# weilonghu/KGC-GCN

Hardware: AMD Instinct MI355X
Metric: aggregated_edges_per_sec (higher is better)
Workload: dtype f32 (dense step as six bf16-split MFMA products, f32 accumulation: f32-faithful); 1 GPU; wn18rr-shape synthetic graph (N=40943, R=11, E=86835), 2-layer M-GCN encoder 100->200->200, full-graph forward, eval mode; n_ranks_seen=1

## Files before the change

include/mgcn_hip.h:

```cpp
#ifndef MGCN_HIP_H
#define MGCN_HIP_H

#include <stddef.h>
#include <stdint.h>

#ifdef __cplusplus
extern "C" {
#endif

#define MGCN_ABI_VERSION 4

enum {
  MGCN_OK = 0,
  MGCN_EINVAL = 1,
  MGCN_ELAUNCH = 2,
  MGCN_EUNSUPPORTED = 3
};

typedef struct mgcn_edge_rec {
  int32_t src;
  int32_t type;
  float norm;
  int32_t eid;
} mgcn_edge_rec;

int mgcn_abi_version(void);
const char *mgcn_last_error(void);

typedef struct mgcn_ingest mgcn_ingest;
int mgcn_ingest_open(const char *train_path, const char *valid_path, const char *test_path, mgcn_ingest **out);
void mgcn_ingest_close(mgcn_ingest *h);
int64_t mgcn_ingest_count(const mgcn_ingest *h, int32_t what);
int mgcn_ingest_triples(const mgcn_ingest *h, int32_t split, int64_t *triples_host);
int64_t mgcn_ingest_names_bytes(const mgcn_ingest *h, int32_t kind);
int mgcn_ingest_names(const mgcn_ingest *h, int32_t kind, char *bytes_host, int64_t *offsets_host);

int mgcn_filter_index_build(int64_t num_triples, const int64_t *triples_host, int64_t num_relations, int64_t *keys_host,
                            int64_t *ptr_host, int32_t *tails_host, int64_t *num_keys, int64_t *num_tails);

int mgcn_csr_build_host(int64_t num_nodes, int64_t num_edges_half, int64_t num_rel_rows,
                        const int64_t *edge_index_host, const int64_t *edge_type_host,
                        int64_t hub_threshold, int64_t hub_chunk, int32_t *rowptr_host,
                        mgcn_edge_rec *rec_host, int64_t *perm_host, int32_t *hubinfo_host,
                        int32_t *chunks_host, int64_t max_chunks, int64_t *num_chunks_host,
                        int32_t *slot_dst_host, int32_t *mirror_host, int32_t *typeptr_host,
                        int32_t *typeslots_host);

int64_t mgcn_hub_partial_floats(int64_t num_chunks, int32_t dim);
int mgcn_aggregate_fwd(int64_t num_nodes, int64_t num_edges_half, int32_t dim, int32_t num_rel_rows,
                       const int32_t *rowptr_dev, const mgcn_edge_rec *rec_dev, const float *x_dev,
                       int64_t ldx, const float *rel_dev, const float *loop_rel_dev, const float *ee_dev,
                       int32_t ee_in_slot_order, const float *loop_edge_dev, float *a_dev, int64_t lda,
                       int64_t node_begin, int64_t node_end, const int32_t *hubinfo_dev, const int32_t *chunks_dev,
                       int64_t chunk_begin, int64_t chunk_end, float *partial_dev, int64_t ee_sub_in, int64_t ee_sub_out,
                       int64_t ee_sub_hub, void *stream);

int mgcn_aggregate_bwd(int64_t num_nodes, int64_t num_edges_half, int32_t dim, int32_t num_rel_rows,
                       const int32_t *rowptr_dev, const mgcn_edge_rec *rec_dev,
                       const int32_t *slot_dst_dev , const int32_t *mirror_dev,
                       const int32_t *hubinfo_dev, const int32_t *chunks_dev, int64_t num_hub_chunks,
                       const int32_t *typeptr_dev, const int32_t *typeslots_dev, const float *x_dev, int64_t ldx, const float *rel_dev, const float *ee_dev,
                       const float *g_dev, int64_t ldg, float *gx_dev, float *gee_dev, float *grel_dev,
                       float *workspace_dev, size_t workspace_bytes, void *stream);
size_t mgcn_aggregate_bwd_workspace(int64_t num_edges_half, int32_t dim, int32_t num_rel_rows, int64_t num_hub_chunks);

size_t mgcn_aggregate_bwd_shard_workspace(int64_t shard_rows, int32_t dim, int32_t num_rel_rows, int64_t num_hub_chunks);
int mgcn_aggregate_bwd_shard(int64_t num_nodes, int64_t num_edges_half, int32_t dim, int32_t num_rel_rows,
                             const mgcn_edge_rec *rec_dev, const int32_t *slot_dst_dev, int64_t node_begin, int64_t node_end,
                             int64_t rows_in, int64_t rows_out, int64_t rows_hub, int64_t ee_sub_in, int64_t ee_sub_out,
                             int64_t ee_sub_hub, const int32_t *src_ptr_dev, const int32_t *src_rows_dev,
                             const int32_t *hubinfo_dev, const int32_t *src_chunks_dev, int64_t num_hub_chunks,
                             const int32_t *type_ptr_dev, const int32_t *type_rows_dev, const float *x_dev, int64_t ldx,
                             const float *rel_dev, const float *ee_dev, const float *g_dev, int64_t ldg, float *gx_dev,
                             float *gee_dev, float *grel_dev, float *workspace_dev, size_t workspace_bytes, void *stream);

int mgcn_dense_bn_tanh_fwd(int64_t num_nodes, int32_t dim_in, int32_t dim_out, const float *a_dev, int64_t lda,
                           const float *w_dev, const float *bias_dev, const float *bn_mean_dev, const float *bn_var_dev,
                           const float *bn_gamma_dev, const float *bn_beta_dev, float bn_eps,
                           float *out_dev, int64_t ldo, void *stream);

int mgcn_fused_kernel_generation(int32_t dim_in, int32_t dim_out, int64_t num_rows, int32_t with_row_bounds);
int mgcn_layer_fwd_fused(int64_t num_nodes, int64_t num_edges_half, int32_t dim_in, int32_t dim_out,
                         int32_t num_rel_rows, const int32_t *rowptr_dev, const mgcn_edge_rec *rec_dev,
                         const float *x_dev, int64_t ldx, const float *rel_dev, const float *loop_rel_dev,
                         const float *ee_dev, int32_t ee_in_slot_order, const float *loop_edge_dev,
                         const float *wp_dev, const float *bias_dev, const float *bn_mean_dev,
                         const float *bn_var_dev, const float *bn_gamma_dev, const float *bn_beta_dev,
                         float bn_eps, float *out_dev, int64_t ldo, int64_t node_begin, int64_t node_end,
                         int64_t ee_sub_in, int64_t ee_sub_out, int64_t ee_sub_hub, const int32_t *hubinfo_dev,
                         const int32_t *chunks_dev, int64_t chunk_begin, int64_t chunk_end, float *partial_dev,
                         const float *rels_weight_dev, float *rel_out_dev, const int32_t *row_bounds_dev,
                         int32_t num_row_bounds, int32_t tune, uint32_t *status_dev, void *stream);
int mgcn_pack_weights(int32_t dim_in, int32_t dim_out, const float *w_dev, float *wp_dev, size_t wp_bytes, void *stream);
size_t mgcn_packed_weights_bytes(int32_t dim_in, int32_t dim_out);
int mgcn_pack_weights_gen(int32_t generation, int32_t dim_in, int32_t dim_out, const float *w_dev, float *wp_dev,
                          size_t wp_bytes, void *stream);
size_t mgcn_packed_weights_bytes_gen(int32_t generation, int32_t dim_in, int32_t dim_out);

size_t mgcn_bn_tanh_train_workspace(int64_t num_rows, int32_t dim_out);
int mgcn_bn_tanh_train_fwd(int64_t num_rows, int32_t dim_out, const float *u_in_dev, const float *u_out_dev,
                           const float *u_loop_dev, int64_t ldu, const float *bias_dev, const float *gamma_dev,
                           const float *beta_dev, float *running_mean_dev, float *running_var_dev, float momentum, float eps,
                           float *z_dev, float *y_dev, float *save_mean_dev, float *save_rstd_dev, float *workspace_dev,
                           size_t workspace_bytes, void *stream);
int mgcn_bn_tanh_train_bwd(int64_t num_rows, int32_t dim_out, const float *z_dev, const float *y_dev, const float *gy_dev,
                           const float *save_mean_dev, const float *save_rstd_dev, const float *gamma_dev, float *gz_dev,
                           float *gu_dev, float *ggamma_dev, float *gbeta_dev, float *workspace_dev, size_t workspace_bytes,
                           void *stream);

int mgcn_bn_train_stage_sum(int64_t num_rows, int32_t dim_out, const float *u_in_dev, const float *u_out_dev,
                            const float *u_loop_dev, int64_t ldu, const float *bias_dev, float *z_dev, float *part_dev, void *stream);
int mgcn_bn_train_stage_center(int64_t num_rows, int32_t dim_out, const float *z_dev, const float *sum_parts_dev, int64_t num_blocks,
                               int64_t total_rows, float *mean_dev, float *part_dev, void *stream);
int mgcn_bn_train_stage_finish(int64_t num_rows, int32_t dim_out, const float *z_dev, const float *sq_parts_dev, int64_t num_blocks,
                               int64_t total_rows, const float *mean_dev, const float *gamma_dev, const float *beta_dev,
                               float *running_mean_dev, float *running_var_dev, float momentum, float eps, float *rstd_dev,
                               float *y_dev, void *stream);
int mgcn_bn_train_bwd_stage_sums(int64_t num_rows, int32_t dim_out, const float *z_dev, const float *y_dev, const float *gy_dev,
                                 const float *save_mean_dev, const float *save_rstd_dev, float *g_part_dev, float *gx_part_dev,
                                 void *stream);
int mgcn_bn_train_bwd_stage_apply(int64_t num_rows, int32_t dim_out, const float *z_dev, const float *y_dev, const float *gy_dev,
                                  const float *save_mean_dev, const float *save_rstd_dev, const float *gamma_dev,
                                  const float *g_parts_dev, const float *gx_parts_dev, int64_t num_blocks, int64_t total_rows,
                                  float *gz_dev, float *gu_dev, float *ggamma_dev, float *gbeta_dev, void *stream);

size_t mgcn_matmul_tn_workspace(int64_t k, int32_t m, int32_t n);
int mgcn_matmul_tn_f32(int64_t k, int32_t m, int32_t n, const float *a_dev, int64_t lda, const float *b_dev, int64_t ldb,
                       float *c_dev, int64_t ldc, float *workspace_dev, size_t workspace_bytes, void *stream);

int mgcn_matmul_f32(int64_t m, int32_t k, int32_t n, const float *a_dev, int64_t lda, const float *b_dev,
                    int64_t ldb, float *c_dev, int64_t ldc, void *stream);

int mgcn_score_fwd(int32_t batch, int64_t n_local, int32_t dim, const float *x_dev, int64_t ldx,
                   const float *ent_dev, int64_t lde, const float *bias_dev, float *score_dev, int64_t lds,
                   void *stream);
int mgcn_score_target(int32_t batch, int64_t n_local, int64_t ent_row0, int32_t dim, const float *x_dev,
                      int64_t ldx, const float *ent_dev, int64_t lde, const float *bias_dev,
                      const int64_t *obj_dev, float *target_dev, void *stream);
int mgcn_score_rank(int32_t batch, int64_t n_local, int64_t ent_row0, int32_t dim, const float *x_dev,
                    int64_t ldx, const float *ent_dev, int64_t lde, const float *bias_dev,
                    const int64_t *obj_dev, const float *target_dev, const float *label_dev, int64_t ldl,
                    const uint32_t *mask_dev, int64_t ldm, int64_t *counts_dev, void *stream);
int64_t mgcn_score_bce_partials(int32_t batch, int64_t n_local);
int mgcn_score_bce_fwd(int32_t batch, int64_t n_local, int32_t dim, const float *x_dev, int64_t ldx, const float *ent_dev,
                       int64_t lde, const float *bias_dev, const uint32_t *mask_dev, int64_t ldm, float hot, float cold,
                       float inv_count, float *grad_logit_dev, int64_t ldg, float *loss_partial_dev, void *stream);

int mgcn_filter_mask(int32_t batch, const int64_t *qkey_dev, int64_t num_keys, const int64_t *keys_dev,
                     const int64_t *ptr_dev, const int32_t *tails_dev, int64_t ent_row0, int64_t n_local,
                     uint32_t *mask_dev, int64_t ldm, void *stream);

int mgcn_label_rows(int32_t batch, const int64_t *qkey_dev, int64_t num_keys, const int64_t *keys_dev,
                    const int64_t *ptr_dev, const int32_t *tails_dev, int64_t ent_row0, int64_t n_local, float hot,
                    float cold, float *out_dev, int64_t ldo, void *stream);

size_t mgcn_score_topk_workspace(int32_t batch, int64_t n_local, int32_t k);
int mgcn_score_topk(int32_t batch, int64_t n_local, int64_t ent_row0, int32_t dim, const float *x_dev, int64_t ldx,
                    const float *ent_dev, int64_t lde, const float *bias_dev, const uint32_t *mask_dev, int64_t ldm,
                    int32_t k, float *out_score_dev, int64_t ldo, int64_t *out_id_dev, int64_t ldi, void *workspace_dev,
                    size_t workspace_bytes, void *stream);
int mgcn_topk_merge(int32_t batch, int32_t lists, const float *in_score_dev, const int64_t *in_id_dev, int64_t ld_in,
                    int32_t k, float *out_score_dev, int64_t *out_id_dev, void *stream);

size_t mgcn_conve_packed_bytes(int32_t k_w, int32_t k_h, int32_t kernel_size, int32_t num_filter, int32_t dim_out);
int mgcn_conve_pack(int32_t k_w, int32_t k_h, int32_t kernel_size, int32_t num_filter, int32_t dim_out,
                    const float *conv_w_dev, const float *conv_b_dev, const float *fc_w_dev, int64_t ldw,
                    const float *fc_b_dev, const float *bn0_mean_dev, const float *bn0_var_dev,
                    const float *bn0_gamma_dev, const float *bn0_beta_dev, float bn0_eps, const float *bn1_mean_dev,
                    const float *bn1_var_dev, const float *bn1_gamma_dev, const float *bn1_beta_dev, float bn1_eps,
                    const float *bn2_mean_dev, const float *bn2_var_dev, const float *bn2_gamma_dev,
                    const float *bn2_beta_dev, float bn2_eps, void *packed_dev, size_t packed_bytes, void *stream);
size_t mgcn_conve_trunk_workspace(int32_t batch, int32_t k_w, int32_t k_h, int32_t kernel_size, int32_t num_filter,
                                  int32_t dim_out);
int mgcn_conve_trunk_fwd(int32_t batch, int32_t k_w, int32_t k_h, int32_t kernel_size, int32_t num_filter,
                         int32_t dim_out, const float *ent_dev, int64_t lde, int64_t ent_rows,
                         const int64_t *src_index_dev, const float *rel_dev, int64_t ldr, int64_t rel_rows,
                         const int64_t *rel_index_dev, const void *packed_dev, float *out_dev, int64_t ldo,
                         void *workspace_dev, size_t workspace_bytes, void *stream);

size_t mgcn_conve_train_workspace(int32_t batch, int32_t k_w, int32_t k_h, int32_t kernel_size, int32_t num_filter,
                                  int32_t dim_out);
int mgcn_conve_train_fwd(int32_t batch, int32_t k_w, int32_t k_h, int32_t kernel_size, int32_t num_filter, int32_t dim_out,
                         const float *s_dev, int64_t lds, const float *r_dev, int64_t ldr, const float *conv_w_dev,
                         const float *conv_b_dev, const float *fc_w_dev, int64_t ldw, const float *fc_b_dev,
                         const float *bn0_gamma_dev, const float *bn0_beta_dev, float *bn0_running_mean_dev,
                         float *bn0_running_var_dev, float bn0_momentum, float bn0_eps, const float *bn1_gamma_dev,
                         const float *bn1_beta_dev, float *bn1_running_mean_dev, float *bn1_running_var_dev, float bn1_momentum,
                         float bn1_eps, const uint8_t *keep_dev, float inv_keep, float *z_dev, int64_t ldz, float *saved_dev,
                         void *workspace_dev, size_t workspace_bytes, void *stream);
int mgcn_conve_train_bwd(int32_t batch, int32_t k_w, int32_t k_h, int32_t kernel_size, int32_t num_filter, int32_t dim_out,
                         const float *s_dev, int64_t lds, const float *r_dev, int64_t ldr, const float *conv_w_dev,
                         const float *fc_w_dev, int64_t ldw, const float *bn0_gamma_dev, const float *bn0_beta_dev,
                         const float *bn1_gamma_dev, const float *bn1_beta_dev, const uint8_t *keep_dev, float inv_keep,
                         const float *saved_dev, const float *gz_dev, int64_t ldg, float *ds_dev, int64_t ldds, float *dr_dev,
                         int64_t lddr, float *d_conv_w_dev, float *d_conv_b_dev, float *d_bn0_gamma_dev, float *d_bn0_beta_dev,
                         float *d_bn1_gamma_dev, float *d_bn1_beta_dev, float *d_fc_w_dev, int64_t lddw, float *d_fc_b_dev,
                         void *workspace_dev, size_t workspace_bytes, void *stream);

#define MGCN_ADAM_CHUNK 8192
#define MGCN_ADAM_BATCH 64
size_t mgcn_adam_sq_norms_workspace(int64_t n, const int64_t *numel_host);
int mgcn_adam_sq_norms(int64_t n, const float *const *grad_host, const int64_t *numel_host, float *sq_dev,
                       void *workspace_dev, size_t workspace_bytes, void *stream);
int mgcn_adam_clip_coef(int64_t n, const float *sq_dev, float max_norm, float *out_dev, void *stream);
int mgcn_adam_step(int64_t n, const float *const *grad_host, float *const *param_host, float *const *exp_avg_host,
                   float *const *exp_avg_sq_host, const int64_t *numel_host, const float *coef_dev, float step_size,
                   float bc2_sqrt, double beta1, double beta2, double eps, double weight_decay, void *stream);

#define MGCN_QUERY_MAX_BATCH 4096
size_t mgcn_query_rows_bwd_workspace(int32_t batch);
int mgcn_query_rows_bwd(int32_t batch, int64_t num_rows, int32_t dim, const int64_t *idx_dev, const float *d_dev, int64_t ldd,
                        float *out_dev, int64_t ldo, void *workspace_dev, size_t workspace_bytes, void *stream);
int mgcn_conve_tail_fwd(int32_t batch, int32_t dim, const float *z_dev, int64_t ldz, const uint8_t *keep_dev, int64_t ldk,
                        float inv_keep, const float *gamma_dev, const float *beta_dev, float *running_mean_dev,
                        float *running_var_dev, float momentum, float eps, float *x_dev, int64_t ldx, float *saved_dev,
                        int64_t ldsv, void *stream);
int mgcn_conve_tail_bwd(int32_t batch, int32_t dim, const float *z_dev, int64_t ldz, const uint8_t *keep_dev, int64_t ldk,
                        float inv_keep, const float *x_dev, int64_t ldx, const float *saved_dev, int64_t ldsv,
                        const float *gamma_dev, const float *gx_dev, int64_t ldg, float *gz_dev, int64_t ldgz,
                        float *d_gamma_dev, float *d_beta_dev, void *stream);

#ifdef __cplusplus
}
#endif
#endif
```

kgc-gcn_amd/_native.py:

```python
import ctypes
import os

import torch

_HERE = os.path.dirname(os.path.abspath(__file__))
LIB_PATH = os.environ.get('MGCN_LIB') or os.path.join(_HERE, 'csrc', 'libmgcn_hip.so')
ABI_VERSION = 4

_lib = None

_i32, _i64, _f32 = ctypes.c_int32, ctypes.c_int64, ctypes.c_float
_ptr = ctypes.c_void_p

_SIGNATURES = {
    'mgcn_abi_version': (ctypes.c_int, []),
    'mgcn_last_error': (ctypes.c_char_p, []),
    'mgcn_csr_build_host': (ctypes.c_int, [_i64, _i64, _i64, _ptr, _ptr, _i64, _i64, _ptr, _ptr, _ptr, _ptr, _ptr, _i64,
                                           _ptr] + [_ptr] * 4),
    'mgcn_aggregate_fwd': (ctypes.c_int, [_i64, _i64, _i32, _i32, _ptr, _ptr, _ptr, _i64, _ptr, _ptr, _ptr, _i32,
                                          _ptr, _ptr, _i64, _i64, _i64, _ptr, _ptr, _i64, _i64, _ptr, _i64, _i64, _i64, _ptr]),
    'mgcn_aggregate_bwd': (ctypes.c_int, [_i64, _i64, _i32, _i32] + [_ptr] * 6 + [_i64, _ptr, _ptr] +
                           [_ptr, _i64, _ptr, _ptr, _ptr, _i64, _ptr, _ptr, _ptr, _ptr, ctypes.c_size_t, _ptr]),
    'mgcn_aggregate_bwd_workspace': (ctypes.c_size_t, [_i64, _i32, _i32, _i64]),
    'mgcn_aggregate_bwd_shard': (ctypes.c_int, [_i64, _i64, _i32, _i32, _ptr, _ptr] + [_i64] * 8 + [_ptr] * 4 + [_i64, _ptr, _ptr,
                                                _ptr, _i64, _ptr, _ptr, _ptr, _i64, _ptr, _ptr, _ptr, _ptr, ctypes.c_size_t, _ptr]),
    'mgcn_aggregate_bwd_shard_workspace': (ctypes.c_size_t, [_i64, _i32, _i32, _i64]),
    'mgcn_bn_train_stage_sum': (ctypes.c_int, [_i64, _i32, _ptr, _ptr, _ptr, _i64, _ptr, _ptr, _ptr, _ptr]),
    'mgcn_bn_train_stage_center': (ctypes.c_int, [_i64, _i32, _ptr, _ptr, _i64, _i64, _ptr, _ptr, _ptr]),
    'mgcn_bn_train_stage_finish': (ctypes.c_int, [_i64, _i32, _ptr, _ptr, _i64, _i64] + [_ptr] * 5 + [_f32, _f32, _ptr, _ptr, _ptr]),
    'mgcn_bn_train_bwd_stage_sums': (ctypes.c_int, [_i64, _i32] + [_ptr] * 8),
    'mgcn_bn_train_bwd_stage_apply': (ctypes.c_int, [_i64, _i32] + [_ptr] * 8 + [_i64, _i64] + [_ptr] * 5),
    'mgcn_dense_bn_tanh_fwd': (ctypes.c_int, [_i64, _i32, _i32, _ptr, _i64] + [_ptr] * 6 + [_f32, _ptr, _i64, _ptr]),
    'mgcn_layer_fwd_fused': (ctypes.c_int, [_i64, _i64, _i32, _i32, _i32, _ptr, _ptr, _ptr, _i64, _ptr, _ptr, _ptr, _i32,
                                            _ptr, _ptr, _ptr, _ptr, _ptr, _ptr, _ptr, _f32, _ptr, _i64, _i64, _i64,
                                            _i64, _i64, _i64, _ptr, _ptr, _i64, _i64, _ptr, _ptr, _ptr, _ptr, _i32, _i32, _ptr,
                                            _ptr]),
    'mgcn_pack_weights': (ctypes.c_int, [_i32, _i32, _ptr, _ptr, ctypes.c_size_t, _ptr]),
    'mgcn_packed_weights_bytes': (ctypes.c_size_t, [_i32, _i32]),
    'mgcn_pack_weights_gen': (ctypes.c_int, [_i32, _i32, _i32, _ptr, _ptr, ctypes.c_size_t, _ptr]),
    'mgcn_packed_weights_bytes_gen': (ctypes.c_size_t, [_i32, _i32, _i32]),
    'mgcn_matmul_f32': (ctypes.c_int, [_i64, _i32, _i32, _ptr, _i64, _ptr, _i64, _ptr, _i64, _ptr]),
    'mgcn_bn_tanh_train_workspace': (ctypes.c_size_t, [_i64, _i32]),
    'mgcn_bn_tanh_train_fwd': (ctypes.c_int, [_i64, _i32, _ptr, _ptr, _ptr, _i64, _ptr, _ptr, _ptr, _ptr, _ptr, _f32, _f32, _ptr,
                                              _ptr, _ptr, _ptr, _ptr, ctypes.c_size_t, _ptr]),
    'mgcn_bn_tanh_train_bwd': (ctypes.c_int, [_i64, _i32] + [_ptr] * 11 + [ctypes.c_size_t, _ptr]),
    'mgcn_matmul_tn_workspace': (ctypes.c_size_t, [_i64, _i32, _i32]),
    'mgcn_matmul_tn_f32': (ctypes.c_int, [_i64, _i32, _i32, _ptr, _i64, _ptr, _i64, _ptr, _i64, _ptr, ctypes.c_size_t, _ptr]),
    'mgcn_score_fwd': (ctypes.c_int, [_i32, _i64, _i32, _ptr, _i64, _ptr, _i64, _ptr, _ptr, _i64, _ptr]),
    'mgcn_score_target': (ctypes.c_int, [_i32, _i64, _i64, _i32, _ptr, _i64, _ptr, _i64, _ptr, _ptr, _ptr, _ptr]),
    'mgcn_score_rank': (ctypes.c_int, [_i32, _i64, _i64, _i32, _ptr, _i64, _ptr, _i64, _ptr, _ptr, _ptr, _ptr, _i64,
                                       _ptr, _i64, _ptr, _ptr]),
    'mgcn_filter_mask': (ctypes.c_int, [_i32, _ptr, _i64, _ptr, _ptr, _ptr, _i64, _i64, _ptr, _i64, _ptr]),
    'mgcn_score_bce_partials': (_i64, [_i32, _i64]),
    'mgcn_hub_partial_floats': (_i64, [_i64, _i32]),
    'mgcn_fused_kernel_generation': (ctypes.c_int, [_i32, _i32, _i64, _i32]),
    'mgcn_score_bce_fwd': (ctypes.c_int, [_i32, _i64, _i32, _ptr, _i64, _ptr, _i64, _ptr, _ptr, _i64, _f32, _f32, _f32, _ptr,
                                          _i64, _ptr, _ptr]),
    'mgcn_label_rows': (ctypes.c_int, [_i32, _ptr, _i64, _ptr, _ptr, _ptr, _i64, _i64, _f32, _f32, _ptr, _i64, _ptr]),
    'mgcn_score_topk_workspace': (ctypes.c_size_t, [_i32, _i64, _i32]),
    'mgcn_score_topk': (ctypes.c_int, [_i32, _i64, _i64, _i32, _ptr, _i64, _ptr, _i64, _ptr, _ptr, _i64, _i32, _ptr, _i64,
                                       _ptr, _i64, _ptr, ctypes.c_size_t, _ptr]),
    'mgcn_topk_merge': (ctypes.c_int, [_i32, _i32, _ptr, _ptr, _i64, _i32, _ptr, _ptr, _ptr]),
    'mgcn_conve_packed_bytes': (ctypes.c_size_t, [_i32] * 5),
    'mgcn_conve_pack': (ctypes.c_int, [_i32] * 5 + [_ptr, _ptr, _ptr, _i64, _ptr] + ([_ptr] * 4 + [_f32]) * 3 +
                        [_ptr, ctypes.c_size_t, _ptr]),
    'mgcn_conve_trunk_workspace': (ctypes.c_size_t, [_i32] * 6),
    'mgcn_conve_trunk_fwd': (ctypes.c_int, [_i32] * 6 + [_ptr, _i64, _i64, _ptr, _ptr, _i64, _i64, _ptr, _ptr, _ptr, _i64, _ptr,
                                            ctypes.c_size_t, _ptr]),
    'mgcn_conve_train_workspace': (ctypes.c_size_t, [_i32] * 6),
    'mgcn_conve_train_fwd': (ctypes.c_int, [_i32] * 6 + [_ptr, _i64, _ptr, _i64, _ptr, _ptr, _ptr, _i64, _ptr] +
                             [_ptr, _ptr, _ptr, _ptr, _f32, _f32] * 2 + [_ptr, _f32, _ptr, _i64, _ptr, _ptr, ctypes.c_size_t, _ptr]),
    'mgcn_conve_train_bwd': (ctypes.c_int, [_i32] * 6 + [_ptr, _i64, _ptr, _i64, _ptr, _ptr, _i64] + [_ptr] * 5 + [_f32, _ptr, _ptr, _i64,
                                                         _ptr, _i64, _ptr, _i64] + [_ptr] * 7 + [_i64, _ptr, _ptr, ctypes.c_size_t, _ptr]),
    'mgcn_adam_sq_norms_workspace': (ctypes.c_size_t, [_i64, _ptr]),
    'mgcn_adam_sq_norms': (ctypes.c_int, [_i64, _ptr, _ptr, _ptr, _ptr, ctypes.c_size_t, _ptr]),
    'mgcn_adam_clip_coef': (ctypes.c_int, [_i64, _ptr, _f32, _ptr, _ptr]),
    'mgcn_adam_step': (ctypes.c_int, [_i64] + [_ptr] * 6 + [_f32, _f32] + [ctypes.c_double] * 4 + [_ptr]),
    'mgcn_query_rows_bwd_workspace': (ctypes.c_size_t, [_i32]),
    'mgcn_query_rows_bwd': (ctypes.c_int, [_i32, _i64, _i32, _ptr, _ptr, _i64, _ptr, _i64, _ptr, ctypes.c_size_t, _ptr]),
    'mgcn_conve_tail_fwd': (ctypes.c_int, [_i32, _i32, _ptr, _i64, _ptr, _i64, _f32, _ptr, _ptr, _ptr, _ptr, _f32, _f32, _ptr, _i64, _ptr,
                                           _i64, _ptr]),
    'mgcn_conve_tail_bwd': (ctypes.c_int, [_i32, _i32, _ptr, _i64, _ptr, _i64, _f32, _ptr, _i64, _ptr, _i64, _ptr, _ptr, _i64, _ptr, _i64,
                                           _ptr, _ptr, _ptr]),
    'mgcn_ingest_open': (ctypes.c_int, [ctypes.c_char_p, ctypes.c_char_p, ctypes.c_char_p, ctypes.POINTER(_ptr)]),
    'mgcn_ingest_close': (None, [_ptr]),
    'mgcn_ingest_count': (_i64, [_ptr, _i32]),
    'mgcn_ingest_triples': (ctypes.c_int, [_ptr, _i32, _ptr]),
    'mgcn_ingest_names_bytes': (_i64, [_ptr, _i32]),
    'mgcn_ingest_names': (ctypes.c_int, [_ptr, _i32, _ptr, _ptr]),
    'mgcn_filter_index_build': (ctypes.c_int, [_i64, _ptr, _i64, _ptr, _ptr, _ptr, ctypes.POINTER(_i64), ctypes.POINTER(_i64)]),
}

EXPORTS = tuple(sorted(_SIGNATURES))


class NativeError(RuntimeError):
    pass


class FusedUnsupported(NativeError):
    """mgcn_layer_fwd_fused returned MGCN_EUNSUPPORTED (misaligned operand, shape outside the kernel): callers take the
    aggregation + dense launches instead."""


def lib():
    global _lib
    if _lib is None:
        if not os.path.exists(LIB_PATH):
            raise NativeError('%s not found: build it with `python -c "import __graft_entry__ as g; g.build()"` '
                              '(hipcc --offload-arch=gfx950). There is no CPU fallback.' % LIB_PATH)
        handle = ctypes.CDLL(LIB_PATH)
        for name, (res, args) in _SIGNATURES.items():
            fn = getattr(handle, name)
            fn.restype, fn.argtypes = res, args
        if handle.mgcn_abi_version() != ABI_VERSION:
            raise NativeError('libmgcn_hip.so ABI %d, binding expects %d' % (handle.mgcn_abi_version(), ABI_VERSION))
        _lib = handle
    return _lib


def _check(rc, what):
    if rc != 0:
        raise NativeError('%s failed (%d): %s' % (what, rc, lib().mgcn_last_error().decode()))


def _dev(t, dtype, what, allow_none=False):
    if t is None:
        if allow_none:
            return None
        raise NativeError('%s: tensor required' % what)
    if not t.is_cuda:
        raise NativeError('%s must live on a GPU (got %s): the M-GCN hot path has no CPU fallback' % (what, t.device))
    if t.dtype != dtype:
        raise NativeError('%s: dtype %s, expected %s' % (what, t.dtype, dtype))
    if t.dim() > 0 and t.numel() > 0 and t.size(-1) > 1 and t.stride(-1) != 1:
        raise NativeError('%s: last dimension must be contiguous' % what)
    return t.data_ptr()


def _ld(t):
    return t.stride(0) if t.dim() == 2 and t.size(0) > 1 else t.size(-1)


def _stream(t):
    return torch.cuda.current_stream(t.device).cuda_stream


def _same_device(*ts):
    devs = {t.device for t in ts if t is not None}
    if len(devs) > 1:
        raise NativeError('tensors on different devices: %s' % sorted(map(str, devs)))


HUB_THRESHOLD = int(os.environ.get('MGCN_HUB_THRESHOLD', '32'))
HUB_CHUNK = int(os.environ.get('MGCN_HUB_CHUNK', '64'))


def csr_build_host(num_nodes, num_rel_rows, edge_index, edge_type, with_backward=True, hub_threshold=None,
                   hub_chunk=None):
    ei = edge_index.detach().to('cpu', torch.int64).contiguous()
    et = edge_type.detach().to('cpu', torch.int64).contiguous()
    if ei.dim() != 2 or ei.size(0) != 2 or ei.size(1) % 2 or et.numel() != ei.size(1):
        raise NativeError('csr_build: edge_index must be [2, 2E] and edge_type [2E]')
    E2, E, N = ei.size(1), ei.size(1) // 2, int(num_nodes)
    thr = HUB_THRESHOLD if hub_threshold is None else int(hub_threshold)
    chk = HUB_CHUNK if hub_chunk is None else int(hub_chunk)
    max_chunks = (E2 // max(chk, 1) + E2 // max(thr, 1) + 2) if thr > 0 else 0
    out = dict(rowptr=torch.empty((2, N + 1), dtype=torch.int32), rec=torch.empty((E2, 4), dtype=torch.int32),
               perm=torch.empty(E2, dtype=torch.int64), hubinfo=torch.empty((2, N, 2), dtype=torch.int32),
               chunks=torch.empty((max(max_chunks, 1), 4), dtype=torch.int32))
    nch = ctypes.c_int64(0)
    if with_backward:
        out.update(slot_dst=torch.empty(E2, dtype=torch.int32), mirror=torch.empty(E2, dtype=torch.int32),
                   typeptr=torch.empty(num_rel_rows + 1, dtype=torch.int32),
                   typeslots=torch.empty(E2, dtype=torch.int32))
    p = lambda k: out[k].data_ptr() if k in out else None
    _check(lib().mgcn_csr_build_host(N, E, int(num_rel_rows), ei.data_ptr(), et.data_ptr(), thr, chk, p('rowptr'),
                                     p('rec'), p('perm'), p('hubinfo'), p('chunks'), max_chunks, ctypes.byref(nch),
                                     p('slot_dst'), p('mirror'), p('typeptr'), p('typeslots')),
           'mgcn_csr_build_host')
    out['num_chunks'] = int(nch.value)
    out['chunks'] = out['chunks'][:max(int(nch.value), 1)].contiguous()
    return out


def _hub_args(csr, d, device, n0, n1):
    c0, c1 = csr.chunk_range(n0, n1)
    if c1 == c0:
        return None, None, 0, 0, None
    cache = csr.__dict__.setdefault('_hub_partials', {})
    key = (int(d), c0, c1, str(device))
    hit = cache.get(key)
    stream = torch.cuda.current_stream(device)
    if hit is None:
        hit = cache[key] = [torch.zeros(int(lib().mgcn_hub_partial_floats(c1 - c0, int(d))), dtype=torch.float32, device=device),
                            stream]
    elif hit[1] != stream and not torch.cuda.is_current_stream_capturing():
        stream.wait_stream(hit[1])
        hit[1] = stream
    return _dev(csr.hubinfo, torch.int32, 'hubinfo'), _dev(csr.chunks, torch.int32, 'chunks'), c0, c1, hit[0]


def _hub_failed(csr, d, device, n0, n1):
    c0, c1 = csr.chunk_range(n0, n1)
    csr.__dict__.get('_hub_partials', {}).pop((int(d), c0, c1, str(device)), None)


def aggregate_fwd(csr, x, rel, ee, ee_in_slot_order, loop_edge, out, loop_rel=None, node_range=None, ee_sub=(0, 0, 0),
                  out_row0=0):
    N, E, D = csr.num_nodes, csr.num_edges_half, x.size(1)
    _same_device(csr.rowptr, x, rel, ee, loop_edge, out, loop_rel)
    if loop_rel is None:
        if rel.size(0) != csr.num_rel_rows:
            raise NativeError('aggregate_fwd: rel has %d rows, graph expects %d' % (rel.size(0), csr.num_rel_rows))
        loop_rel, rel = rel[-1], rel[:-1]
    if x.size(0) != N or rel.size(0) != csr.num_rel_rows - 1 or rel.size(1) != D or loop_rel.numel() != D:
        raise NativeError('aggregate_fwd: x %s / rel %s do not match graph (N=%d, rel rows=%d)'
                          % (tuple(x.shape), tuple(rel.shape), N, csr.num_rel_rows))
    ee_sub = tuple(int(v) for v in ee_sub)
    sharded = ee_sub != (0, 0, 0) or (ee is not None and ee.size(0) != 2 * E)
    if ee is not None and not sharded and tuple(ee.shape) != (2 * E, D):
        raise NativeError('aggregate_fwd: per-edge table %s, expected (%d, %d)' % (tuple(ee.shape), 2 * E, D))
    if not rel.is_contiguous() or (ee is not None and not ee.is_contiguous()):
        raise NativeError('aggregate_fwd: relation and per-edge tables must be contiguous')
    modes = 3 if loop_edge is not None else 2
    if loop_edge is not None and loop_edge.numel() != D:
        raise NativeError('aggregate_fwd: loop_edge must have %d elements' % D)
    n0, n1 = (0, N) if node_range is None else (int(node_range[0]), int(node_range[1]))
    if not 0 <= n0 <= n1 <= N:
        raise NativeError('aggregate_fwd: node range (%d, %d) outside [0, %d]' % (n0, n1, N))
    out_row0 = int(out_row0)
    if out.size(1) < modes * D or out_row0 > n0 or out_row0 + out.size(0) < n1 or (out_row0 == 0 and node_range is None and out.size(0) != N):
        raise NativeError('aggregate_fwd: out %s (rows from %d) does not cover destinations [%d, %d) x %d columns'
                          % (tuple(out.shape), out_row0, n0, n1, modes * D))
    if sharded:
        rows = csr.shard_slot_counts(n0, n1)
        if ee is None or not ee_in_slot_order or tuple(ee.shape) != (sum(rows), D) or not ee.is_contiguous() or \
                ee_sub != csr.shard_ee_sub(n0, n1):
            raise NativeError('aggregate_fwd: per-edge shard does not match destinations [%d, %d)' % (n0, n1))
        if ee.numel() == 0:
            ee = x.new_zeros((1, D))
    hub_info, hub_chunks, hub_c0, hub_c1, hub_partial = _hub_args(csr, D, x.device, n0, n1)
    rc = lib().mgcn_aggregate_fwd(
        N, E, D, csr.num_rel_rows, _dev(csr.rowptr, torch.int32, 'rowptr'), _dev(csr.rec, torch.int32, 'rec'),
        _dev(x, torch.float32, 'x'), _ld(x), _dev(rel, torch.float32, 'rel'), _dev(loop_rel, torch.float32, 'loop_rel'),
        _dev(ee, torch.float32, 'ee', True), int(bool(ee_in_slot_order)), _dev(loop_edge, torch.float32, 'loop_edge', True),
        _dev(out, torch.float32, 'out') - out_row0 * _ld(out) * 4, _ld(out), n0, n1, hub_info, hub_chunks, hub_c0, hub_c1,
        _dev(hub_partial, torch.float32, 'partial', True), ee_sub[0], ee_sub[1], ee_sub[2], _stream(x))
    if rc != 0 and hub_partial is not None:
        _hub_failed(csr, D, x.device, n0, n1)
    _check(rc, 'mgcn_aggregate_fwd')
    return out


def _bwd_out(out, i, want, shape, device, what):
    given = None if out is None else out[i]
    if not want:
        if given is not None:
            raise NativeError('%s: out[%d] given for a gradient that is not computed' % (what, i))
        return None
    if given is None:
        return torch.empty(shape, dtype=torch.float32, device=device)
    if tuple(given.shape) != tuple(shape) or given.dtype != torch.float32 or given.device != device or not given.is_contiguous():
        raise NativeError('%s: out[%d] must be a contiguous float32 %s on %s' % (what, i, tuple(shape), device))
    return given


def aggregate_bwd(csr, x, rel, ee, g, want_gx=True, want_gee=True, want_grel=True, out=None):
    N, E, D = csr.num_nodes, csr.num_edges_half, x.size(1)
    _same_device(csr.rowptr, x, rel, ee, g)
    if not csr.has_backward:
        raise NativeError('aggregate_bwd: graph was prepared without the backward indices')
    if want_gx and not csr.mirrored:
        raise NativeError('aggregate_bwd: the edge list is not mirror-symmetric (edge e + E is not the reverse of edge e, '
                          'data_loader.py:143-149), so the gradient w.r.t. the layer input cannot be formed from the '
                          'destination runs; forward, per-edge and relation gradients are unaffected')
    if g.size(0) != N or g.size(1) < 2 * D:
        raise NativeError('aggregate_bwd: g %s too small' % (tuple(g.shape),))
    if x.size(0) != N or tuple(rel.shape) != (csr.num_rel_rows, D) or not rel.is_contiguous():
        raise NativeError('aggregate_bwd: x / rel do not match the graph')
    if ee is not None and (tuple(ee.shape) != (2 * E, D) or not ee.is_contiguous()):
        raise NativeError('aggregate_bwd: per-edge table must be contiguous (%d, %d) in slot order' % (2 * E, D))
    if out is not None and len(out) != 3:
        raise NativeError('aggregate_bwd: out must be (gx, gee, grel)')
    gx = _bwd_out(out, 0, want_gx, (N, D), x.device, 'aggregate_bwd')
    gee = _bwd_out(out, 1, want_gee and ee is not None, (2 * E, D), x.device, 'aggregate_bwd')
    grel = _bwd_out(out, 2, want_grel, (csr.num_rel_rows, D), x.device, 'aggregate_bwd')
    need_ws = want_grel or (want_gx and csr.num_chunks > 0)
    ws_bytes = lib().mgcn_aggregate_bwd_workspace(E, D, csr.num_rel_rows, csr.num_chunks) if need_ws else 0
    ws = torch.empty(max(ws_bytes // 4, 1), dtype=torch.float32, device=x.device) if need_ws else None
    hubs = csr.num_chunks > 0
    _check(lib().mgcn_aggregate_bwd(
        N, E, D, csr.num_rel_rows, _dev(csr.rowptr, torch.int32, 'rowptr'), _dev(csr.rec, torch.int32, 'rec'),
        _dev(csr.slot_dst, torch.int32, 'slot_dst'), _dev(csr.mirror, torch.int32, 'mirror'),
        _dev(csr.hubinfo, torch.int32, 'hubinfo') if hubs else None,
        _dev(csr.chunks, torch.int32, 'chunks') if hubs else None, csr.num_chunks,
        _dev(csr.typeptr, torch.int32, 'typeptr'), _dev(csr.typeslots, torch.int32, 'typeslots'),
        _dev(x, torch.float32, 'x'), _ld(x), _dev(rel, torch.float32, 'rel'), _dev(ee, torch.float32, 'ee', True),
        _dev(g, torch.float32, 'g'), _ld(g), _dev(gx, torch.float32, 'gx', True), _dev(gee, torch.float32, 'gee', True),
        _dev(grel, torch.float32, 'grel', True), _dev(ws, torch.float32, 'ws', True), ws_bytes, _stream(x)),
        'mgcn_aggregate_bwd')
    return gx, gee, grel


def aggregate_bwd_shard(csr, x, rel, ee, g, node_range, want_gx=True, out=None):
    N, E, D = csr.num_nodes, csr.num_edges_half, x.size(1)
    n0, n1 = int(node_range[0]), int(node_range[1])
    _same_device(csr.rowptr, x, rel, ee, g)
    if not csr.has_backward:
        raise NativeError('aggregate_bwd_shard: graph was prepared without the backward indices')
    if want_gx and not csr.mirrored:
        raise NativeError('aggregate_bwd_shard: the edge list is not mirror-symmetric: no gradient w.r.t. the layer input')
    if not 0 <= n0 <= n1 <= N:
        raise NativeError('aggregate_bwd_shard: node range (%d, %d) outside [0, %d]' % (n0, n1, N))
    if x.size(0) != N or tuple(rel.shape) != (csr.num_rel_rows, D) or not rel.is_contiguous():
        raise NativeError('aggregate_bwd_shard: x / rel do not match the graph')
    rows = csr.shard_slot_counts(n0, n1)
    if ee is None or tuple(ee.shape) != (sum(rows), D) or not ee.is_contiguous():
        raise NativeError('aggregate_bwd_shard: per-edge shard %s does not match destinations [%d, %d) (%d rows)'
                          % (None if ee is None else tuple(ee.shape), n0, n1, sum(rows)))
    if g.dim() != 2 or g.size(0) != n1 - n0 or g.size(1) < 2 * D:
        raise NativeError('aggregate_bwd_shard: g %s must be [%d, >= %d]' % (tuple(g.shape), n1 - n0, 2 * D))
    idx = csr.shard_backward_index(n0, n1)
    sub = csr.shard_ee_sub(n0, n1)
    if out is not None and len(out) != 3:
        raise NativeError('aggregate_bwd_shard: out must be (gx, gee, grel)')
    gx = _bwd_out(out, 0, want_gx, (N, D), x.device, 'aggregate_bwd_shard')
    gee = _bwd_out(out, 1, True, (sum(rows), D), x.device, 'aggregate_bwd_shard')
    grel = _bwd_out(out, 2, True, (csr.num_rel_rows, D), x.device, 'aggregate_bwd_shard')
    hubs = csr.num_chunks > 0
    ws_bytes = lib().mgcn_aggregate_bwd_shard_workspace(sum(rows), D, csr.num_rel_rows, csr.num_chunks)
    ws = torch.empty(max(ws_bytes // 4, 4), dtype=torch.float32, device=x.device)
    nz = lambda t, dtype, what: _dev(t, dtype, what) if t.numel() > 0 else None
    _check(lib().mgcn_aggregate_bwd_shard(
        N, E, D, csr.num_rel_rows, _dev(csr.rec, torch.int32, 'rec'), _dev(csr.slot_dst, torch.int32, 'slot_dst'), n0, n1,
        rows[0], rows[1], rows[2], sub[0], sub[1], sub[2], _dev(idx['src_ptr'], torch.int32, 'src_ptr'),
        nz(idx['src_rows'], torch.int32, 'src_rows'), _dev(csr.hubinfo, torch.int32, 'hubinfo') if hubs else None,
        _dev(idx['src_chunks'], torch.int32, 'src_chunks') if hubs else None, csr.num_chunks,
        _dev(idx['type_ptr'], torch.int32, 'type_ptr'), nz(idx['type_rows'], torch.int32, 'type_rows'), _dev(x, torch.float32, 'x'), _ld(x),
        _dev(rel, torch.float32, 'rel'), nz(ee, torch.float32, 'ee'), nz(g, torch.float32, 'g'), _ld(g) if g.numel() > 0 else 2 * D,
        _dev(gx, torch.float32, 'gx', True), nz(gee, torch.float32, 'gee'), _dev(grel, torch.float32, 'grel'), _dev(ws, torch.float32, 'ws'),
        ws_bytes, _stream(x)), 'mgcn_aggregate_bwd_shard')
    return gx, gee, grel


def dense_bn_tanh_fwd(a, w_cat, bias, bn_mean, bn_var, bn_gamma, bn_beta, eps, out):
    N, O = a.size(0), w_cat.size(1)
    D = w_cat.size(0) // 3
    _same_device(a, w_cat, bias, bn_mean, bn_var, bn_gamma, bn_beta, out)
    if w_cat.dim() != 2 or w_cat.size(0) != 3 * D or not w_cat.is_contiguous():
        raise NativeError('dense_bn_tanh_fwd: w_cat must be contiguous (3D, O)')
    for v in (bn_mean, bn_var, bn_gamma, bn_beta) + ((bias,) if bias is not None else ()):
        if v.numel() != O:
            raise NativeError('dense_bn_tanh_fwd: per-column vectors must have %d elements' % O)
    if a.size(1) < 3 * D or tuple(out.shape) != (N, O):
        raise NativeError('dense_bn_tanh_fwd: a %s / out %s do not match' % (tuple(a.shape), tuple(out.shape)))
    _check(lib().mgcn_dense_bn_tanh_fwd(
        N, D, O, _dev(a, torch.float32, 'a'), _ld(a), _dev(w_cat, torch.float32, 'w_cat'),
        _dev(bias, torch.float32, 'bias', True), _dev(bn_mean, torch.float32, 'bn_mean'),
        _dev(bn_var, torch.float32, 'bn_var'), _dev(bn_gamma, torch.float32, 'bn_gamma'),
        _dev(bn_beta, torch.float32, 'bn_beta'), float(eps), _dev(out, torch.float32, 'out'), _ld(out), _stream(a)),
        'mgcn_dense_bn_tanh_fwd')
    return out


FUSED_TUNE = int(os.environ.get('MGCN_FUSED_TUNE', '0'), 0)


def tune_generation(tune=None):
    f = ((FUSED_TUNE if tune is None else int(tune)) >> 10) & 3
    return 0 if f == 0 else (4 if f == 1 else f)


_FUSED_STATUS = {}


def fused_status(device):
    key = str(torch.device(device))
    if key not in _FUSED_STATUS:
        _FUSED_STATUS[key] = torch.zeros(1, dtype=torch.int32, device=device)
    return _FUSED_STATUS[key]


def check_fused_status(device):
    key = str(torch.device(device))
    if key in _FUSED_STATUS:
        v = int(_FUSED_STATUS[key].item())
        if v:
            _FUSED_STATUS[key].zero_()
            raise NativeError('a fused layer launch on %s reported status %d: a bounded LDS-counter spin ran out '
                              '(layer_fused3.hip), rows of that launch are invalid' % (key, v))
FUSED_ENABLED = os.environ.get('MGCN_FUSED', '1') != '0'


_CU_COUNT = {}


def _cu_count(device):
    key = str(device)
    if key not in _CU_COUNT:
        _CU_COUNT[key] = int(torch.cuda.get_device_properties(device).multi_processor_count)
    return _CU_COUNT[key]


def fused_supported(d_in, d_out):
    return FUSED_ENABLED and d_in % 4 == 0 and d_in <= 1024 and d_out % 4 == 0 and d_out <= 512


def pack_weights(w_cat, out=None, generation=None):
    D, O = w_cat.size(0) // 3, w_cat.size(1)
    if w_cat.dim() != 2 or w_cat.size(0) != 3 * D or not w_cat.is_contiguous():
        raise NativeError('pack_weights: w_cat must be contiguous (3D, O)')
    gen = tune_generation() if generation is None else int(generation)
    nbytes = lib().mgcn_packed_weights_bytes_gen(gen, D, O)
    if out is None:
        out = torch.empty(nbytes // 4, dtype=torch.float32, device=w_cat.device)
    if out.numel() * 4 < nbytes:
        raise NativeError('pack_weights: out too small')
    _same_device(w_cat, out)
    _check(lib().mgcn_pack_weights_gen(gen, D, O, _dev(w_cat, torch.float32, 'w_cat'), _dev(out, torch.float32, 'wp'),
                                       out.numel() * 4, _stream(w_cat)), 'mgcn_pack_weights')
    return out


def layer_fwd_fused(csr, x, rel, loop_rel, ee, ee_in_slot_order, loop_edge, w_packed, d_out, bias, bn_mean, bn_var,
                    bn_gamma, bn_beta, eps, out, node_range=None, ee_sub=(0, 0, 0), rels_weight=None, rel_out=None,
                    tune=None, balance=True):
    N, E, D, O = csr.num_nodes, csr.num_edges_half, x.size(1), int(d_out)
    n0, n1 = (0, N) if node_range is None else (int(node_range[0]), int(node_range[1]))
    if not 0 <= n0 <= n1 <= N:
        raise NativeError('layer_fwd_fused: node range (%d, %d) outside [0, %d]' % (n0, n1, N))
    ee_sub = tuple(int(v) for v in ee_sub) + (0,) * (3 - len(ee_sub))
    sharded = ee_sub != (0, 0, 0) or (ee is not None and ee.size(0) != 2 * E)
    _same_device(csr.rowptr, x, rel, loop_rel, ee, loop_edge, w_packed, bias, bn_mean, bn_var, bn_gamma, bn_beta, out)
    if x.size(0) != N or tuple(rel.shape) != (csr.num_rel_rows - 1, D) or loop_rel.numel() != D or loop_edge.numel() != D:
        raise NativeError('layer_fwd_fused: x / rel / loop rows do not match the graph')
    if ee is not None and not sharded and (tuple(ee.shape) != (2 * E, D) or not ee.is_contiguous()):
        raise NativeError('layer_fwd_fused: per-edge table must be contiguous (%d, %d)' % (2 * E, D))
    if ee is not None and sharded:
        rows = csr.shard_slot_counts(n0, n1)
        if not ee_in_slot_order or tuple(ee.shape) != (sum(rows), D) or not ee.is_contiguous() or \
                ee_sub != csr.shard_ee_sub(n0, n1):
            raise NativeError('layer_fwd_fused: per-edge shard does not match destinations [%d, %d)' % (n0, n1))
    tune = FUSED_TUNE if tune is None else int(tune)
    if not rel.is_contiguous() or w_packed.numel() * 4 < lib().mgcn_packed_weights_bytes_gen(tune_generation(tune), D, O):
        raise NativeError('layer_fwd_fused: rel must be contiguous and w_packed sized by mgcn_packed_weights_bytes')
    for v in (bn_mean, bn_var, bn_gamma, bn_beta) + ((bias,) if bias is not None else ()):
        if v.numel() != O:
            raise NativeError('layer_fwd_fused: per-column vectors must have %d elements' % O)
    if tuple(out.shape) != (n1 - n0, O):
        raise NativeError('layer_fwd_fused: out must be (%d, %d)' % (n1 - n0, O))
    if (rels_weight is None) != (rel_out is None):
        raise NativeError('layer_fwd_fused: give rels_weight and rel_out together')
    if rel_out is not None:
        _same_device(x, rels_weight, rel_out)
        if tuple(rels_weight.shape) != (D, O) or not rels_weight.is_contiguous() or \
                tuple(rel_out.shape) != (csr.num_rel_rows - 1, O) or not rel_out.is_contiguous():
            raise NativeError('layer_fwd_fused: rels_weight must be contiguous (%d, %d) and rel_out (%d, %d)'
                              % (D, O, csr.num_rel_rows - 1, O))
    if n1 == n0 and rel_out is None:
        return out
    if ee is not None and ee.numel() == 0:
        ee = x.new_zeros((1, D))
    hub_info, hub_chunks, hub_c0, hub_c1, hub_partial = _hub_args(csr, D, x.device, n0, n1)
    bounds = csr.workgroup_bounds(n0, n1, _cu_count(x.device)) if balance and n1 > n0 else None
    rc = lib().mgcn_layer_fwd_fused(
        N, E, D, O, csr.num_rel_rows, _dev(csr.rowptr, torch.int32, 'rowptr'), _dev(csr.rec, torch.int32, 'rec'),
        _dev(x, torch.float32, 'x'), _ld(x), _dev(rel, torch.float32, 'rel'), _dev(loop_rel, torch.float32, 'loop_rel'),
        _dev(ee, torch.float32, 'ee', True), int(bool(ee_in_slot_order)), _dev(loop_edge, torch.float32, 'loop_edge'),
        _dev(w_packed, torch.float32, 'w_packed'), _dev(bias, torch.float32, 'bias', True),
        _dev(bn_mean, torch.float32, 'bn_mean'), _dev(bn_var, torch.float32, 'bn_var'),
        _dev(bn_gamma, torch.float32, 'bn_gamma'), _dev(bn_beta, torch.float32, 'bn_beta'), float(eps),
        _dev(out, torch.float32, 'out'), _ld(out), n0, n1, int(ee_sub[0]), int(ee_sub[1]), int(ee_sub[2]),
        hub_info, hub_chunks, hub_c0, hub_c1,
        _dev(hub_partial, torch.float32, 'partial', True), _dev(rels_weight, torch.float32, 'rels_weight', True),
        _dev(rel_out, torch.float32, 'rel_out', True), _dev(bounds, torch.int32, 'row_bounds', True),
        bounds.numel() - 1 if bounds is not None else 0, tune, _dev(fused_status(x.device), torch.int32, 'status'),
        _stream(x))
    if rc != 0 and hub_partial is not None:
        _hub_failed(csr, D, x.device, n0, n1)
    if rc == 3:
        raise FusedUnsupported('mgcn_layer_fwd_fused: %s' % lib().mgcn_last_error().decode())
    _check(rc, 'mgcn_layer_fwd_fused')
    return out


def matmul(a, b):
    _same_device(a, b)
    if a.dim() != 2 or b.dim() != 2 or a.size(1) != b.size(0):
        raise NativeError('matmul: shapes %s @ %s' % (tuple(a.shape), tuple(b.shape)))
    c = torch.empty((a.size(0), b.size(1)), dtype=torch.float32, device=a.device)
    _check(lib().mgcn_matmul_f32(a.size(0), a.size(1), b.size(1), _dev(a, torch.float32, 'a'), _ld(a),
                                 _dev(b, torch.float32, 'b'), _ld(b), _dev(c, torch.float32, 'c'), _ld(c), _stream(a)),
           'mgcn_matmul_f32')
    return c


def matmul_tn(a, b):
    _same_device(a, b)
    if a.dim() != 2 or b.dim() != 2 or a.size(0) != b.size(0):
        raise NativeError('matmul_tn: shapes %s^T @ %s' % (tuple(a.shape), tuple(b.shape)))
    K, M, N = a.size(0), a.size(1), b.size(1)
    c = torch.empty((M, N), dtype=torch.float32, device=a.device)
    nbytes = lib().mgcn_matmul_tn_workspace(K, M, N)
    ws = torch.empty(max(nbytes // 4, 1), dtype=torch.float32, device=a.device)
    _check(lib().mgcn_matmul_tn_f32(K, M, N, _dev(a, torch.float32, 'a'), _ld(a), _dev(b, torch.float32, 'b'), _ld(b),
                                    _dev(c, torch.float32, 'c'), _ld(c), _dev(ws, torch.float32, 'ws'), nbytes, _stream(a)),
           'mgcn_matmul_tn_f32')
    return c


def matmul_tn_supported(m, n):
    return m <= 208 and n <= 256


def bn_tanh_train_fwd(u_in, u_out, u_loop, bias, gamma, beta, running_mean, running_var, momentum, eps):
    N, O = u_in.shape
    _same_device(u_in, u_out, u_loop, bias, gamma, beta, running_mean, running_var)
    for t in (u_in, u_out, u_loop):
        if tuple(t.shape) != (N, O) or t.stride(1) != 1 or t.stride(0) != u_in.stride(0):
            raise NativeError('bn_tanh_train_fwd: the three products must be [N, O] with the same row stride')
    z = torch.empty((N, O), dtype=torch.float32, device=u_in.device)
    y = torch.empty_like(z)
    mean = torch.empty(O, dtype=torch.float32, device=u_in.device)
    rstd = torch.empty_like(mean)
    nbytes = lib().mgcn_bn_tanh_train_workspace(N, O)
    ws = torch.empty(nbytes // 4, dtype=torch.float32, device=u_in.device)
    _check(lib().mgcn_bn_tanh_train_fwd(
        N, O, _dev(u_in, torch.float32, 'u_in'), _dev(u_out, torch.float32, 'u_out'), _dev(u_loop, torch.float32, 'u_loop'),
        u_in.stride(0), _dev(bias, torch.float32, 'bias', True), _dev(gamma, torch.float32, 'gamma'), _dev(beta, torch.float32, 'beta'),
        _dev(running_mean, torch.float32, 'running_mean', True), _dev(running_var, torch.float32, 'running_var', True),
        float(momentum), float(eps), _dev(z, torch.float32, 'z'), _dev(y, torch.float32, 'y'), _dev(mean, torch.float32, 'mean'),
        _dev(rstd, torch.float32, 'rstd'), _dev(ws, torch.float32, 'ws'), nbytes, _stream(u_in)), 'mgcn_bn_tanh_train_fwd')
    return y, z, mean, rstd


def bn_tanh_train_bwd(z, y, gy, mean, rstd, gamma):
    N, O = z.shape
    _same_device(z, y, gy, mean, rstd, gamma)
    gy = gy.contiguous()
    gz, gu = torch.empty_like(z), torch.empty_like(z)
    gg, gb = torch.empty_like(mean), torch.empty_like(mean)
    nbytes = lib().mgcn_bn_tanh_train_workspace(N, O)
    ws = torch.empty(nbytes // 4, dtype=torch.float32, device=z.device)
    _check(lib().mgcn_bn_tanh_train_bwd(
        N, O, _dev(z, torch.float32, 'z'), _dev(y, torch.float32, 'y'), _dev(gy, torch.float32, 'gy'), _dev(mean, torch.float32, 'mean'),
        _dev(rstd, torch.float32, 'rstd'), _dev(gamma, torch.float32, 'gamma'), _dev(gz, torch.float32, 'gz'), _dev(gu, torch.float32, 'gu'),
        _dev(gg, torch.float32, 'ggamma'), _dev(gb, torch.float32, 'gbeta'), _dev(ws, torch.float32, 'ws'), nbytes, _stream(z)),
        'mgcn_bn_tanh_train_bwd')
    return gz, gu, gg, gb


BN_BLOCK = 128


def bn_blocks(rows):
    return (int(rows) + BN_BLOCK - 1) // BN_BLOCK


def _bn_parts(parts, O, what):
    if parts.dim() != 2 or parts.size(0) < 1 or parts.size(1) != O or not parts.is_contiguous():
        raise NativeError('%s: block partials must be contiguous [blocks >= 1, %d]' % (what, O))
    return parts.size(0)


def bn_train_stage_sum(u_in, u_out, u_loop, bias):
    n, O = u_in.shape
    _same_device(u_in, u_out, u_loop, bias)
    for t in (u_in, u_out, u_loop):
        if tuple(t.shape) != (n, O) or (n > 0 and (t.stride(1) != 1 or t.stride(0) != u_in.stride(0))):
            raise NativeError('bn_train_stage_sum: the three products must be [N, O] with the same row stride')
    if bias is not None and bias.numel() != O:
        raise NativeError('bn_train_stage_sum: bias must have %d elements' % O)
    z = torch.empty((n, O), dtype=torch.float32, device=u_in.device)
    part = torch.empty((bn_blocks(n), O), dtype=torch.float32, device=u_in.device)
    if n > 0:
        _check(lib().mgcn_bn_train_stage_sum(n, O, _dev(u_in, torch.float32, 'u_in'), _dev(u_out, torch.float32, 'u_out'),
                                             _dev(u_loop, torch.float32, 'u_loop'), u_in.stride(0), _dev(bias, torch.float32, 'bias', True),
                                             _dev(z, torch.float32, 'z'), _dev(part, torch.float32, 'part'), _stream(u_in)),
               'mgcn_bn_train_stage_sum')
    return z, part


def bn_train_stage_center(z, sum_parts, total_rows):
    n, O = z.shape
    _same_device(z, sum_parts)
    nb = _bn_parts(sum_parts, O, 'bn_train_stage_center')
    mean = torch.empty(O, dtype=torch.float32, device=z.device)
    part = torch.empty((bn_blocks(n), O), dtype=torch.float32, device=z.device)
    _check(lib().mgcn_bn_train_stage_center(n, O, _dev(z, torch.float32, 'z', n == 0), _dev(sum_parts, torch.float32, 'sum_parts'), nb,
                                            int(total_rows), _dev(mean, torch.float32, 'mean'),
                                            _dev(part, torch.float32, 'part') if n > 0 else None, _stream(sum_parts)),
           'mgcn_bn_train_stage_center')
    return mean, part


def bn_train_stage_finish(z, sq_parts, total_rows, mean, gamma, beta, running_mean, running_var, momentum, eps):
    n, O = z.shape
    _same_device(z, sq_parts, mean, gamma, beta, running_mean, running_var)
    nb = _bn_parts(sq_parts, O, 'bn_train_stage_finish')
    for v in (mean, gamma, beta) + tuple(t for t in (running_mean, running_var) if t is not None):
        if v.numel() != O or not v.is_contiguous():
            raise NativeError('bn_train_stage_finish: per-column vectors must be contiguous with %d elements' % O)
    y = torch.empty_like(z)
    rstd = torch.empty(O, dtype=torch.float32, device=z.device)
    _check(lib().mgcn_bn_train_stage_finish(
        n, O, _dev(z, torch.float32, 'z', n == 0), _dev(sq_parts, torch.float32, 'sq_parts'), nb, int(total_rows),
        _dev(mean, torch.float32, 'mean'), _dev(gamma, torch.float32, 'gamma'), _dev(beta, torch.float32, 'beta'),
        _dev(running_mean, torch.float32, 'running_mean', True), _dev(running_var, torch.float32, 'running_var', True),
        float(momentum), float(eps), _dev(rstd, torch.float32, 'rstd'), _dev(y, torch.float32, 'y') if n > 0 else None,
        _stream(sq_parts)), 'mgcn_bn_train_stage_finish')
    return y, rstd


def bn_train_bwd_stage_sums(z, y, gy, mean, rstd):
    n, O = z.shape
    _same_device(z, y, gy, mean, rstd)
    gy = gy.contiguous()
    part = torch.empty((2, bn_blocks(n), O), dtype=torch.float32, device=z.device)
    if n > 0:
        _check(lib().mgcn_bn_train_bwd_stage_sums(n, O, _dev(z, torch.float32, 'z'), _dev(y, torch.float32, 'y'),
                                                  _dev(gy, torch.float32, 'gy'), _dev(mean, torch.float32, 'mean'),
                                                  _dev(rstd, torch.float32, 'rstd'), _dev(part[0], torch.float32, 'g_part'),
                                                  _dev(part[1], torch.float32, 'gx_part'), _stream(z)), 'mgcn_bn_train_bwd_stage_sums')
    return part


def bn_train_bwd_stage_apply(z, y, gy, mean, rstd, gamma, g_parts, gx_parts, total_rows):
    n, O = z.shape
    _same_device(z, y, gy, mean, rstd, gamma, g_parts, gx_parts)
    nb = _bn_parts(g_parts, O, 'bn_train_bwd_stage_apply')
    if _bn_parts(gx_parts, O, 'bn_train_bwd_stage_apply') != nb:
        raise NativeError('bn_train_bwd_stage_apply: g / gx partials differ in blocks')
    gy = gy.contiguous()
    gz, gu = torch.empty_like(z), torch.empty_like(z)
    gg, gb = torch.empty_like(mean), torch.empty_like(mean)
    live = n > 0
    _check(lib().mgcn_bn_train_bwd_stage_apply(
        n, O, _dev(z, torch.float32, 'z', not live), _dev(y, torch.float32, 'y', not live), _dev(gy, torch.float32, 'gy', not live),
        _dev(mean, torch.float32, 'mean'), _dev(rstd, torch.float32, 'rstd'), _dev(gamma, torch.float32, 'gamma'),
        _dev(g_parts, torch.float32, 'g_parts'), _dev(gx_parts, torch.float32, 'gx_parts'), nb, int(total_rows),
        _dev(gz, torch.float32, 'gz') if live else None, _dev(gu, torch.float32, 'gu') if live else None,
        _dev(gg, torch.float32, 'ggamma'), _dev(gb, torch.float32, 'gbeta'), _stream(mean)), 'mgcn_bn_train_bwd_stage_apply')
    return gz, gu, gg, gb


def _score_args(x, ent, bias):
    _same_device(x, ent, bias)
    if x.dim() != 2 or ent.dim() != 2 or x.size(1) != ent.size(1) or bias.numel() != ent.size(0):
        raise NativeError('score: x %s, ent %s, bias %s do not match' % (tuple(x.shape), tuple(ent.shape), tuple(bias.shape)))
    return x.size(0), ent.size(0), x.size(1)


def score_fwd(x, ent, bias):
    B, n, O = _score_args(x, ent, bias)
    out = torch.empty((B, n), dtype=torch.float32, device=x.device)
    _check(lib().mgcn_score_fwd(B, n, O, _dev(x, torch.float32, 'x'), _ld(x), _dev(ent, torch.float32, 'ent'), _ld(ent),
                                _dev(bias, torch.float32, 'bias'), _dev(out, torch.float32, 'score'), _ld(out),
                                _stream(x)), 'mgcn_score_fwd')
    return out


def score_target(x, ent, bias, obj, ent_row0=0, out=None):
    B, n, O = _score_args(x, ent, bias)
    if obj.numel() != B:
        raise NativeError('score_target: obj must have %d elements' % B)
    if out is None:
        out = torch.zeros(B, dtype=torch.float32, device=x.device)
    _check(lib().mgcn_score_target(B, n, int(ent_row0), O, _dev(x, torch.float32, 'x'), _ld(x),
                                   _dev(ent, torch.float32, 'ent'), _ld(ent), _dev(bias, torch.float32, 'bias'),
                                   _dev(obj, torch.int64, 'obj'), _dev(out, torch.float32, 'target'), _stream(x)),
           'mgcn_score_target')
    return out


def score_rank(x, ent, bias, obj, target, label=None, ent_row0=0, counts=None, mask=None):
    B, n, O = _score_args(x, ent, bias)
    if (label is None) == (mask is None):
        raise NativeError('score_rank: give exactly one of label / mask')
    if obj.numel() != B or target.numel() != B:
        raise NativeError('score_rank: obj/target do not match batch %d' % B)
    if label is not None and (label.dim() != 2 or label.size(0) != B or label.size(1) != n):
        raise NativeError('score_rank: label must be (%d, %d)' % (B, n))
    if mask is not None and (mask.dim() != 2 or mask.size(0) != B or mask.size(1) < (n + 31) // 32 or not mask.is_contiguous()):
        raise NativeError('score_rank: mask must be contiguous (%d, >= %d)' % (B, (n + 31) // 32))
    if counts is None:
        counts = torch.zeros((B, 3), dtype=torch.int64, device=x.device)
    _same_device(x, ent, bias, obj, target, label, mask, counts)
    _check(lib().mgcn_score_rank(B, n, int(ent_row0), O, _dev(x, torch.float32, 'x'), _ld(x),
                                 _dev(ent, torch.float32, 'ent'), _ld(ent), _dev(bias, torch.float32, 'bias'),
                                 _dev(obj, torch.int64, 'obj'), _dev(target, torch.float32, 'target'),
                                 _dev(label, torch.float32, 'label', True), _ld(label) if label is not None else 0,
                                 _dev(mask, torch.int32, 'mask', True), mask.size(1) if mask is not None else 0,
                                 _dev(counts, torch.int64, 'counts'), _stream(x)), 'mgcn_score_rank')
    return counts


TOPK_MAX = 1024


def _check_k(k, what):
    if not 1 <= int(k) <= TOPK_MAX:
        raise NativeError('%s: k = %d outside [1, %d]' % (what, int(k), TOPK_MAX))
    return int(k)


def _topk_out(out, B, k, device, what, contiguous):
    if out is None:
        return (torch.empty((B, k), dtype=torch.float32, device=device),
                torch.empty((B, k), dtype=torch.int64, device=device))
    scores, ids = out
    for t, name in ((scores, 'scores'), (ids, 'ids')):
        if t.dim() != 2 or tuple(t.shape) != (B, k):
            raise NativeError('%s: out %s %s must be (%d, %d)' % (what, name, tuple(t.shape), B, k))
        if contiguous and not t.is_contiguous():
            raise NativeError('%s: out %s must be contiguous' % (what, name))
        if B > 1 and t.stride(0) < k:
            raise NativeError('%s: out %s rows overlap (stride %d < %d)' % (what, name, t.stride(0), k))
    return scores, ids


def score_topk(x, ent, bias, k, mask=None, ent_row0=0, out=None):
    B, n, O = _score_args(x, ent, bias)
    k = _check_k(k, 'score_topk')
    if mask is not None and (mask.dim() != 2 or mask.size(0) != B or mask.size(1) < (n + 31) // 32 or not mask.is_contiguous()):
        raise NativeError('score_topk: mask must be contiguous (%d, >= %d)' % (B, (n + 31) // 32))
    scores, ids = _topk_out(out, B, k, x.device, 'score_topk', False)
    _same_device(x, ent, bias, mask, scores, ids)
    nbytes = lib().mgcn_score_topk_workspace(B, n, k)
    ws = torch.empty(max(nbytes, 16), dtype=torch.uint8, device=x.device)
    _check(lib().mgcn_score_topk(B, n, int(ent_row0), O, _dev(x, torch.float32, 'x'), _ld(x),
                                 _dev(ent, torch.float32, 'ent'), _ld(ent), _dev(bias, torch.float32, 'bias'),
                                 _dev(mask, torch.int32, 'mask', True), mask.size(1) if mask is not None else 0, k,
                                 _dev(scores, torch.float32, 'scores'), _ld(scores),
                                 _dev(ids, torch.int64, 'ids'), _ld(ids),
                                 _dev(ws, torch.uint8, 'workspace'), nbytes, _stream(x)), 'mgcn_score_topk')
    return scores, ids


def topk_merge(scores, ids, k, out=None):
    k = _check_k(k, 'topk_merge')
    _same_device(scores, ids)
    if scores.dim() != 2 or ids.shape != scores.shape or scores.size(1) % k != 0:
        raise NativeError('topk_merge: scores %s / ids %s must be equal [B, lists * %d]' % (tuple(scores.shape), tuple(ids.shape), k))
    B, lists = scores.size(0), scores.size(1) // k
    scores, ids = scores.contiguous(), ids.contiguous()
    out_s, out_i = _topk_out(out, B, k, scores.device, 'topk_merge', True)
    _same_device(scores, out_s, out_i)
    _check(lib().mgcn_topk_merge(B, lists, _dev(scores, torch.float32, 'scores'), _dev(ids, torch.int64, 'ids'),
                                 scores.size(1), k, _dev(out_s, torch.float32, 'out scores'),
                                 _dev(out_i, torch.int64, 'out ids'), _stream(scores)), 'mgcn_topk_merge')
    return out_s, out_i


def conve_supported(k_w, k_h, kernel_size, num_filter, dim_out):
    geom = tuple(int(v) for v in (k_w, k_h, kernel_size, num_filter, dim_out))
    return min(geom) >= 1 and lib().mgcn_conve_packed_bytes(*geom) > 0


def conve_pack(geom, conv_w, conv_b, fc_w, fc_b, bn0, bn1, bn2, out=None):
    geom = tuple(int(v) for v in geom)
    nbytes = lib().mgcn_conve_packed_bytes(*geom)
    if nbytes == 0:
        raise NativeError('conve_pack: geometry %s is not supported' % (geom,))
    if not conv_w.is_contiguous() or fc_w.dim() != 2:
        raise NativeError('conve_pack: conv weight must be contiguous, fc weight 2-d')
    if out is None or out.numel() * 4 < nbytes or out.device != fc_w.device:
        out = torch.empty(nbytes // 4, dtype=torch.float32, device=fc_w.device)
    args = []
    for mean, var, gamma, beta, eps in (bn0, bn1, bn2):
        _same_device(fc_w, mean, var, gamma, beta)
        args += [_dev(mean, torch.float32, 'bn mean'), _dev(var, torch.float32, 'bn var'), _dev(gamma, torch.float32, 'bn weight', True),
                 _dev(beta, torch.float32, 'bn bias', True), float(eps)]
    _same_device(fc_w, conv_w, conv_b, fc_b, out)
    _check(lib().mgcn_conve_pack(*geom, _dev(conv_w, torch.float32, 'conv weight'), _dev(conv_b, torch.float32, 'conv bias', True),
                                 _dev(fc_w, torch.float32, 'fc weight'), _ld(fc_w), _dev(fc_b, torch.float32, 'fc bias', True),
                                 *args, _dev(out, torch.float32, 'pack'), out.numel() * 4, _stream(fc_w)), 'mgcn_conve_pack')
    return out


def conve_trunk(geom, packed, ent, src, rel, rel_idx, out=None):
    geom = tuple(int(v) for v in geom)
    O = geom[4]
    if ent.dim() != 2 or rel.dim() != 2 or ent.size(1) != O or rel.size(1) != O:
        raise NativeError('conve_trunk: tables must be [rows, %d], got %s and %s' % (O, tuple(ent.shape), tuple(rel.shape)))
    if (src is None) != (rel_idx is None):
        raise NativeError('conve_trunk: give both index vectors or neither')
    B = int(src.numel()) if src is not None else int(ent.size(0))
    if src is not None and (rel_idx.numel() != B or not src.is_contiguous() or not rel_idx.is_contiguous()):
        raise NativeError('conve_trunk: index vectors must be contiguous and of equal length')
    if src is None and rel.size(0) != B:
        raise NativeError('conve_trunk: without index vectors both tables need the same number of rows')
    _same_device(ent, rel, src, rel_idx, packed, out)
    if out is None:
        out = torch.empty((B, O), dtype=torch.float32, device=ent.device)
    elif out.dim() != 2 or out.size(0) != B or out.size(1) != O:
        raise NativeError('conve_trunk: out must be [%d, %d]' % (B, O))
    if B == 0:
        return out
    nbytes = lib().mgcn_conve_trunk_workspace(B, *geom)
    ws = torch.empty(nbytes, dtype=torch.uint8, device=ent.device) if nbytes else None
    _check(lib().mgcn_conve_trunk_fwd(B, *geom, _dev(ent, torch.float32, 'ent'), _ld(ent), ent.size(0),
                                      _dev(src, torch.int64, 'src', True), _dev(rel, torch.float32, 'rel'), _ld(rel), rel.size(0),
                                      _dev(rel_idx, torch.int64, 'rel index', True), _dev(packed, torch.float32, 'pack'),
                                      _dev(out, torch.float32, 'out'), _ld(out) if B > 1 else max(out.stride(0), O),
                                      _dev(ws, torch.uint8, 'workspace', True), nbytes, _stream(ent)), 'mgcn_conve_trunk_fwd')
    return out


def conve_train_supported(batch, geom):
    geom = tuple(int(v) for v in geom)
    return min(geom) >= 1 and int(batch) >= 1 and lib().mgcn_conve_train_workspace(int(batch), *geom) > 0


def _rows(t, O, what):
    if t.dim() != 2 or t.size(1) != O:
        raise NativeError('%s must be [B, %d], got %s' % (what, O, tuple(t.shape)))
    return _dev(t, torch.float32, what), (_ld(t) if t.size(0) > 1 else max(t.stride(0), O))


def conve_train_fwd(geom, s, r, conv_w, conv_b, fc_w, fc_b, bn0, bn1, keep, inv_keep):
    geom = tuple(int(v) for v in geom)
    O, B = geom[4], int(s.size(0))
    nbytes = lib().mgcn_conve_train_workspace(B, *geom)
    if nbytes == 0:
        raise NativeError('conve_train_fwd: batch %d of geometry %s is not supported' % (B, geom))
    if not conv_w.is_contiguous() or fc_w.dim() != 2 or (keep is not None and not keep.is_contiguous()):
        raise NativeError('conve_train_fwd: conv weight and mask must be contiguous, fc weight 2-d')
    _same_device(s, r, conv_w, conv_b, fc_w, fc_b, keep, *bn0[:4], *bn1[:4])
    sp, lds = _rows(s, O, 's')
    rp, ldr = _rows(r, O, 'r')
    z = torch.empty((B, O), dtype=torch.float32, device=s.device)
    saved = torch.empty(2 + 2 * geom[3], dtype=torch.float32, device=s.device)
    ws = torch.empty(nbytes, dtype=torch.uint8, device=s.device)
    bn_args = []
    for gamma, beta, rm, rv, mom, eps in (bn0, bn1):
        bn_args += [_dev(gamma, torch.float32, 'bn weight'), _dev(beta, torch.float32, 'bn bias'), _dev(rm, torch.float32, 'running mean'),
                    _dev(rv, torch.float32, 'running var'), float(mom), float(eps)]
    _check(lib().mgcn_conve_train_fwd(B, *geom, sp, lds, rp, ldr, _dev(conv_w, torch.float32, 'conv weight'),
                                      _dev(conv_b, torch.float32, 'conv bias', True), _dev(fc_w, torch.float32, 'fc weight'), _ld(fc_w),
                                      _dev(fc_b, torch.float32, 'fc bias', True), *bn_args,
                                      None if keep is None else keep.data_ptr(), float(inv_keep), _dev(z, torch.float32, 'z'), O,
                                      _dev(saved, torch.float32, 'saved'), ws.data_ptr(), nbytes, _stream(s)), 'mgcn_conve_train_fwd')
    return z, saved, ws


def conve_train_bwd(geom, s, r, conv_w, fc_w, bn0_weight, bn0_bias, bn1_weight, bn1_bias, keep, inv_keep, saved, ws, gz, want):
    geom = tuple(int(v) for v in geom)
    k_w, k_h, ks, F, O = geom
    B = int(s.size(0))
    sp, lds = _rows(s, O, 's')
    rp, ldr = _rows(r, O, 'r')
    gp, ldg = _rows(gz, O, 'gz')
    _same_device(s, r, conv_w, fc_w, keep, saved, ws, gz)
    shapes = {'s': (B, O), 'r': (B, O), 'conv_w': tuple(conv_w.shape), 'conv_b': (F,), 'g0': (1,), 'b0': (1,), 'g1': (F,), 'b1': (F,),
              'fc_w': (O, fc_w.size(1)), 'fc_b': (O,)}
    out = {k: torch.empty(shapes[k], dtype=torch.float32, device=s.device) for k in shapes if k in want}
    ptr = lambda k: out[k].data_ptr() if k in out else None
    _check(lib().mgcn_conve_train_bwd(B, *geom, sp, lds, rp, ldr, _dev(conv_w, torch.float32, 'conv weight'),
                                      _dev(fc_w, torch.float32, 'fc weight'), _ld(fc_w), _dev(bn0_weight, torch.float32, 'bn0 weight'),
                                      _dev(bn0_bias, torch.float32, 'bn0 bias'), _dev(bn1_weight, torch.float32, 'bn1 weight'),
                                      _dev(bn1_bias, torch.float32, 'bn1 bias'), None if keep is None else keep.data_ptr(),
                                      float(inv_keep), _dev(saved, torch.float32, 'saved'), gp, ldg, ptr('s'), O, ptr('r'), O,
                                      ptr('conv_w'), ptr('conv_b'), ptr('g0'), ptr('b0'), ptr('g1'), ptr('b1'), ptr('fc_w'),
                                      fc_w.size(1), ptr('fc_b'), ws.data_ptr(), ws.numel(), _stream(s)), 'mgcn_conve_train_bwd')
    return out


QUERY_MAX_BATCH = 4096


def query_rows_supported(batch):
    return 1 <= int(batch) <= QUERY_MAX_BATCH


def query_rows_bwd(idx, d, num_rows, out=None):
    if idx.dim() != 1 or d.dim() != 2 or d.size(0) != idx.numel():
        raise NativeError('query_rows_bwd: idx must be [B] and d [B, dim], got %s and %s' % (tuple(idx.shape), tuple(d.shape)))
    B, dim = int(d.size(0)), int(d.size(1))
    if out is None:
        out = torch.empty((int(num_rows), dim), dtype=torch.float32, device=d.device)
    elif out.dim() != 2 or tuple(out.shape) != (int(num_rows), dim):
        raise NativeError('query_rows_bwd: out must be [%d, %d]' % (num_rows, dim))
    _same_device(idx, d, out)
    dp, ldd = _rows(d, dim, 'd')
    op, ldo = _rows(out, dim, 'out')
    nbytes = lib().mgcn_query_rows_bwd_workspace(B)
    if nbytes == 0:
        raise NativeError('query_rows_bwd: a batch of %d is not supported' % B)
    ws = torch.empty(nbytes, dtype=torch.uint8, device=d.device)
    _check(lib().mgcn_query_rows_bwd(B, int(num_rows), dim, _dev(idx.contiguous(), torch.int64, 'idx'), dp, ldd, op, ldo, ws.data_ptr(),
                                     nbytes, _stream(d)), 'mgcn_query_rows_bwd')
    return out


def conve_tail_supported(batch, dim):
    return 2 <= int(batch) <= QUERY_MAX_BATCH and int(dim) >= 1


def _keep_rows(keep, B, O):
    if keep is None:
        return None, O
    if keep.dtype not in (torch.bool, torch.uint8) or tuple(keep.shape) != (B, O) or (O > 1 and keep.stride(1) != 1):
        raise NativeError('conve tail: keep must be bool / uint8 [%d, %d] with a contiguous last dimension' % (B, O))
    return keep.data_ptr(), max(keep.stride(0), O)


def conve_tail_fwd(z, keep, inv_keep, gamma, beta, running_mean, running_var, momentum, eps):
    B, O = int(z.size(0)), int(z.size(1))
    _same_device(z, keep, gamma, beta, running_mean, running_var)
    zp, ldz = _rows(z, O, 'z')
    kp, ldk = _keep_rows(keep, B, O)
    x = torch.empty((B, O), dtype=torch.float32, device=z.device)
    saved = torch.empty((2, O), dtype=torch.float32, device=z.device)
    _check(lib().mgcn_conve_tail_fwd(B, O, zp, ldz, kp, ldk, float(inv_keep), _dev(gamma, torch.float32, 'bn weight'),
                                     _dev(beta, torch.float32, 'bn bias'), _dev(running_mean, torch.float32, 'running mean'),
                                     _dev(running_var, torch.float32, 'running var'), float(momentum), float(eps), x.data_ptr(), O,
                                     saved.data_ptr(), O, _stream(z)), 'mgcn_conve_tail_fwd')
    return x, saved


def conve_tail_bwd(z, keep, inv_keep, x, saved, gamma, gx, want=('z', 'gamma', 'beta')):
    B, O = int(z.size(0)), int(z.size(1))
    _same_device(z, keep, x, saved, gamma, gx)
    zp, ldz = _rows(z, O, 'z')
    kp, ldk = _keep_rows(keep, B, O)
    xp, ldx = _rows(x, O, 'x')
    gp, ldg = _rows(gx, O, 'gx')
    if tuple(saved.shape) != (2, O) or not saved.is_contiguous():
        raise NativeError('conve_tail_bwd: saved must be contiguous [2, %d]' % O)
    new = lambda name, shape: torch.empty(shape, dtype=torch.float32, device=z.device) if name in want else None
    gz, dg, db = new('z', (B, O)), new('gamma', (O,)), new('beta', (O,))
    ptr = lambda t: None if t is None else t.data_ptr()
    _check(lib().mgcn_conve_tail_bwd(B, O, zp, ldz, kp, ldk, float(inv_keep), xp, ldx, _dev(saved, torch.float32, 'saved'), O,
                                     _dev(gamma, torch.float32, 'bn weight'), gp, ldg, ptr(gz), O, ptr(dg), ptr(db), _stream(z)),
           'mgcn_conve_tail_bwd')
    return gz, dg, db


def filter_mask(qkey, keys, ptr, tails, n_local, ent_row0=0, out=None):
    B, words = qkey.numel(), (int(n_local) + 31) // 32
    if out is None:
        out = torch.empty((B, words), dtype=torch.int32, device=qkey.device)
    if out.size(0) != B or out.size(1) < words or not out.is_contiguous():
        raise NativeError('filter_mask: out must be contiguous (%d, >= %d)' % (B, words))
    if ptr.numel() != keys.numel() + 1:
        raise NativeError('filter_mask: ptr must have len(keys) + 1 entries')
    _same_device(qkey, keys, ptr, tails, out)
    _check(lib().mgcn_filter_mask(B, _dev(qkey, torch.int64, 'qkey'), keys.numel(), _dev(keys, torch.int64, 'keys'),
                                  _dev(ptr, torch.int64, 'ptr'), _dev(tails, torch.int32, 'tails'), int(ent_row0),
                                  int(n_local), _dev(out, torch.int32, 'mask'), out.size(1), _stream(qkey)),
           'mgcn_filter_mask')
    return out


def smoothed_targets(lbl_smooth, num_entities):
    import numpy as np
    y = np.array([1.0, 0.0], dtype=np.float32)
    if lbl_smooth != 0.0:
        y = (1.0 - lbl_smooth) * y + (1.0 / int(num_entities))
    return float(y[0]), float(y[1])


def score_bce_supported(x, ent):
    return (x.size(0) % 4 == 0 and x.size(1) % 4 == 0 and x.is_contiguous() and ent.is_contiguous()
            and x.data_ptr() % 16 == 0 and ent.data_ptr() % 16 == 0)


def score_bce_fwd(x, ent, bias, mask, hot, cold, num_entities=None):
    B, n, O = _score_args(x, ent, bias)
    if mask.dim() != 2 or mask.size(0) != B or mask.size(1) < (n + 31) // 32 or not mask.is_contiguous():
        raise NativeError('score_bce_fwd: mask must be contiguous (%d, >= %d)' % (B, (n + 31) // 32))
    _same_device(x, ent, bias, mask)
    g = torch.empty((n, B), dtype=torch.float32, device=x.device)
    parts = torch.empty(int(lib().mgcn_score_bce_partials(B, n)), dtype=torch.float32, device=x.device)
    inv = 1.0 / (float(B) * float(n if num_entities is None else int(num_entities)))
    _check(lib().mgcn_score_bce_fwd(B, n, O, _dev(x, torch.float32, 'x'), _ld(x), _dev(ent, torch.float32, 'ent'), _ld(ent),
                                    _dev(bias, torch.float32, 'bias'), _dev(mask, torch.int32, 'mask'), mask.size(1),
                                    float(hot), float(cold), inv, _dev(g, torch.float32, 'grad_logit'), g.stride(0),
                                    _dev(parts, torch.float32, 'loss_partial'), _stream(x)), 'mgcn_score_bce_fwd')
    return parts.sum() * inv, g


def label_rows(qkey, keys, ptr, tails, n_local, lbl_smooth=0.0, num_entities=None, ent_row0=0, out=None):
    B = qkey.numel()
    y = smoothed_targets(lbl_smooth, int(n_local if num_entities is None else num_entities))
    if out is None:
        out = torch.empty((B, int(n_local)), dtype=torch.float32, device=qkey.device)
    if out.size(0) != B or out.size(1) < n_local or out.stride(1) != 1:
        raise NativeError('label_rows: out must be (%d, >= %d) with unit column stride' % (B, n_local))
    if ptr.numel() != keys.numel() + 1:
        raise NativeError('label_rows: ptr must have len(keys) + 1 entries')
    _same_device(qkey, keys, ptr, tails, out)
    _check(lib().mgcn_label_rows(B, _dev(qkey, torch.int64, 'qkey'), keys.numel(), _dev(keys, torch.int64, 'keys'),
                                 _dev(ptr, torch.int64, 'ptr'), _dev(tails, torch.int32, 'tails'), int(ent_row0),
                                 int(n_local), float(y[0]), float(y[1]), _dev(out, torch.float32, 'labels'),
                                 out.stride(0), _stream(qkey)), 'mgcn_label_rows')
    return out


ADAM_CHUNK = 8192
ADAM_BATCH = 64


def _ptr_array(tensors):
    return (_ptr * max(len(tensors), 1))(*[None if t is None else t.data_ptr() for t in tensors])


def _adam_list(what, lists):
    first = lists[0]
    for ts in lists:
        if len(ts) != len(first):
            raise NativeError('%s: the tensor lists differ in length' % what)
        for t, ref in zip(ts, first):
            if t is None:
                continue
            _dev(t, torch.float32, what)
            if not t.is_contiguous() or (ref is not None and t.numel() != ref.numel()):
                raise NativeError('%s: tensors must be contiguous with matching element counts' % what)
    _same_device(*[t for ts in lists for t in ts])


def adam_sq_norms(grads, out=None):
    _adam_list('adam_sq_norms', [grads])
    live = [g for g in grads if g is not None]
    if not live:
        raise NativeError('adam_sq_norms: no gradient to take the device from')
    dev, n = live[0].device, len(grads)
    numel = (_i64 * max(n, 1))(*[0 if g is None else g.numel() for g in grads])
    sq = torch.empty(n, dtype=torch.float32, device=dev) if out is None else out
    if sq.numel() != n or not sq.is_contiguous():
        raise NativeError('adam_sq_norms: out must be contiguous [%d]' % n)
    nbytes = lib().mgcn_adam_sq_norms_workspace(n, numel)
    ws = torch.empty(max(nbytes // 4, 1), dtype=torch.float32, device=dev)
    _check(lib().mgcn_adam_sq_norms(n, _ptr_array(grads), numel, _dev(sq, torch.float32, 'sq'), _dev(ws, torch.float32, 'ws'),
                                    nbytes, _stream(sq)), 'mgcn_adam_sq_norms')
    return sq


def adam_clip_coef(sq, max_norm, out=None):
    if out is None:
        out = torch.empty(2, dtype=torch.float32, device=sq.device)
    _same_device(sq, out)
    if not sq.is_contiguous() or out.numel() != 2 or not out.is_contiguous():
        raise NativeError('adam_clip_coef: sq must be contiguous and out [2]')
    _check(lib().mgcn_adam_clip_coef(sq.numel(), _dev(sq, torch.float32, 'sq'), float(max_norm), _dev(out, torch.float32, 'out'),
                                     _stream(sq)), 'mgcn_adam_clip_coef')
    return out


def adam_step(grads, params, exp_avgs, exp_avg_sqs, coef, step_size, bc2_sqrt, beta1, beta2, eps, weight_decay):
    _adam_list('adam_step', [params, grads, exp_avgs, exp_avg_sqs])
    _same_device(coef, *params)
    n = len(params)
    if n == 0:
        return
    numel = (_i64 * n)(*[p.numel() for p in params])
    _check(lib().mgcn_adam_step(n, _ptr_array(grads), _ptr_array(params), _ptr_array(exp_avgs), _ptr_array(exp_avg_sqs), numel,
                                _dev(coef, torch.float32, 'coef', True), float(step_size), float(bc2_sqrt), float(beta1),
                                float(beta2), float(eps), float(weight_decay), _stream(params[0])), 'mgcn_adam_step')


class IngestUnsupported(NativeError):
    """The native reader declined the files (non-ASCII names): use the Python reader."""


def ingest(train_path, valid_path, test_path):
    handle = _ptr()
    rc = lib().mgcn_ingest_open(os.fsencode(train_path), os.fsencode(valid_path), os.fsencode(test_path),
                                ctypes.byref(handle))
    if rc != 0:
        msg = (lib().mgcn_last_error() or b'').decode('utf-8', 'replace')
        if rc == 3:
            raise IngestUnsupported(msg)
        if 'KeyError' in msg:
            raise KeyError(msg.split("'")[1] if "'" in msg else msg)
        if 'ValueError' in msg:
            raise ValueError(msg)
        if 'cannot open' in msg:
            raise FileNotFoundError(msg)
        raise NativeError('mgcn_ingest_open failed (%d): %s' % (rc, msg))
    try:
        names = []
        for kind in (0, 1):
            n, nbytes = lib().mgcn_ingest_count(handle, kind), lib().mgcn_ingest_names_bytes(handle, kind)
            buf = ctypes.create_string_buffer(max(int(nbytes), 1))
            offs = torch.empty(n + 1, dtype=torch.int64)
            _check(lib().mgcn_ingest_names(handle, kind, ctypes.cast(buf, _ptr), offs.data_ptr()), 'mgcn_ingest_names')
            raw, o = buf.raw, offs.tolist()
            names.append([raw[o[i]:o[i + 1]].decode('ascii') for i in range(n)])
        ids = {}
        for k, split in enumerate(('train', 'valid', 'test')):
            t = torch.empty((int(lib().mgcn_ingest_count(handle, 2 + k)), 3), dtype=torch.int64)
            _check(lib().mgcn_ingest_triples(handle, k, t.data_ptr() if t.numel() else None), 'mgcn_ingest_triples')
            ids[split] = t
        return names[0], names[1], ids
    finally:
        lib().mgcn_ingest_close(handle)


def filter_index_build(triples, num_relations):
    t = triples.detach().to('cpu', torch.int64).contiguous().reshape(-1, 3)
    nk, nt = _i64(0), _i64(0)
    tp = t.data_ptr() if t.numel() else None
    _check(lib().mgcn_filter_index_build(t.size(0), tp, int(num_relations), None, None, None, ctypes.byref(nk),
                                         ctypes.byref(nt)), 'mgcn_filter_index_build')
    keys = torch.empty(nk.value, dtype=torch.int64)
    ptr = torch.empty(nk.value + 1, dtype=torch.int64)
    tails = torch.empty(nt.value, dtype=torch.int32)
    _check(lib().mgcn_filter_index_build(t.size(0), tp, int(num_relations), keys.data_ptr(), ptr.data_ptr(),
                                         tails.data_ptr() if nt.value else None, ctypes.byref(nk), ctypes.byref(nt)),
           'mgcn_filter_index_build')
    return keys, ptr, tails
```

kgc-gcn_amd/csrc/csr_build.cpp:

```cpp
#include <cmath>
#include <cstring>
#include <vector>

#include "mgcn_common.h"

namespace mgcn {
char *error_buffer() {
  static thread_local char buf[512] = {0};
  return buf;
}
}

extern "C" int mgcn_abi_version(void) { return MGCN_ABI_VERSION; }
extern "C" const char *mgcn_last_error(void) { return mgcn::error_buffer(); }

extern "C" int mgcn_csr_build_host(int64_t num_nodes, int64_t num_edges_half, int64_t num_rel_rows,
                                   const int64_t *edge_index_host, const int64_t *edge_type_host,
                                   int64_t hub_threshold, int64_t hub_chunk, int32_t *rowptr_host,
                                   mgcn_edge_rec *rec_host, int64_t *perm_host, int32_t *hubinfo_host,
                                   int32_t *chunks_host, int64_t max_chunks, int64_t *num_chunks_host,
                                   int32_t *slot_dst_host, int32_t *mirror_host, int32_t *typeptr_host,
                                   int32_t *typeslots_host) {
  const int64_t N = num_nodes, E = num_edges_half, E2 = 2 * num_edges_half;
  MGCN_REQUIRE(N >= 0 && E >= 0 && num_rel_rows >= 0, "csr_build: negative size");
  MGCN_REQUIRE(N < (int64_t(1) << 31) - 1 && E2 < (int64_t(1) << 31) - 1, "csr_build: sizes exceed int32 slots");
  MGCN_REQUIRE(rowptr_host && (E == 0 || (rec_host && perm_host)), "csr_build: null output");
  MGCN_REQUIRE(E == 0 || (edge_index_host && edge_type_host), "csr_build: null input");
  const bool hubs = hub_threshold > 0;
  MGCN_REQUIRE(!hubs || (hub_chunk > 0 && hubinfo_host && chunks_host && num_chunks_host),
               "csr_build: hub splitting needs hub_chunk > 0 and the hubinfo / chunks / num_chunks outputs");
  const bool bwd = typeptr_host != nullptr;
  MGCN_REQUIRE(E == 0 || (bwd == (slot_dst_host != nullptr) && bwd == (mirror_host != nullptr) &&
                          bwd == (typeslots_host != nullptr)),
               "csr_build: backward index outputs must be given all together or not at all");
  const int64_t *src = edge_index_host, *dst = edge_index_host + E2;
  for (int64_t e = 0; e < E2; ++e) {
    MGCN_REQUIRE(src[e] >= 0 && src[e] < N && dst[e] >= 0 && dst[e] < N,
                 "csr_build: edge %lld endpoint (%lld -> %lld) outside [0, %lld)", (long long)e,
                 (long long)src[e], (long long)dst[e], (long long)N);
    MGCN_REQUIRE(edge_type_host[e] >= 0 && edge_type_host[e] < num_rel_rows - 1,
                 "csr_build: edge %lld type %lld outside [0, %lld) (row %lld is the self-loop row)", (long long)e,
                 (long long)edge_type_host[e], (long long)(num_rel_rows - 1), (long long)(num_rel_rows - 1));
  }
  std::vector<int32_t> cnt(2 * N, 0);
  for (int h = 0; h < 2; ++h)
    for (int64_t e = h * E; e < (h + 1) * E; ++e) cnt[h * N + dst[e]]++;
  auto is_hub = [&](int h, int64_t n) { return hubs && cnt[h * N + n] > hub_threshold; };
  int64_t pos = 0;
  for (int h = 0; h < 2; ++h) {
    int32_t *rowptr = rowptr_host + h * (N + 1);
    for (int64_t n = 0; n < N; ++n) {
      rowptr[n] = int32_t(pos);
      if (!is_hub(h, n)) pos += cnt[h * N + n];
    }
    rowptr[N] = int32_t(pos);
  }
  std::vector<int32_t> cursor(2 * N);
  for (int h = 0; h < 2; ++h)
    for (int64_t n = 0; n < N; ++n) cursor[h * N + n] = rowptr_host[h * (N + 1) + n];
  int64_t nchunks = 0;
  if (hubinfo_host)
    for (int64_t i = 0; i < 4 * N; ++i) hubinfo_host[i] = (i & 1) ? 0 : -1;
  if (hubs) {
    for (int64_t n = 0; n < N; ++n)
      for (int h = 0; h < 2; ++h) {
        if (!is_hub(h, n)) continue;
        const int64_t len = cnt[h * N + n], nch = (len + hub_chunk - 1) / hub_chunk;
        MGCN_REQUIRE(nchunks + nch <= max_chunks, "csr_build: chunk table too small (%lld)", (long long)max_chunks);
        hubinfo_host[(h * N + n) * 2 + 0] = int32_t(nchunks);
        hubinfo_host[(h * N + n) * 2 + 1] = int32_t(nch);
        for (int64_t k = 0; k < nch; ++k) {
          int32_t *c = chunks_host + (nchunks + k) * 4;
          c[0] = int32_t(pos + k * hub_chunk);
          c[1] = int32_t(pos + (k + 1 < nch ? (k + 1) * hub_chunk : len));
          c[2] = int32_t(nchunks);
          c[3] = int32_t(nch);
        }
        nchunks += nch;
        cursor[h * N + n] = int32_t(pos);
        pos += len;
      }
  }
  if (num_chunks_host) *num_chunks_host = nchunks;
  std::vector<float> cinv(N);
  for (int h = 0; h < 2; ++h) {
    const int64_t lo = h * E;
    std::vector<int32_t> deg(N, 0);
    for (int64_t e = lo; e < lo + E; ++e) deg[src[e]]++;
    for (int64_t n = 0; n < N; ++n) cinv[n] = deg[n] ? 1.0f / std::sqrt(static_cast<float>(deg[n])) : 0.0f;
    for (int64_t e = lo; e < lo + E; ++e) {
      const int64_t slot = cursor[h * N + dst[e]]++;
      mgcn_edge_rec r;
      r.src = static_cast<int32_t>(src[e]);
      r.type = static_cast<int32_t>(edge_type_host[e]);
      r.norm = cinv[src[e]] * cinv[dst[e]];
      r.eid = static_cast<int32_t>(e);
      rec_host[slot] = r;
      perm_host[slot] = e;
      if (bwd) slot_dst_host[slot] = static_cast<int32_t>(dst[e]) | (h ? int32_t(0x80000000u) : 0);
    }
  }
  if (bwd) {
    bool mirrored = true;
    for (int64_t e = 0; e < E && mirrored; ++e) mirrored = src[e + E] == dst[e] && dst[e + E] == src[e];
    if (mirrored) {
      std::vector<int32_t> slot_of(E2);
      for (int64_t s = 0; s < E2; ++s) slot_of[perm_host[s]] = int32_t(s);
      for (int64_t s = 0; s < E2; ++s) mirror_host[s] = slot_of[(perm_host[s] + E) % E2];
    } else {
      for (int64_t s = 0; s < E2; ++s) mirror_host[s] = -1;
    }
    std::vector<int32_t> tcur(num_rel_rows + 1, 0);
    std::memset(typeptr_host, 0, sizeof(int32_t) * (num_rel_rows + 1));
    for (int64_t s = 0; s < E2; ++s) typeptr_host[rec_host[s].type + 1]++;
    for (int64_t t = 0; t < num_rel_rows; ++t) typeptr_host[t + 1] += typeptr_host[t];
    std::memcpy(tcur.data(), typeptr_host, sizeof(int32_t) * (num_rel_rows + 1));
    for (int64_t s = 0; s < E2; ++s) typeslots_host[tcur[rec_host[s].type]++] = static_cast<int32_t>(s);
  }
  return MGCN_OK;
}
```

kgc-gcn_amd/csrc/layer_fused.hip:

```cpp
#include <hip/hip_runtime.h>

#include <cstdlib>

#include "fused_common.h"


namespace {
bool lockstep_shape(int32_t dim_in, int32_t dim_out) { return dim_in <= 256 && mgcn::fused2_takes(dim_in, dim_out); }
int pack_generation(int32_t dim_in, int32_t dim_out) { return lockstep_shape(dim_in, dim_out) ? 2 : 3; }
bool generation_takes(int gen, int32_t dim_in, int32_t dim_out) {
  if (gen == 4) return mgcn::fused4_takes(dim_in, dim_out);
  if (gen == 2) return lockstep_shape(dim_in, dim_out);
  return gen == 3 && mgcn::fused3_takes(dim_in, dim_out);
}
}

extern "C" size_t mgcn_packed_weights_bytes_gen(int32_t generation, int32_t dim_in, int32_t dim_out) {
  const int gen = generation ? generation : pack_generation(dim_in, dim_out);
  if (gen == 4) return mgcn::fused4_packed_bytes(dim_in, dim_out);
  if (gen == 2) return mgcn::fused2_packed_bytes(dim_in, dim_out);
  return mgcn::fused3_packed_bytes(dim_in, dim_out);
}

extern "C" size_t mgcn_packed_weights_bytes(int32_t dim_in, int32_t dim_out) {
  return mgcn_packed_weights_bytes_gen(0, dim_in, dim_out);
}

extern "C" int mgcn_pack_weights_gen(int32_t generation, int32_t dim_in, int32_t dim_out, const float *w_dev, float *wp_dev,
                                     size_t wp_bytes, void *stream) {
  MGCN_REQUIRE(dim_in > 0 && dim_out > 0 && w_dev && wp_dev, "pack_weights: bad arguments");
  const int gen = generation ? generation : pack_generation(dim_in, dim_out);
  MGCN_REQUIRE(gen >= 2 && gen <= 4 && generation_takes(gen, dim_in, dim_out),
               "pack_weights: generation %d does not take D=%d O=%d", gen, dim_in, dim_out);
  MGCN_REQUIRE(wp_bytes >= mgcn_packed_weights_bytes_gen(gen, dim_in, dim_out) && mgcn::aligned16(wp_dev),
               "pack_weights: packed buffer too small or misaligned");
  if (gen == 4) return mgcn::fused4_pack(dim_in, dim_out, w_dev, wp_dev, stream);
  if (gen == 2) return mgcn::fused2_pack(dim_in, dim_out, w_dev, wp_dev, stream);
  return mgcn::fused3_pack(dim_in, dim_out, w_dev, wp_dev, stream);
}

extern "C" int mgcn_pack_weights(int32_t dim_in, int32_t dim_out, const float *w_dev, float *wp_dev, size_t wp_bytes,
                                 void *stream) {
  return mgcn_pack_weights_gen(0, dim_in, dim_out, w_dev, wp_dev, wp_bytes, stream);
}

extern "C" int mgcn_fused_kernel_generation(int32_t dim_in, int32_t dim_out, int64_t num_rows, int32_t with_row_bounds) {
  if (!lockstep_shape(dim_in, dim_out)) return 3;
  const bool few_tiles = (num_rows + 79) / 80 < 2 * int64_t(mgcn::cu_count());
  return (with_row_bounds && few_tiles && dim_out > 128) ? 3 : 2;
}

extern "C" int mgcn_layer_fwd_fused(int64_t num_nodes, int64_t num_edges_half, int32_t dim_in, int32_t dim_out,
                                    int32_t num_rel_rows, const int32_t *rowptr_dev, const mgcn_edge_rec *rec_dev,
                                    const float *x_dev, int64_t ldx, const float *rel_dev, const float *loop_rel_dev,
                                    const float *ee_dev, int32_t ee_in_slot_order, const float *loop_edge_dev,
                                    const float *wp_dev, const float *bias_dev, const float *bn_mean_dev,
                                    const float *bn_var_dev, const float *bn_gamma_dev, const float *bn_beta_dev,
                                    float bn_eps, float *out_dev, int64_t ldo, int64_t node_begin, int64_t node_end,
                                    int64_t ee_sub_in, int64_t ee_sub_out, int64_t ee_sub_hub,
                                    const int32_t *hubinfo_dev, const int32_t *chunks_dev, int64_t chunk_begin,
                                    int64_t chunk_end, float *partial_dev, const float *rels_weight_dev,
                                    float *rel_out_dev, const int32_t *row_bounds_dev, int32_t num_row_bounds,
                                    int32_t tune, uint32_t *status_dev, void *stream) {
  MGCN_REQUIRE(num_nodes >= 0 && num_edges_half >= 0 && dim_in > 0 && dim_out > 0 && num_rel_rows > 0,
               "layer_fwd_fused: bad sizes");
  MGCN_REQUIRE(node_begin >= 0 && node_begin <= node_end && node_end <= num_nodes, "layer_fwd_fused: bad node range");
  MGCN_REQUIRE(num_nodes < (int64_t(1) << 31) - 256 && 2 * num_edges_half < (int64_t(1) << 31) - 1,
               "layer_fwd_fused: sizes exceed int32");
  MGCN_REQUIRE(rowptr_dev && x_dev && loop_rel_dev && loop_edge_dev && wp_dev && bn_mean_dev && bn_var_dev &&
                   bn_gamma_dev && bn_beta_dev && (out_dev || node_end == node_begin) && (rel_dev || num_rel_rows == 1) &&
                   (num_edges_half == 0 || rec_dev), "layer_fwd_fused: null pointer");
  MGCN_REQUIRE(ldx >= dim_in && ldo >= dim_out, "layer_fwd_fused: ldx/ldo too small");
  const bool aligned = mgcn::aligned16(x_dev) && mgcn::aligned16(rel_dev) && mgcn::aligned16(loop_rel_dev) &&
                       mgcn::aligned16(loop_edge_dev) && (!ee_dev || mgcn::aligned16(ee_dev)) &&
                       mgcn::aligned16(out_dev) && mgcn::aligned16(wp_dev) && ldx % 4 == 0 && ldo % 4 == 0;
  if (!aligned || !mgcn::fused3_takes(dim_in, dim_out) || !ee_dev || !ee_in_slot_order || ldx >= (int64_t(1) << 31))
    return mgcn::fail(MGCN_EUNSUPPORTED, "layer_fwd_fused: needs 16-byte aligned operands, a per-edge table in slot order, "
                      "D %% 4 == 0, D <= 1024, O %% 4 == 0, O <= 512 (got D=%d O=%d)", dim_in, dim_out);
  const int64_t num_chunks = chunk_end - chunk_begin;
  MGCN_REQUIRE(chunk_begin >= 0 && num_chunks >= 0 && chunk_end < (int64_t(1) << 31) &&
                   (num_chunks == 0 || (hubinfo_dev && chunks_dev && partial_dev && mgcn::aligned16(partial_dev))),
               "layer_fwd_fused: hub chunks need hubinfo / chunks / a 16-byte aligned partial buffer");
  const bool want_rel = rel_out_dev != nullptr && num_rel_rows > 1;
  MGCN_REQUIRE(!want_rel || (rels_weight_dev && rel_dev), "layer_fwd_fused: the relation projection needs rels_weight and rel");
  if (node_end == node_begin && !want_rel) return MGCN_OK;
  if (num_chunks > 0 && node_end > node_begin) {
    if (int rc = mgcn::launch_hub_partials(num_nodes, dim_in, num_rel_rows, rec_dev, x_dev, ldx, rel_dev, loop_rel_dev,
                                           ee_dev, ee_in_slot_order, ee_sub_hub, chunks_dev, chunk_begin, chunk_end,
                                           partial_dev, stream))
      return rc;
  }
  const int forced = ((tune >> 10) & 3) == 1 ? 4 : ((tune >> 10) & 3);
  const int gen = forced == 0 ? mgcn_fused_kernel_generation(dim_in, dim_out, node_end - node_begin, num_row_bounds > 0) : forced;
  MGCN_REQUIRE(forced != 3 || !lockstep_shape(dim_in, dim_out) || dim_out > 128,
               "layer_fwd_fused: tune %d: generation 3 reads another packing than generation 2 for O <= 128", tune);
  MGCN_REQUIRE(generation_takes(gen, dim_in, dim_out), "layer_fwd_fused: tune %d: generation %d does not take D=%d O=%d", tune, gen,
               dim_in, dim_out);
  MGCN_REQUIRE(num_row_bounds >= 0 && num_row_bounds <= 4096 && (num_row_bounds == 0 || row_bounds_dev),
               "layer_fwd_fused: bad row bounds");
  const mgcn::FusedLaunch a = {num_nodes, dim_in, dim_out, num_rel_rows, rowptr_dev, rec_dev, x_dev, ldx, rel_dev, loop_rel_dev, ee_dev,
                               loop_edge_dev, wp_dev, bias_dev, bn_mean_dev, bn_var_dev, bn_gamma_dev, bn_beta_dev, bn_eps, out_dev, ldo,
                               node_begin, node_end, ee_sub_in, ee_sub_out, num_chunks > 0 ? hubinfo_dev : nullptr, chunk_begin,
                               partial_dev, want_rel ? rels_weight_dev : nullptr, want_rel ? rel_out_dev : nullptr, row_bounds_dev,
                               num_row_bounds, tune, status_dev, stream};
  if (gen == 4) return mgcn::fused4_launch(a);
  if (gen == 2) return mgcn::fused2_launch(a);
  return mgcn::fused3_launch(a);
}
```

kgc-gcn_amd/csrc/layer_fused2.hip:

```cpp
#include <hip/hip_runtime.h>

#include <cstdlib>
#include <type_traits>

#include "fused_common.h"

namespace {

constexpr int T2 = 1024;

struct Args2 : LayerArgs {
  int32_t nch, nkb_last, kbm, G;
  float bn_eps;
#ifdef MGCN_DIAG
  unsigned long long *stamps;
  int32_t ablate;
#endif
};
#ifdef MGCN_DIAG
#define MGCN_ABLATE(bit) (p.ablate & (bit))
#define MGCN_STAMP(role, idx)                                                                                      \
  do {                                                                                                             \
    if (p.stamps && lane == 0 && (idx) < 128) p.stamps[(int64_t(blockIdx.x) * 2 + (role)) * 128 + (idx)] = __builtin_readcyclecounter(); \
  } while (0)
#else
#define MGCN_ABLATE(bit) 0
#define MGCN_STAMP(role, idx) do {} while (0)
#endif

constexpr int EPI_FLOATS = 2 * 208;
constexpr int REL_LDS_MAX_BYTES = 32 * 1024;

template <int NT, int NRT, bool RELLDS, bool HUBS>
__global__ __launch_bounds__(T2, 4) void layer_fused2_kernel(Args2 p) {
  constexpr int BM = NRT * 16;
  constexpr int PIECE = 16 * BM * 16;
  constexpr int BUF = 3 * PIECE;
  constexpr int RPG = BM / 16;
  constexpr int UB = 4;
  constexpr int CH = 32 / UB * UB;
  extern __shared__ __attribute__((aligned(16))) unsigned char lds2[];
  float *epi = reinterpret_cast<float *>(lds2 + 2 * BUF);
  float *rel_lds = epi + EPI_FLOATS;

  const int bid = int(blockIdx.x), nblk = int(gridDim.x);
  const int tid = threadIdx.x;
  const int wave = __builtin_amdgcn_readfirstlane(tid >> 6), lane = tid & 63;
  const int nrows = p.node1 - p.node0;
  const int ntiles = (nrows + BM - 1) / BM;
  const int my_tiles = (ntiles - bid + nblk - 1) / nblk;
  const int nch = p.nch;

#ifdef MGCN_DIAG
  if (p.stamps && lane == 0 && (wave == 0 || wave == 8)) {
    p.stamps[(int64_t(blockIdx.x) * 2 + (wave ? 1 : 0)) * 128 + 120] = __builtin_readcyclecounter();
    p.stamps[(int64_t(blockIdx.x) * 2 + (wave ? 1 : 0)) * 128 + 121] = __builtin_amdgcn_s_memrealtime();
  }
#endif
  auto stage_barrier = [] () __attribute__((always_inline)) {
    asm volatile("s_waitcnt lgkmcnt(0)\n\ts_barrier" ::: "memory");
  };
  if (wave >= 8) {
    __builtin_amdgcn_s_setprio(3);
    const int gtid = tid - 512;
    const int grp = gtid >> 5, lig = gtid & 31;
    const int glane0 = lane & 32;
    const int g_lo = grp * RPG, g_hi = g_lo + RPG;
    const int qcol = lig >> 1, frot = (qcol >> 1) & 7;
    const int wbase = qcol * BM * 16 + (lig & 1) * 8;
    const uint32_t ldx32 = uint32_t(p.ldx), d32 = uint32_t(p.d);

    auto write_row = [&](unsigned char *img, int row, float4 v, bool ok) __attribute__((always_inline)) {
      uint32_t h[2], m[2], l[2];
      split3p(ok ? v.x : 0.f, ok ? v.y : 0.f, h[0], m[0], l[0]);
      split3p(ok ? v.z : 0.f, ok ? v.w : 0.f, h[1], m[1], l[1]);
      unsigned char *dst = img + wbase + ((row & ~15) + (((row & 15) + frot) & 15)) * 16;
      *reinterpret_cast<uint2 *>(dst) = make_uint2(h[0], h[1]);
      *reinterpret_cast<uint2 *>(dst + PIECE) = make_uint2(m[0], m[1]);
      *reinterpret_cast<uint2 *>(dst + 2 * PIECE) = make_uint2(l[0], l[1]);
    };
    auto rp_of = [&](int it_, int mode_) {
      return rp_load(p.rowptr + int64_t(mode_) * (p.n + 1), p.node0 + (bid + it_ * nblk) * BM, BM, p.node1, lig);
    };
    auto rp_get = [&](const RowPtrs &r, int idx) {
      const int from = glane0 + (idx & 31);
      const int va = __shfl(r.a, from), vb = __shfl(r.b, from), vc = __shfl(r.c, from);
      return idx < 32 ? va : (idx < 64 ? vb : vc);
    };
    struct Part { int lo, hi, rp; };
    auto partition = [&](const RowPtrs &r) {
      const int base = __shfl(r.a, glane0);
      const int tot = rp_get(r, BM) - base;
      const int c = 2 > (tot >> 8) + 1 ? 2 : (tot >> 8) + 1;
      const int ptot = tot + c * BM;
      const int thr_lo = (grp * ptot) >> 4, thr_hi = ((grp + 1) * ptot) >> 4;
      int lo = 0, hi = 0;
      const int vals[3] = {r.a, r.b, r.c};
#pragma unroll
      for (int k = 0; k < 3; ++k) {
        const int i = lig + 32 * k;
        const int pw = (vals[k] - base) + c * i;
        const unsigned long long blo = __ballot(i < BM && pw < thr_lo), bhi = __ballot(i < BM && pw < thr_hi);
        lo += __popc(uint32_t(blo >> glane0));
        hi += __popc(uint32_t(bhi >> glane0));
      }
      Part q;
      q.lo = lo; q.hi = hi;
      const int idx = lo + (lig < hi - lo ? lig : hi - lo);
      const int from = glane0 + (idx & 31);
      const int va = __shfl(r.a, from), vb = __shfl(r.b, from), vc = __shfl(r.c, from);
      q.rp = idx < 32 ? va : (idx < 64 ? vb : vc);
      return q;
    };
    auto rec_chunk = [&](int cbeg, int end) {
      int4 r = make_int4(0, 0, 0, 0);
      if (end > cbeg) r = p.rec[(cbeg + lig < end) ? cbeg + lig : end - 1];
      return r;
    };
    Part cur = partition(rp_of(0, 0));
    int4 currec = rec_chunk(__shfl(cur.rp, glane0), __shfl(cur.rp, glane0 + (cur.hi - cur.lo)));
    int stage = 0;
    for (int it = 0; it < my_tiles; ++it) {
      const int r0 = p.node0 + (bid + it * nblk) * BM;
      for (int mi = 0; mi < 3; ++mi) {
        const int mode = mi == 0 ? 2 : mi - 1;
        if (mode < 2) {
          const int myrp = cur.rp, e_lo = cur.lo, e_hi = cur.hi, e_n = cur.hi - cur.lo;
          const int4 firstrec = currec;
          const int ee_sub_mode = p.ee_sub[mode];
          const bool has_next = mode == 0 || it + 1 < my_tiles;
          RowPtrs nrp = {0, 0, 0};
          if (has_next) nrp = rp_of(mode == 0 ? it : it + 1, mode == 0 ? 1 : 0);
          Part nxt = {0, 0, 0};
          bool next_recs_issued = false;
          int4 nrec = make_int4(0, 0, 0, 0);
          auto prefetch_next = [&]() __attribute__((always_inline)) {
            if (has_next) {
              nxt = partition(nrp);
              nrec = rec_chunk(__shfl(nxt.rp, glane0), __shfl(nxt.rp, glane0 + (nxt.hi - nxt.lo)));
            }
          };
          int2 myhub = make_int2(-1, 0);
          {
            const int node = r0 + e_lo + lig;
            if (HUBS && p.hubinfo && lig < e_n && node < p.node1) myhub = p.hubinfo[int64_t(mode) * p.n + node];
          }
          const int beg = __shfl(myrp, glane0), end = MGCN_ABLATE(1) ? beg : __shfl(myrp, glane0 + e_n);
          for (int chunk = 0; chunk < nch; ++chunk, ++stage) {
            if (wave == 8) MGCN_STAMP(1, 2 * stage);
            unsigned char *img = lds2 + (stage & 1) * BUF;
            const int coff_ = chunk * 128 + lig * 4;
            const bool col_ok = coff_ < p.d;
            const int coff = col_ok ? coff_ : 0;
            const float *xb = p.x + coff, *relb = (RELLDS ? rel_lds : p.rel) + coff, *eeb = p.ee + coff;
            int4 myrec = firstrec;
            int row = e_lo, nb = __shfl(myrp, glane0 + 1);
            float4 sum = make_float4(0.f, 0.f, 0.f, 0.f);
            auto flush = [&]() __attribute__((always_inline)) {
              if (HUBS && p.hubinfo) {
                const int first = __shfl(myhub.x, glane0 + (row - e_lo)), cnt = __shfl(myhub.y, glane0 + (row - e_lo));
                if (cnt > 0) {
                  const float4 ps = *reinterpret_cast<const float4 *>(p.partial + int64_t(first - p.chunk0) * p.d + coff);
                  sum = make_float4(sum.x + ps.x, sum.y + ps.y, sum.z + ps.z, sum.w + ps.w);
                }
              }
              write_row(img, row, sum, col_ok);
              sum = make_float4(0.f, 0.f, 0.f, 0.f);
              ++row;
            };
            int cbase = beg;
#ifdef MGCN_DIAG
            int bstamp = 64;
            if (wave == 8 && stage == 1) { MGCN_STAMP(1, 63); }
#endif
            for (int s = beg; s < end; s += UB) {
              if (s >= cbase + CH) {
                cbase += CH;
                myrec = rec_chunk(cbase, end);
              }
              int rsrc[UB], rtyp[UB], rnrm[UB];
#pragma unroll
              for (int u = 0; u < UB; ++u) {
                const int from = glane0 + (((s + u < end) ? s + u : end - 1) - cbase);
                rsrc[u] = __shfl(myrec.x, from);
                rtyp[u] = __shfl(myrec.y, from);
                rnrm[u] = __shfl(myrec.z, from);
              }
              float4 xv[UB], rv[UB], ev[UB];
#pragma unroll
              for (int u = 0; u < UB; ++u) {
                if (MGCN_ABLATE(16)) rsrc[u] = 0;
                xv[u] = *reinterpret_cast<const float4 *>(xb + uint64_t(uint32_t(rsrc[u])) * ldx32);
                if (!RELLDS) rv[u] = *reinterpret_cast<const float4 *>(relb + uint64_t(uint32_t(rtyp[u])) * d32);
                const uint32_t erow = MGCN_ABLATE(16) ? 0u : uint32_t(((s + u < end) ? s + u : end - 1) - ee_sub_mode);
                ev[u] = *reinterpret_cast<const float4 *>(eeb + uint64_t(erow) * d32);
              }
#ifdef MGCN_DIAG
              if (wave == 8 && stage == 1 && bstamp < 126) { MGCN_STAMP(1, bstamp); ++bstamp; }
#endif
              if (!next_recs_issued) {
                next_recs_issued = true;
                prefetch_next();
              }
#ifdef MGCN_DIAG
              if (wave == 8 && stage == 1 && bstamp < 126) {
                asm volatile("s_waitcnt vmcnt(0)" ::: "memory");
                MGCN_STAMP(1, bstamp); ++bstamp;
              }
#endif
#pragma unroll
              for (int u = 0; u < UB; ++u) {
                if (s + u < end) {
                  while (s + u >= nb) {
                    flush();
                    nb = __shfl(myrp, glane0 + (row - e_lo) + 1);
                  }
                  const float4 rr = RELLDS ? *reinterpret_cast<const float4 *>(relb + uint32_t(rtyp[u]) * d32) : rv[u];
                  const float4 m = f4mul(f4mul(xv[u], rr), ev[u]);
                  const float wgt = __int_as_float(rnrm[u]);
                  sum = make_float4(sum.x + m.x * wgt, sum.y + m.y * wgt, sum.z + m.z * wgt, sum.w + m.w * wgt);
                }
              }
            }
            if (!next_recs_issued) {
              next_recs_issued = true;
              prefetch_next();
            }
#ifdef MGCN_DIAG
            if (wave == 8 && stage == 1 && bstamp < 126) { MGCN_STAMP(1, bstamp); ++bstamp; }
#endif
            while (row < e_hi) flush();
            if (wave == 8) MGCN_STAMP(1, 2 * stage + 1);
            stage_barrier();
          }
          cur = nxt;
          currec = nrec;
        } else {
          for (int chunk = 0; chunk < nch; ++chunk, ++stage) {
            if (wave == 8) MGCN_STAMP(1, 2 * stage);
            unsigned char *img = lds2 + (stage & 1) * BUF;
            const int coff_ = chunk * 128 + lig * 4;
            const bool col_ok = coff_ < p.d;
            const int coff = col_ok ? coff_ : 0;
            const float4 lr = *reinterpret_cast<const float4 *>(p.loop_rel + coff);
            const float4 le = *reinterpret_cast<const float4 *>(p.loop_edge + coff);
            float4 xs[RPG];
#pragma unroll
            for (int i = 0; i < RPG; ++i) {
              const int node = (r0 + g_lo + i < p.node1) ? r0 + g_lo + i : p.node1 - 1;
              xs[i] = *reinterpret_cast<const float4 *>(p.x + int64_t(node) * p.ldx + coff);
            }
#pragma unroll
            for (int i = 0; i < RPG; ++i) write_row(img, g_lo + i, f4mul(f4mul(xs[i], lr), le), col_ok);
            if (wave == 8) MGCN_STAMP(1, 2 * stage + 1);
            stage_barrier();
          }
        }
      }
    }
    if (p.rel_out) rel_projection(p, wave, 8, 8, lane, bid, nblk);
#ifdef MGCN_DIAG
    if (p.stamps && lane == 0 && wave == 8) {
      p.stamps[(int64_t(blockIdx.x) * 2 + 1) * 128 + 122] = __builtin_readcyclecounter();
      p.stamps[(int64_t(blockIdx.x) * 2 + 1) * 128 + 123] = __builtin_amdgcn_s_memrealtime();
    }
#endif
  } else {
    auto multiply = [&](auto Hc) __attribute__((always_inline)) {
    constexpr int H = decltype(Hc)::value;
    constexpr int QALL = NT / 4, R = NT % 4;
    constexpr int QA = (QALL + 1) / 2;
    constexpr int Q = H == 0 ? QA : QALL - QA;
    constexpr int QF = Q > 0 ? Q : 1;
    constexpr int NX = H == 1 ? R * NRT : 0;
    constexpr int XE = (NX + 3) / 4;
    constexpr int XF = XE > 0 ? XE : 1;
    constexpr int XW = (R == 1) ? 1 : XF;
    const int w = wave & 3;
    const int r = lane & 15, gq = lane >> 4;
    const int ct0 = w * QALL + (H == 0 ? 0 : QA);
    int xct[XF], xrt[XF];
    bool xok[XF];
#pragma unroll
    for (int j = 0; j < XF; ++j) {
      const int e = 4 * j + w;
      xok[j] = XE > 0 && e < NX;
      xct[j] = xok[j] ? 4 * QALL + e / NRT : 0;
      xrt[j] = xok[j] ? e % NRT : -1;
    }
    const int G = p.G;
    auto wload = [&](u32x4 (&wq)[QF][3], u32x4 (&wx)[XW][3], int g) {
      if (MGCN_ABLATE(8)) g = 0;
      if (MGCN_ABLATE(64) && g != 0) return;
      const u32x4 *base = p.wp + (int64_t(g) * NT) * 3 * 64 + lane;
#pragma unroll
      for (int t = 0; t < Q; ++t) {
#pragma unroll
        for (int pc = 0; pc < 3; ++pc) wq[t][pc] = base[((ct0 + t) * 3 + pc) * 64];
      }
      if (XE > 0) {
#pragma unroll
        for (int j = 0; j < XW; ++j) {
#pragma unroll
          for (int pc = 0; pc < 3; ++pc) wx[j][pc] = base[(xct[j] * 3 + pc) * 64];
        }
      }
    };
    u32x4 wq0[QF][3], wx0[XW][3], wq1[QF][3], wx1[XW][3], wq2[QF][3], wx2[XW][3];

    f32x4 acc[NRT][QF], accx[XF];
    auto zero_acc = [&]() {
#pragma unroll
      for (int rt = 0; rt < NRT; ++rt) {
#pragma unroll
        for (int t = 0; t < QF; ++t) acc[rt][t] = f32x4{0.f, 0.f, 0.f, 0.f};
      }
#pragma unroll
      for (int j = 0; j < XF; ++j) accx[j] = f32x4{0.f, 0.f, 0.f, 0.f};
    };
    auto store_unit = [&](f32x4 a, int prow, int col, const float4 &sc, const float4 &sh) {
      if (prow < nrows) {
        const float4 v = make_float4(tanh_fast(fmaf(a[0], sc.x, sh.x)), tanh_fast(fmaf(a[1], sc.y, sh.y)),
                                     tanh_fast(fmaf(a[2], sc.z, sh.z)), tanh_fast(fmaf(a[3], sc.w, sh.w)));
        *reinterpret_cast<float4 *>(p.out + int64_t(prow) * p.ldo + col) = v;
      }
    };
    auto epilogue = [&](int tile) {
      const int prow0 = tile * BM + r;
      auto column_tile = [&](int ct, auto &&body) {
        const int col = ct * 16 + 4 * gq;
        if (col < p.o) body(col, *reinterpret_cast<const float4 *>(epi + col), *reinterpret_cast<const float4 *>(epi + 208 + col));
      };
#pragma unroll
      for (int t = 0; t < Q; ++t) {
        column_tile(ct0 + t, [&](int col, const float4 &sc, const float4 &sh) {
#pragma unroll
          for (int rt = 0; rt < NRT; ++rt) store_unit(acc[rt][t], prow0 + rt * 16, col, sc, sh);
        });
      }
      if (XE > 0) {
#pragma unroll
        for (int j = 0; j < XF; ++j) {
          if (xok[j])
            column_tile(xct[j], [&](int col, const float4 &sc, const float4 &sh) { store_unit(accx[j], prow0 + xrt[j] * 16, col, sc, sh); });
        }
      }
    };

    auto rotated = [&](int kb_, int) { return kb_; };
    int kb = 0, chunk = 0, stage = 0;
    bool barrier_done = false;
    int nkb_ = 0, nchunk = 0, nmode = 0;
    auto advance_next = [&]() {
      const int n = (nchunk == nch - 1) ? p.nkb_last : 4;
      if (++nkb_ == n) {
        nkb_ = 0;
        if (++nchunk == nch) {
          nchunk = 0;
          nmode = nmode == 2 ? 0 : nmode + 1;
        }
      }
    };
    auto gindex = [&]() {
      const int mode_ = nmode == 0 ? 2 : nmode - 1;
      return mode_ * p.kbm + 4 * nchunk + rotated(nkb_, nchunk);
    };
    wload(wq0, wx0, gindex());
    advance_next();
    if (H == 0) {
      const int t8 = (wave & 3) * 64 + lane;
      if (t8 < 208) epilogue_table_entry(p, p.bn_eps, epi, 208, t8);
    }
    if (RELLDS) copy_rel_table(p, rel_lds, wave, lane, 8);
    auto kblock = [&](u32x4 (&wq)[QF][3], u32x4 (&wx)[XW][3], u32x4 (&nq)[QF][3], u32x4 (&nx)[XW][3]) {
      wload(nq, nx, gindex());
      advance_next();
      const int nkb_c = (chunk == nch - 1) ? p.nkb_last : 4;
      if (kb == 0) {
        if (!barrier_done) stage_barrier();
        barrier_done = false;
        if (wave == 0) MGCN_STAMP(0, 2 * stage);
      }
      const int qc = 4 * rotated(kb, chunk) + gq;
      const unsigned char *ap = lds2 + (stage & 1) * BUF + (qc * BM + ((r + ((qc >> 1) & 7)) & 15)) * 16;
      constexpr int WP[6] = {0, 2, 1, 0, 1, 0}, AP[6] = {2, 0, 1, 1, 0, 0};
#pragma unroll
      for (int rt = 0; rt < NRT; ++rt) {
        if (Q > 0 && !MGCN_ABLATE(2)) {
          bf16x8 a[3];
#pragma unroll
          for (int pc = 0; pc < 3; ++pc)
            a[pc] = __builtin_bit_cast(bf16x8, MGCN_ABLATE(32) ? wq[0][pc] : *reinterpret_cast<const u32x4 *>(ap + pc * PIECE + rt * 256));
#pragma unroll
          for (int pr = 0; pr < 6; ++pr) {
#pragma unroll
            for (int t = 0; t < Q; ++t)
              acc[rt][t] = __builtin_amdgcn_mfma_f32_16x16x32_bf16(__builtin_bit_cast(bf16x8, wq[t][WP[pr]]), a[AP[pr]],
                                                                   acc[rt][t], 0, 0, 0);
          }
        }
      }
      if (XE > 0) {
#pragma unroll
        for (int j = 0; j < XF; ++j) {
          if (xok[j]) {
            bf16x8 a[3];
#pragma unroll
            for (int pc = 0; pc < 3; ++pc)
              a[pc] = __builtin_bit_cast(bf16x8, MGCN_ABLATE(32) ? wx[0][pc] : *reinterpret_cast<const u32x4 *>(ap + pc * PIECE + xrt[j] * 256));
#pragma unroll
            for (int pr = 0; pr < 6; ++pr)
              accx[j] = __builtin_amdgcn_mfma_f32_16x16x32_bf16(__builtin_bit_cast(bf16x8, wx[XW == 1 ? 0 : j][WP[pr]]),
                                                                a[AP[pr]], accx[j], 0, 0, 0);
          }
        }
      }
      if (++kb == nkb_c) {
        if (wave == 0) MGCN_STAMP(0, 2 * stage + 1);
        if (stage < 8) MGCN_STAMP(0, 32 + 8 * stage + wave);
        kb = 0;
        ++stage;
        if (++chunk == nch) chunk = 0;
      }
    };
    for (int it = 0; it < my_tiles; ++it) {
      zero_acc();
      for (int g0 = 0; g0 < G; g0 += 3) {
        kblock(wq0, wx0, wq1, wx1);
        kblock(wq1, wx1, wq2, wx2);
        kblock(wq2, wx2, wq0, wx0);
      }
      if (it + 1 < my_tiles) {
        stage_barrier();
        barrier_done = true;
      }
      if (wave == 0) MGCN_STAMP(0, 100 + 2 * it);
      if (!MGCN_ABLATE(4)) epilogue(bid + it * nblk);
      if (wave == 0) MGCN_STAMP(0, 101 + 2 * it);
    }
#ifdef MGCN_DIAG
    if (p.stamps && lane == 0 && wave == 0) {
      p.stamps[int64_t(blockIdx.x) * 2 * 128 + 122] = __builtin_readcyclecounter();
      p.stamps[int64_t(blockIdx.x) * 2 * 128 + 123] = __builtin_amdgcn_s_memrealtime();
    }
#endif
    };
    if (wave < 4) multiply(std::integral_constant<int, 0>{});
    else multiply(std::integral_constant<int, 1>{});
  }
}

template <int NT, int NRT, bool RELLDS, bool HUBS>
int launch2(const Args2 &p, int grid, hipStream_t st) {
  constexpr size_t lds_bytes = size_t(2) * 3 * 16 * (NRT * 16) * 16 + EPI_FLOATS * 4 + (RELLDS ? REL_LDS_MAX_BYTES : 0);
  if (hipFuncSetAttribute(reinterpret_cast<const void *>(&layer_fused2_kernel<NT, NRT, RELLDS, HUBS>),
                          hipFuncAttributeMaxDynamicSharedMemorySize, int(lds_bytes)) != hipSuccess)
    return mgcn::fail(MGCN_ELAUNCH, "layer_fused2: cannot reserve %zu bytes of LDS", lds_bytes);
  hipLaunchKernelGGL((layer_fused2_kernel<NT, NRT, RELLDS, HUBS>), dim3(unsigned(grid)), dim3(T2), lds_bytes, st, p);
  MGCN_CHECK_LAUNCH("layer_fused2_kernel");
  return MGCN_OK;
}

int pick_nt2(int o) { return o <= 32 ? 2 : o <= 64 ? 4 : o <= 128 ? 8 : 13; }

struct Shape2 {
  int nch, nkb_last, kbm, G;
};
Shape2 shape2(int d) {
  Shape2 s;
  s.nch = (d + 127) / 128;
  const int wlast = d - 128 * (s.nch - 1);
  s.nkb_last = (wlast + 31) / 32;
  s.kbm = 4 * (s.nch - 1) + s.nkb_last;
  s.G = 3 * s.kbm;
  return s;
}

#ifdef MGCN_DIAG
unsigned long long *diag_stamps() {
  static unsigned long long *buf = nullptr;
  if (!buf && getenv("MGCN_FUSED_STAMPS")) {
    if (hipMalloc(&buf, 1024 * 2 * 128 * 8) != hipSuccess) buf = nullptr;
    else (void)hipMemset(buf, 0, 1024 * 2 * 128 * 8);
  }
  return buf;
}
#endif

}

#ifdef MGCN_DIAG
extern "C" int mgcn_diag_read_stamps(unsigned long long *host_out) {
  unsigned long long *b = diag_stamps();
  if (!b) return 1;
  return hipMemcpy(host_out, b, 1024 * 2 * 128 * 8, hipMemcpyDeviceToHost) == hipSuccess ? 0 : 2;
}
#endif

namespace mgcn {

bool fused2_takes(int32_t dim_in, int32_t dim_out) {
  return dim_in > 0 && dim_in % 4 == 0 && dim_in <= 1024 && dim_out > 0 && dim_out % 4 == 0 && dim_out <= 208;
}

size_t fused2_packed_bytes(int32_t dim_in, int32_t dim_out) { return pack_modes_bytes(dim_in, pick_nt2(dim_out)); }

int fused2_pack(int32_t dim_in, int32_t dim_out, const float *w_dev, void *wp_dev, void *stream) {
  const int kbm = pack_modes_kbm(dim_in);
  return pack_launch(wp_dev, 3 * kbm, pick_nt2(dim_out), ModeWeights{w_dev, dim_in, dim_out, kbm}, stream);
}

int fused2_launch(const FusedLaunch &a) {
  const int32_t dim_in = a.dim_in, dim_out = a.dim_out;
  const Shape2 s = shape2(dim_in);
  Args2 p = {};
  fill_layer_args(p, a);
  p.nch = s.nch; p.nkb_last = s.nkb_last; p.kbm = s.kbm; p.G = s.G;
  p.bn_eps = a.bn_eps;
#ifdef MGCN_DIAG
  if (const char *ab = getenv("MGCN_FUSED_ABLATE")) p.ablate = atoi(ab);
  p.stamps = diag_stamps();
#endif
  const int cus = cu_count();
  const int64_t nrows = a.node_end - a.node_begin;
  auto grid_for = [&](int rt) { const int64_t t = (nrows + rt * 16 - 1) / (rt * 16); return int(t < cus ? (t > 0 ? t : 1) : cus); };
  auto makespan = [&](int bm) { return ((nrows + bm - 1) / bm + cus - 1) / cus * bm; };
  int nrt = makespan(64) < makespan(80) ? 4 : 5;
#ifdef MGCN_DIAG
  if (const char *e = getenv("MGCN_FUSED_NRT")) nrt = atoi(e) == 4 ? 4 : 5;
#endif
  const int grid = grid_for(nrt);
  hipStream_t st = static_cast<hipStream_t>(a.stream);
  const bool rel_lds = a.rel && size_t(a.num_rel_rows - 1) * dim_in * 4 <= size_t(REL_LDS_MAX_BYTES);
  const bool hubs = a.hubinfo != nullptr;
  switch (pick_nt2(dim_out)) {
    case 2: return launch2<2, 5, false, true>(p, grid_for(5), st);
    case 4: return launch2<4, 5, false, true>(p, grid_for(5), st);
    case 8: return launch2<8, 5, false, true>(p, grid_for(5), st);
    default:
      if (nrt == 4) {
        if (rel_lds) return hubs ? launch2<13, 4, true, true>(p, grid, st) : launch2<13, 4, true, false>(p, grid, st);
        return hubs ? launch2<13, 4, false, true>(p, grid, st) : launch2<13, 4, false, false>(p, grid, st);
      }
      if (rel_lds) return hubs ? launch2<13, 5, true, true>(p, grid, st) : launch2<13, 5, true, false>(p, grid, st);
      return hubs ? launch2<13, 5, false, true>(p, grid, st) : launch2<13, 5, false, false>(p, grid, st);
  }
}

}
```

kgc-gcn_amd/csrc/layer_fused3.hip:

```cpp
#include <hip/hip_runtime.h>

#include <type_traits>

#include "fused_common.h"

namespace {

constexpr int T3 = 1024;
constexpr int SPIN_LIMIT = 1 << 22;

struct Args3 : LayerArgs {
  int32_t npass, nkb_last, kbp, kbm, G;
  int32_t ncc;
  int32_t rows_per_wg, nimg;
  uint32_t *status;
  const int32_t *bounds;
  float bn_eps;
#ifdef MGCN_DIAG
  unsigned long long *diag;
#endif
};
#ifdef MGCN_DIAG
#define DIAG_NOW() __builtin_readcyclecounter()
#define DIAG_LAP(acc) do { const unsigned long long t_ = DIAG_NOW(); acc += t_ - t_last; t_last = t_; } while (0)
#else
#define DIAG_NOW() 0ull
#define DIAG_LAP(acc) do {} while (0)
#endif

__device__ __forceinline__ void wait_ge_(const uint32_t *c, uint32_t need, uint32_t *status) {
  int spins = 0;
#pragma nounroll
  for (; spins < SPIN_LIMIT; ++spins) {
    const uint32_t v = __builtin_amdgcn_readfirstlane(__hip_atomic_load(c, __ATOMIC_RELAXED, __HIP_MEMORY_SCOPE_WORKGROUP));
    if (v >= need) break;
    __builtin_amdgcn_s_sleep(1);
  }
  if (spins == SPIN_LIMIT && status) __hip_atomic_fetch_or(status, 1u, __ATOMIC_RELAXED, __HIP_MEMORY_SCOPE_AGENT);
  asm volatile("" ::: "memory");
}
__device__ __forceinline__ void signal_add(uint32_t *c, int lane) {
  asm volatile("" ::: "memory");
  if (lane == 0) __hip_atomic_fetch_add(c, 1u, __ATOMIC_RELAXED, __HIP_MEMORY_SCOPE_WORKGROUP);
  asm volatile("" ::: "memory");
}

template <int NT, int NRT, int NCH, bool RELLDS>
__global__ __launch_bounds__(T3, 4) void layer_fused3_kernel(Args3 p) {
  constexpr int BM = NRT * 16;
  constexpr int UB = 4 / NCH;
  constexpr int CH = 32;
  constexpr int OP = NT * 16;
  extern __shared__ __attribute__((aligned(16))) unsigned char lds3[];
  const int piece = p.ncc * BM * 16;
  const int rowb = p.ncc * 32;
  const int sbuf = BM * rowb;
  unsigned char *stg0 = lds3 + 3 * piece;
  uint32_t *cnt = reinterpret_cast<uint32_t *>(stg0 + p.nimg * sbuf);
  float *epi = reinterpret_cast<float *>(cnt + 16);
  float *rel_lds = epi + 2 * OP;

  const int bid = int(blockIdx.x), nblk = int(gridDim.x);
  const int tid = threadIdx.x;
  const int wave = __builtin_amdgcn_readfirstlane(tid >> 6), lane = tid & 63;
  const int nimg = p.nimg;
  int row_lo = p.node0 + bid * p.rows_per_wg;
  int row_hi = row_lo + p.rows_per_wg < p.node1 ? row_lo + p.rows_per_wg : p.node1;
  if (p.bounds) {
    row_lo = p.node0 + p.bounds[bid];
    row_hi = p.node0 + p.bounds[bid + 1];
    row_hi = row_hi < p.node1 ? row_hi : p.node1;
  }
  const int myrows = row_hi > row_lo ? row_hi - row_lo : 0;
  const int my_tiles = (myrows + BM - 1) / BM;
  const int npass = p.npass;

  if (tid < 16) cnt[tid] = 0;
  __syncthreads();
#ifdef MGCN_DIAG
  const unsigned long long t_begin = DIAG_NOW();
  unsigned long long t_wait = 0, n_wait = 0, t_load = 0, n_load = 0, t_last = t_begin, t_a = 0, t_b = 0, t_d = 0, t_o = 0;
  auto wait_ge = [&](const uint32_t *c, uint32_t need) __attribute__((always_inline)) {
    const unsigned long long t0 = DIAG_NOW();
    wait_ge_(c, need, p.status);
    t_wait += DIAG_NOW() - t0;
    ++n_wait;
  };
  auto diag_end = [&]() __attribute__((always_inline)) {
    if (p.diag && lane == 0) {
      unsigned long long *d = p.diag + (int64_t(bid) * 16 + wave) * 8;
      d[0] = DIAG_NOW() - t_begin; d[1] = t_wait; d[2] = t_load; d[3] = n_load; d[4] = t_a; d[5] = t_b; d[6] = t_d; d[7] = t_o;
    }
  };
#else
  auto wait_ge = [&](const uint32_t *c, uint32_t need) __attribute__((always_inline)) { wait_ge_(c, need, p.status); };
  auto diag_end = [] () {};
#endif

  if (wave >= 8) {
    __builtin_amdgcn_s_setprio(3);
    const int gtid = tid - 512;
    const int grp = gtid >> 5, lig = gtid & 31;
    const int glane0 = lane & 32;
    const int qcol = lig >> 1;
    const uint32_t ldx32 = uint32_t(p.ldx), d32 = uint32_t(p.d);
    bool wr[NCH];
#pragma unroll
    for (int j = 0; j < NCH; ++j) wr[j] = 16 * j + qcol < p.ncc;

    auto write_row = [&](unsigned char *stg, int row, const float4 (&v)[NCH], const bool (&ok)[NCH]) __attribute__((always_inline)) {
      unsigned char *dst = stg + row * rowb + lig * 16;
#pragma unroll
      for (int j = 0; j < NCH; ++j) {
        if (wr[j]) *reinterpret_cast<float4 *>(dst + j * 512) = ok[j] ? v[j] : make_float4(0.f, 0.f, 0.f, 0.f);
      }
    };
    int s_img = 0;
    uint32_t s_round = 0;
    auto acquire = [&]() __attribute__((always_inline)) {
      if (s_round > 0) {
        __builtin_amdgcn_s_setprio(0);
        wait_ge(cnt + 4 + s_img, 8u * s_round);
        __builtin_amdgcn_s_setprio(3);
      }
      return stg0 + s_img * sbuf;
    };
    auto publish = [&]() __attribute__((always_inline)) {
      signal_add(cnt + s_img, lane);
      if (++s_img == nimg) { s_img = 0; ++s_round; }
    };
    auto tile_rows16 = [&](int it_) {
      const int left = myrows - it_ * BM;
      const int r = left < BM ? left : BM;
      return (r + 15) & ~15;
    };
    auto rp_of = [&](int it_, int mode_) {
      return rp_load(p.rowptr + int64_t(mode_) * (p.n + 1), row_lo + it_ * BM, BM, row_hi, lig);
    };
    auto rp_get = [&](const RowPtrs &r, int idx) {
      const int from = glane0 + (idx & 31);
      const int va = __shfl(r.a, from), vb = __shfl(r.b, from), vc = __shfl(r.c, from);
      return idx < 32 ? va : (idx < 64 ? vb : vc);
    };
    struct Part { int lo, hi, rp; };
    auto partition = [&](const RowPtrs &r, int nr) {
      const int base = __shfl(r.a, glane0);
      const int tot = rp_get(r, nr) - base;
      const int c = 2 > (tot >> 8) + 1 ? 2 : (tot >> 8) + 1;
      const int ptot = tot + c * nr;
      const int thr_lo = (grp * ptot) >> 4, thr_hi = ((grp + 1) * ptot) >> 4;
      int lo = 0, hi = 0;
      const int vals[3] = {r.a, r.b, r.c};
#pragma unroll
      for (int k = 0; k < 3; ++k) {
        const int i = lig + 32 * k;
        const int pw = (vals[k] - base) + c * i;
        const unsigned long long blo = __ballot(i < nr && pw < thr_lo), bhi = __ballot(i < nr && pw < thr_hi);
        lo += __popc(uint32_t(blo >> glane0));
        hi += __popc(uint32_t(bhi >> glane0));
      }
      Part q;
      q.lo = lo; q.hi = hi;
      const int idx = lo + (lig < hi - lo ? lig : hi - lo);
      const int from = glane0 + (idx & 31);
      const int va = __shfl(r.a, from), vb = __shfl(r.b, from), vc = __shfl(r.c, from);
      q.rp = idx < 32 ? va : (idx < 64 ? vb : vc);
      return q;
    };
    auto rec_chunk = [&](int cbeg, int end) {
      int4 r = make_int4(0, 0, 0, 0);
      if (end > cbeg) r = p.rec[(cbeg + lig < end) ? cbeg + lig : end - 1];
      return r;
    };
    Part cur = {0, 0, 0};
    int4 currec = make_int4(0, 0, 0, 0);
    if (my_tiles > 0) {
      cur = partition(rp_of(0, 0), tile_rows16(0));
      currec = rec_chunk(__shfl(cur.rp, glane0), __shfl(cur.rp, glane0 + (cur.hi - cur.lo)));
    }
    bool tables_ready = !RELLDS;
    for (int it = 0; it < my_tiles; ++it) {
      const int r0 = row_lo + it * BM;
      const int nr = tile_rows16(it);
      for (int mi = 0; mi < 3; ++mi) {
        const int mode = mi == 0 ? 2 : mi - 1;
        if (mode < 2) {
          if (!tables_ready) {
            wait_ge(cnt + 8, 8u);
            tables_ready = true;
          }
          const int myrp = cur.rp, e_lo = cur.lo, e_hi = cur.hi, e_n = cur.hi - cur.lo;
          const int4 firstrec = currec;
          const int ee_sub_mode = p.ee_sub[mode];
          const bool has_next = mode == 0 || it + 1 < my_tiles;
          RowPtrs nrp = {0, 0, 0};
          if (has_next) nrp = rp_of(mode == 0 ? it : it + 1, mode == 0 ? 1 : 0);
          const int nnr = mode == 0 ? nr : (it + 1 < my_tiles ? tile_rows16(it + 1) : 16);
          Part nxt = {0, 0, 0};
          bool next_recs_issued = false;
          int4 nrec = make_int4(0, 0, 0, 0);
          auto prefetch_next = [&]() __attribute__((always_inline)) {
            if (has_next) {
              nxt = partition(nrp, nnr);
              nrec = rec_chunk(__shfl(nxt.rp, glane0), __shfl(nxt.rp, glane0 + (nxt.hi - nxt.lo)));
            }
          };
          int2 myhub = make_int2(-1, 0);
          {
            const int node = r0 + e_lo + lig;
            if (p.hubinfo && lig < e_n && node < row_hi) myhub = p.hubinfo[int64_t(mode) * p.n + node];
          }
          const int beg = __shfl(myrp, glane0), end = __shfl(myrp, glane0 + e_n);
          for (int pass = 0; pass < npass; ++pass) {
            unsigned char *img = acquire();
            bool col_ok[NCH];
            int coff[NCH];
#pragma unroll
            for (int j = 0; j < NCH; ++j) {
              const int c_ = pass * (128 * NCH) + j * 128 + lig * 4;
              col_ok[j] = c_ < p.d;
              coff[j] = col_ok[j] ? c_ : 0;
            }
            const float *relbase = RELLDS ? rel_lds : p.rel;
            int4 myrec = firstrec;
            int row = e_lo, nb = __shfl(myrp, glane0 + 1);
            float4 sum[NCH];
#pragma unroll
            for (int j = 0; j < NCH; ++j) sum[j] = make_float4(0.f, 0.f, 0.f, 0.f);
            auto flush = [&]() __attribute__((always_inline)) {
              if (p.hubinfo) {
                const int first = __shfl(myhub.x, glane0 + (row - e_lo)), hcnt = __shfl(myhub.y, glane0 + (row - e_lo));
                if (hcnt > 0) {
#pragma unroll
                  for (int j = 0; j < NCH; ++j) {
                    const float4 ps = *reinterpret_cast<const float4 *>(p.partial + int64_t(first - p.chunk0) * p.d + coff[j]);
                    sum[j] = make_float4(sum[j].x + ps.x, sum[j].y + ps.y, sum[j].z + ps.z, sum[j].w + ps.w);
                  }
                }
              }
              write_row(img, row, sum, col_ok);
#pragma unroll
              for (int j = 0; j < NCH; ++j) sum[j] = make_float4(0.f, 0.f, 0.f, 0.f);
              ++row;
            };
            int cbase = beg;
            for (int s = beg; s < end; s += UB) {
              DIAG_LAP(t_o);
              if (s >= cbase + CH) {
                cbase += CH;
                myrec = rec_chunk(cbase, end);
              }
              int rsrc[UB], rtyp[UB], rnrm[UB];
#pragma unroll
              for (int u = 0; u < UB; ++u) {
                const int from = glane0 + (((s + u < end) ? s + u : end - 1) - cbase);
                rsrc[u] = __shfl(myrec.x, from);
                rtyp[u] = __shfl(myrec.y, from);
                rnrm[u] = __shfl(myrec.z, from);
              }
              float4 xv[UB][NCH], rv[UB][NCH], ev[UB][NCH];
#pragma unroll
              for (int u = 0; u < UB; ++u) {
                const uint32_t erow = uint32_t(((s + u < end) ? s + u : end - 1) - ee_sub_mode);
#pragma unroll
                for (int j = 0; j < NCH; ++j) {
                  xv[u][j] = *reinterpret_cast<const float4 *>(p.x + coff[j] + uint64_t(uint32_t(rsrc[u])) * ldx32);
                  if (!RELLDS) rv[u][j] = *reinterpret_cast<const float4 *>(p.rel + coff[j] + uint64_t(uint32_t(rtyp[u])) * d32);
                  ev[u][j] = *reinterpret_cast<const float4 *>(p.ee + coff[j] + uint64_t(erow) * d32);
                }
              }
              DIAG_LAP(t_a);
              if (!next_recs_issued) {
                next_recs_issued = true;
                prefetch_next();
              }
              DIAG_LAP(t_b);
#ifdef MGCN_DIAG
              asm volatile("s_waitcnt vmcnt(0)" ::: "memory");
              ++n_load;
#endif
              DIAG_LAP(t_load);
#pragma unroll
              for (int u = 0; u < UB; ++u) {
                if (s + u < end) {
                  while (s + u >= nb) {
                    flush();
                    nb = __shfl(myrp, glane0 + (row - e_lo) + 1);
                  }
                  const float wgt = __int_as_float(rnrm[u]);
#pragma unroll
                  for (int j = 0; j < NCH; ++j) {
                    const float4 rr = RELLDS ? *reinterpret_cast<const float4 *>(relbase + coff[j] + uint32_t(rtyp[u]) * d32) : rv[u][j];
                    sum[j] = f4axpy(sum[j], f4mul(f4mul(xv[u][j], rr), ev[u][j]), wgt);
                  }
                }
              }
              DIAG_LAP(t_d);
            }
            if (!next_recs_issued) {
              next_recs_issued = true;
              prefetch_next();
            }
            while (row < e_hi) flush();
            publish();
          }
          cur = nxt;
          currec = nrec;
        } else {
          for (int pass = 0; pass < npass; ++pass) {
            unsigned char *img = acquire();
            bool col_ok[NCH];
            int coff[NCH];
            float4 lr[NCH], le[NCH];
#pragma unroll
            for (int j = 0; j < NCH; ++j) {
              const int c_ = pass * (128 * NCH) + j * 128 + lig * 4;
              col_ok[j] = c_ < p.d;
              coff[j] = col_ok[j] ? c_ : 0;
              lr[j] = *reinterpret_cast<const float4 *>(p.loop_rel + coff[j]);
              le[j] = *reinterpret_cast<const float4 *>(p.loop_edge + coff[j]);
            }
            const int g_lo = grp * NRT;
            float4 xs[NRT][NCH];
#pragma unroll
            for (int i = 0; i < NRT; ++i) {
              const int node = (r0 + g_lo + i < row_hi) ? r0 + g_lo + i : row_hi - 1;
#pragma unroll
              for (int j = 0; j < NCH; ++j) xs[i][j] = *reinterpret_cast<const float4 *>(p.x + int64_t(node) * p.ldx + coff[j]);
            }
#pragma unroll
            for (int i = 0; i < NRT; ++i) {
              if (g_lo + i < nr) {
                float4 v[NCH];
#pragma unroll
                for (int j = 0; j < NCH; ++j) v[j] = f4mul(f4mul(xs[i][j], lr[j]), le[j]);
                write_row(img, g_lo + i, v, col_ok);
              }
            }
            publish();
          }
        }
      }
    }
    if (p.rel_out) rel_projection(p, wave, 8, 8, lane, bid, nblk);
    diag_end();
  } else {
    auto multiply = [&](auto Hc) __attribute__((always_inline)) {
    constexpr int H = decltype(Hc)::value;
    static_assert(NT == 13 || NT == 32, "13 column tiles (O <= 208) or 32 (O <= 512)");
    constexpr int E = NT == 13 ? 2 : 4;
    constexpr bool UNITS = NT == 13 && H == 1;
    constexpr int XF = (NRT + 3) / 4;
    const int w = wave & 3;
    const int r = lane & 15, gq = lane >> 4;
    auto ct_of = [&](int e) { return NT == 13 ? (e == 0 ? 3 * w + 2 * H : (H == 0 ? 3 * w + 1 : 12)) : 8 * w + 4 * H + e; };
    int xrt[XF];
#pragma unroll
    for (int j = 0; j < XF; ++j) xrt[j] = (UNITS && 4 * j + w < NRT) ? 4 * j + w : NRT;
    auto wload = [&](u32x4 (&wv)[3], int g, int ct) __attribute__((always_inline)) {
      const u32x4 *base = p.wp + ((int64_t(g) * NT + ct) * 3) * 64 + lane;
#pragma unroll
      for (int pc = 0; pc < 3; ++pc) wv[pc] = base[pc * 64];
    };
    u32x4 wn[3][3];
    f32x4 acc[E][NRT];
    auto zero_acc = [&]() {
#pragma unroll
      for (int e = 0; e < E; ++e) {
#pragma unroll
        for (int rt = 0; rt < NRT; ++rt) acc[e][rt] = f32x4{0.f, 0.f, 0.f, 0.f};
      }
    };
    auto store_unit = [&](f32x4 a, int node, int col, const float4 &sc, const float4 &sh) {
      if (node < row_hi) {
        const float4 v = make_float4(tanh_fast(fmaf(a[0], sc.x, sh.x)), tanh_fast(fmaf(a[1], sc.y, sh.y)),
                                     tanh_fast(fmaf(a[2], sc.z, sh.z)), tanh_fast(fmaf(a[3], sc.w, sh.w)));
        *reinterpret_cast<float4 *>(p.out + int64_t(node - p.node0) * p.ldo + col) = v;
      }
    };
    auto epilogue = [&](int it_) {
      const int node0_ = row_lo + it_ * BM + r;
#pragma unroll
      for (int e = 0; e < E; ++e) {
        const int col = ct_of(e) * 16 + 4 * gq;
        if (col < p.o) {
          const float4 sc = *reinterpret_cast<const float4 *>(epi + col), sh = *reinterpret_cast<const float4 *>(epi + OP + col);
          if (UNITS && e == E - 1) {
#pragma unroll
            for (int j = 0; j < XF; ++j) {
              if (xrt[j] < NRT) store_unit(acc[e][j], node0_ + xrt[j] * 16, col, sc, sh);
            }
          } else {
#pragma unroll
            for (int rt = 0; rt < NRT; ++rt) store_unit(acc[e][rt], node0_ + rt * 16, col, sc, sh);
          }
        }
      }
    };

    int kb = 0, pass = 0;
    int nkb_ = 0, npass_ = 0, nmode = 0;
    auto advance_next = [&]() {
      const int n = (npass_ == npass - 1) ? p.nkb_last : p.kbp;
      if (++nkb_ == n) {
        nkb_ = 0;
        if (++npass_ == npass) {
          npass_ = 0;
          nmode = nmode == 2 ? 0 : nmode + 1;
        }
      }
    };
    auto gindex = [&]() {
      const int mode_ = nmode == 0 ? 2 : nmode - 1;
      return mode_ * p.kbm + p.kbp * npass_ + nkb_;
    };
    int gcur = gindex();
    wload(wn[0], gcur, ct_of(0));
    advance_next();
    if (H == 0) {
      for (int c = (wave & 3) * 64 + lane; c < OP; c += 256) epilogue_table_entry(p, p.bn_eps, epi, OP, c);
    }
    if (RELLDS) copy_rel_table(p, rel_lds, wave, lane, 8);
    signal_add(cnt + 8, lane);
    int m_img = 0;
    uint32_t m_round = 0, m_stage = 0;
    int nrt_eff = NRT;
    auto six = [&](f32x4 &accv, const u32x4 (&wv)[3], const bf16x8 (&a)[3]) __attribute__((always_inline)) {
      constexpr int WP[6] = {0, 2, 1, 0, 1, 0}, AP[6] = {2, 0, 1, 1, 0, 0};
#pragma unroll
      for (int pr = 0; pr < 6; ++pr)
        accv = __builtin_amdgcn_mfma_f32_16x16x32_bf16(__builtin_bit_cast(bf16x8, wv[WP[pr]]), a[AP[pr]], accv, 0, 0, 0);
    };
    auto frag = [&](bf16x8 (&a)[3], const unsigned char *ap, int rt) __attribute__((always_inline)) {
#pragma unroll
      for (int pc = 0; pc < 3; ++pc) a[pc] = __builtin_bit_cast(bf16x8, *reinterpret_cast<const u32x4 *>(ap + pc * piece + rt * 256));
    };
    auto tile_entry = [&](f32x4 (&accv)[NRT], const u32x4 (&wv)[3], const unsigned char *ap) __attribute__((always_inline)) {
      if (nrt_eff == NRT) {
        bf16x8 a[2][3];
        frag(a[0], ap, 0);
#pragma unroll
        for (int rt = 0; rt < NRT; ++rt) {
          if (rt + 1 < NRT) frag(a[(rt + 1) & 1], ap, rt + 1);
          asm volatile("" ::: "memory");
          six(accv[rt], wv, a[rt & 1]);
        }
      } else {
#pragma unroll
        for (int rt = 0; rt < NRT; ++rt) {
          if (rt < nrt_eff) {
            bf16x8 a[3];
            frag(a, ap, rt);
            six(accv[rt], wv, a);
          }
        }
      }
    };
    auto unit_entry = [&](f32x4 (&accv)[NRT], const u32x4 (&wv)[3], const unsigned char *ap) __attribute__((always_inline)) {
#pragma unroll
      for (int j = 0; j < XF; ++j) {
        if (xrt[j] < nrt_eff) {
          bf16x8 a[3];
          frag(a, ap, xrt[j]);
          six(accv[j], wv, a);
        }
      }
    };
    auto kblock = [&](auto Kc) __attribute__((always_inline)) {
      constexpr int K = decltype(Kc)::value;
      wload(wn[(K * E + 1) % 3], gcur, ct_of(1));
      const int nkb_c = (pass == npass - 1) ? p.nkb_last : p.kbp;
      if (kb == 0) {
        DIAG_LAP(t_o);
        wait_ge(cnt + m_img, 8u * (m_round + 1));
        if (m_stage > 0) wait_ge(cnt + 10, 8u * m_stage);
        const unsigned char *stg = stg0 + m_img * sbuf;
        constexpr int RPI = NCH == 1 ? 16 : 8;
        const int ql = NCH == 1 ? (lane & 31) : lane;
        const int crow0 = NCH == 1 ? 2 * wave + (lane >> 5) : wave;
        const bool qok = ql < 2 * p.ncc;
        const int cc = ql >> 1;
        const int coff = cc * BM * 16 + (ql & 1) * 8;
        const int crot = (cc >> 1) & 7;
        auto convert_row = [&](int row, const float4 &v) __attribute__((always_inline)) {
          uint32_t h[2], m[2], l[2];
          split3p(v.x, v.y, h[0], m[0], l[0]);
          split3p(v.z, v.w, h[1], m[1], l[1]);
          unsigned char *dst = lds3 + coff + ((row & ~15) + (((row & 15) + crot) & 15)) * 16;
          *reinterpret_cast<uint2 *>(dst) = make_uint2(h[0], h[1]);
          *reinterpret_cast<uint2 *>(dst + piece) = make_uint2(m[0], m[1]);
          *reinterpret_cast<uint2 *>(dst + 2 * piece) = make_uint2(l[0], l[1]);
        };
        if (qok) {
          const unsigned char *src = stg + ql * 16;
          const int rows = nrt_eff * 16;
          int row = crow0;
          for (; row + RPI < rows; row += 2 * RPI) {
            const float4 v0 = *reinterpret_cast<const float4 *>(src + row * rowb);
            const float4 v1 = *reinterpret_cast<const float4 *>(src + (row + RPI) * rowb);
            convert_row(row, v0);
            convert_row(row + RPI, v1);
          }
          for (; row < rows; row += RPI) convert_row(row, *reinterpret_cast<const float4 *>(src + row * rowb));
        }
        signal_add(cnt + 4 + m_img, lane);
        signal_add(cnt + 9, lane);
        DIAG_LAP(t_a);
        wait_ge(cnt + 9, 8u * (m_stage + 1));
        DIAG_LAP(t_b);
      }
      int qc = 4 * kb + gq;
      qc = qc < p.ncc ? qc : p.ncc - 1;
      const unsigned char *ap = lds3 + (qc * BM + ((r + ((qc >> 1) & 7)) & 15)) * 16;
#pragma unroll
      for (int e = 0; e < E; ++e) {
        if (e > 0) {
          if (e + 1 < E) {
            wload(wn[(K * E + e + 1) % 3], gcur, ct_of(e + 1));
          } else {
            gcur = gindex();
            wload(wn[(K * E + E) % 3], gcur, ct_of(0));
            advance_next();
          }
        }
        if (NT == 13 || ct_of(e) * 16 < p.o) {
          if (UNITS && e == E - 1) unit_entry(acc[e], wn[(K * E + e) % 3], ap);
          else tile_entry(acc[e], wn[(K * E + e) % 3], ap);
        }
      }
      if (++kb == nkb_c) {
        DIAG_LAP(t_d);
        signal_add(cnt + 10, lane);
        ++m_stage;
        if (++m_img == nimg) { m_img = 0; ++m_round; }
        kb = 0;
        if (++pass == npass) pass = 0;
      }
    };
    wait_ge(cnt + 8, 8u);
    for (int it = 0; it < my_tiles; ++it) {
      zero_acc();
      {
        const int left = myrows - it * BM;
        nrt_eff = left < BM ? (left + 15) >> 4 : NRT;
      }
      for (int g0 = 0; g0 < p.G; g0 += 3) {
        kblock(std::integral_constant<int, 0>{});
        kblock(std::integral_constant<int, 1>{});
        kblock(std::integral_constant<int, 2>{});
      }
      epilogue(it);
    }
    diag_end();
    };
    if (wave < 4) multiply(std::integral_constant<int, 0>{});
    else multiply(std::integral_constant<int, 1>{});
  }
}

int pick_nt3(int o) { return o <= 208 ? 13 : 32; }

struct Shape3 {
  int nch, npass, nkb_last, kbp, kbm, G, ncc;
};
Shape3 shape3(int d, int nch = 0) {
  Shape3 s;
  s.nch = nch ? nch : 1;
  const int wpass = 128 * s.nch;
  s.npass = (d + wpass - 1) / wpass;
  const int wlast = d - wpass * (s.npass - 1);
  s.nkb_last = (wlast + 31) / 32;
  s.kbp = 4 * s.nch;
  s.kbm = s.kbp * (s.npass - 1) + s.nkb_last;
  s.G = 3 * s.kbm;
  const int w0 = d < wpass ? d : wpass;
  s.ncc = (w0 + 7) / 8;
  return s;
}

constexpr size_t LDS_MAX = size_t(160) * 1024;

#ifdef MGCN_DIAG
unsigned long long *diag_buf3() {
  static unsigned long long *buf = nullptr;
  if (!buf) {
    if (hipMalloc(&buf, 1024 * 16 * 8 * 8) != hipSuccess) buf = nullptr;
    else (void)hipMemset(buf, 0, 1024 * 16 * 8 * 8);
  }
  return buf;
}
#endif

size_t lds_bytes3(const Shape3 &s, int nrt, int nimg, int nt, size_t rel_bytes) {
  return size_t(3) * s.ncc * (nrt * 16) * 16 + size_t(nimg) * (nrt * 16) * s.ncc * 32 + 64 + size_t(2) * nt * 16 * 4 + rel_bytes;
}

template <int NT, int NRT, int NCH, bool RELLDS>
int launch3(const Args3 &p, int grid, size_t lds, hipStream_t st) {
  if (hipFuncSetAttribute(reinterpret_cast<const void *>(&layer_fused3_kernel<NT, NRT, NCH, RELLDS>),
                          hipFuncAttributeMaxDynamicSharedMemorySize, int(LDS_MAX)) != hipSuccess)
    return mgcn::fail(MGCN_ELAUNCH, "layer_fused3: cannot reserve %zu bytes of LDS", LDS_MAX);
  hipLaunchKernelGGL((layer_fused3_kernel<NT, NRT, NCH, RELLDS>), dim3(unsigned(grid)), dim3(T3), lds, st, p);
  MGCN_CHECK_LAUNCH("layer_fused3_kernel");
  return MGCN_OK;
}

template <int NT, int NRT, int NCH>
int launch3_rel(const Args3 &p, int grid, size_t lds, bool rel_lds, hipStream_t st) {
  if (rel_lds) return launch3<NT, NRT, NCH, true>(p, grid, lds, st);
  return launch3<NT, NRT, NCH, false>(p, grid, lds, st);
}

template <int NT, int NCH>
int launch3_nrt(const Args3 &p, int nrt, int grid, size_t lds, bool rel_lds, hipStream_t st) {
  if (nrt == 3) return launch3_rel<NT, 3, NCH>(p, grid, lds, rel_lds, st);
  if (nrt == 4) return launch3_rel<NT, 4, NCH>(p, grid, lds, rel_lds, st);
  return launch3_rel<NT, 5, NCH>(p, grid, lds, rel_lds, st);
}

}

#ifdef MGCN_DIAG
extern "C" int mgcn_diag_fused3(unsigned long long *host_out) {
  unsigned long long *b = diag_buf3();
  if (!b) return 1;
  return hipMemcpy(host_out, b, 1024 * 16 * 8 * 8, hipMemcpyDeviceToHost) == hipSuccess ? 0 : 2;
}
#endif

namespace mgcn {

bool fused3_takes(int32_t dim_in, int32_t dim_out) {
  return dim_in > 0 && dim_in % 4 == 0 && dim_in <= 1024 && dim_out > 0 && dim_out % 4 == 0 && dim_out <= 512;
}

size_t fused3_packed_bytes(int32_t dim_in, int32_t dim_out) { return pack_modes_bytes(dim_in, pick_nt3(dim_out)); }

int fused3_pack(int32_t dim_in, int32_t dim_out, const float *w_dev, void *wp_dev, void *stream) {
  const int kbm = pack_modes_kbm(dim_in);
  return pack_launch(wp_dev, 3 * kbm, pick_nt3(dim_out), ModeWeights{w_dev, dim_in, dim_out, kbm}, stream);
}

int fused3_launch(const FusedLaunch &a) {
  const int32_t dim_in = a.dim_in, dim_out = a.dim_out, tune = a.tune;
  const int t_nch = (tune >> 12) & 3;
  if (t_nch > 2) return mgcn::fail(MGCN_EINVAL, "layer_fwd_fused: bad tune %d", tune);
  const Shape3 s = shape3(dim_in, t_nch);
  Args3 p = {};
  fill_layer_args(p, a);
  p.npass = s.npass; p.nkb_last = s.nkb_last; p.kbp = s.kbp; p.kbm = s.kbm; p.G = s.G; p.ncc = s.ncc;
  p.bn_eps = a.bn_eps;
  p.status = a.status;
  const int cus = cu_count();
  const int64_t nrows = a.node_end - a.node_begin;
  int64_t rpw = ((nrows + cus - 1) / cus + 15) / 16 * 16;
  if (rpw < 16) rpw = 16;
  int grid = int(nrows > 0 ? (nrows + rpw - 1) / rpw : 1);
  p.rows_per_wg = int32_t(rpw);
  if (a.row_bounds && a.num_row_bounds > 0 && nrows > 0) {
    p.bounds = a.row_bounds;
    grid = a.num_row_bounds;
    const int64_t per = (nrows + grid - 1) / grid;
    rpw = per <= 80 ? (per + 15) / 16 * 16 : (per + 79) / 80 * 80;
  }
  const int nt = pick_nt3(dim_out);
  const size_t rel_bytes = a.rel ? size_t(a.num_rel_rows - 1) * dim_in * 4 : 0;
  const int t_nrt = tune & 15, t_img = (tune >> 4) & 15, t_rel = (tune >> 8) & 3;
  int nrt = 0, nimg = 0;
  bool rel_lds = false;
  const int nrt_cap = nt == 32 ? 3 : rpw >= 80 ? 5 : rpw >= 64 ? 4 : 3;
  auto fits = [&](int a, int b, bool r) { return lds_bytes3(s, a, b, nt, r ? rel_bytes : 0) <= LDS_MAX; };
  const bool rel_wanted = rel_bytes > 0 && rel_bytes <= size_t(32) * 1024 && t_rel != 1;
  if (t_nrt || t_img || t_nch) {
    nrt = t_nrt ? (t_nrt < nrt_cap ? t_nrt : nrt_cap) : nrt_cap;
    nimg = t_img ? t_img : 2;
    rel_lds = rel_wanted && fits(nrt, nimg, true);
    if (nrt < 3 || nrt > nrt_cap || nimg < 1 || nimg > 4 || !fits(nrt, nimg, rel_lds))
      return mgcn::fail(MGCN_EINVAL, "layer_fwd_fused: tune %d does not fit the LDS", tune);
  } else {
    for (int want_rel = rel_wanted ? 1 : 0; want_rel >= 0 && !nrt; --want_rel) {
      for (int a = nrt_cap; a >= 3 && !nrt; --a) {
        for (int b = 3; b >= 2 && !nrt; --b) {
          if (fits(a, b, want_rel != 0)) { nrt = a; nimg = b; rel_lds = want_rel != 0; }
        }
      }
    }
    if (!nrt && fits(3, 1, false)) { nrt = 3; nimg = 1; }
    if (!nrt) return mgcn::fail(MGCN_EUNSUPPORTED, "layer_fwd_fused: no tile geometry fits the LDS (D=%d O=%d)", dim_in, dim_out);
  }
  p.nimg = nimg;
#ifdef MGCN_DIAG
  p.diag = diag_buf3();
#endif
  const size_t lds = lds_bytes3(s, nrt, nimg, nt, rel_lds ? rel_bytes : 0);
  hipStream_t st = static_cast<hipStream_t>(a.stream);
  if (nt == 32) {
    if (s.nch == 1) return launch3_rel<32, 3, 1>(p, grid, lds, rel_lds, st);
    return launch3_rel<32, 3, 2>(p, grid, lds, rel_lds, st);
  }
  if (s.nch == 1) return launch3_nrt<13, 1>(p, nrt, grid, lds, rel_lds, st);
  return launch3_nrt<13, 2>(p, nrt, grid, lds, rel_lds, st);
}

}
```

kgc-gcn_amd/csrc/mgcn_common.h:

```cpp
#pragma once
#include <cstdarg>
#include <cstdio>

#include "../../include/mgcn_hip.h"

namespace mgcn {

char *error_buffer();

inline int fail(int code, const char *fmt, ...) {
  va_list ap;
  va_start(ap, fmt);
  vsnprintf(error_buffer(), 512, fmt, ap);
  va_end(ap);
  return code;
}

#define MGCN_REQUIRE(cond, ...)                          \
  do {                                                   \
    if (!(cond)) return mgcn::fail(MGCN_EINVAL, __VA_ARGS__); \
  } while (0)

#define MGCN_CHECK_LAUNCH(name)                                                            \
  do {                                                                                     \
    hipError_t e_ = hipGetLastError();                                                     \
    if (e_ != hipSuccess) return mgcn::fail(MGCN_ELAUNCH, "%s: %s", name, hipGetErrorString(e_)); \
  } while (0)

int launch_hub_partials(int64_t num_nodes, int32_t dim, int32_t num_rel_rows, const mgcn_edge_rec *rec_dev,
                        const float *x_dev, int64_t ldx, const float *rel_dev, const float *loop_rel_dev,
                        const float *ee_dev, int32_t ee_in_slot_order, int64_t ee_sub_hub, const int32_t *chunks_dev,
                        int64_t chunk_begin, int64_t chunk_end, float *partial_dev, void *stream);

struct FusedLaunch {
  int64_t num_nodes;
  int32_t dim_in, dim_out, num_rel_rows;
  const int32_t *rowptr;
  const mgcn_edge_rec *rec;
  const float *x;
  int64_t ldx;
  const float *rel, *loop_rel, *ee, *loop_edge;
  const void *wp;
  const float *bias, *bn_mean, *bn_var, *bn_gamma, *bn_beta;
  float bn_eps;
  float *out;
  int64_t ldo;
  int64_t node_begin, node_end, ee_sub_in, ee_sub_out;
  const int32_t *hubinfo;
  int64_t chunk_begin;
  const float *partial;
  const float *rels_weight;
  float *rel_out;
  const int32_t *row_bounds;
  int32_t num_row_bounds;
  int32_t tune;
  uint32_t *status;
  void *stream;
};

bool fused2_takes(int32_t dim_in, int32_t dim_out);
size_t fused2_packed_bytes(int32_t dim_in, int32_t dim_out);
int fused2_pack(int32_t dim_in, int32_t dim_out, const float *w_dev, void *wp_dev, void *stream);
int fused2_launch(const FusedLaunch &a);

bool fused3_takes(int32_t dim_in, int32_t dim_out);
size_t fused3_packed_bytes(int32_t dim_in, int32_t dim_out);
int fused3_pack(int32_t dim_in, int32_t dim_out, const float *w_dev, void *wp_dev, void *stream);
int fused3_launch(const FusedLaunch &a);

bool fused4_takes(int32_t dim_in, int32_t dim_out);
size_t fused4_packed_bytes(int32_t dim_in, int32_t dim_out);
int fused4_pack(int32_t dim_in, int32_t dim_out, const float *w_dev, void *wp_dev, void *stream);
int fused4_launch(const FusedLaunch &a);

inline bool aligned16(const void *p) { return (reinterpret_cast<uintptr_t>(p) & 15u) == 0; }

}
```

kgc-gcn_amd/graph.py:

```python
import torch

from . import _native


class GraphCSR(object):

    _FIELDS = ('rowptr', 'rec', 'perm', 'hubinfo', 'chunks', 'slot_dst', 'mirror', 'typeptr', 'typeslots')

    def __init__(self, num_nodes, num_rel_rows, edge_index, edge_type, device, with_backward=True, hub_threshold=None,
                 hub_chunk=None):
        host = _native.csr_build_host(num_nodes, num_rel_rows, edge_index, edge_type, with_backward, hub_threshold,
                                      hub_chunk)
        self.num_chunks = host['num_chunks']
        self.num_nodes = int(num_nodes)
        self.num_edges_half = int(edge_index.size(1)) // 2
        self.num_rel_rows = int(num_rel_rows)
        self.has_backward = with_backward
        self.mirrored = bool(with_backward and (host['mirror'].numel() == 0 or int(host['mirror'][0]) >= 0))
        for k in self._FIELDS:
            setattr(self, k, host[k].to(device) if k in host else None)
        self._inv_perm = None
        if self.num_chunks:
            per_node = host['hubinfo'][:, :, 1].sum(0, dtype=torch.int64)
            self._chunkptr = torch.cat([per_node.new_zeros(1), per_node.cumsum(0)]).tolist()
            self._chunk_slot0 = host['chunks'][:self.num_chunks, 0].tolist() + [2 * self.num_edges_half]
        else:
            self._chunkptr, self._chunk_slot0 = None, None

    @property
    def device(self):
        return self.rowptr.device

    def to(self, device):
        for k in self._FIELDS:
            v = getattr(self, k)
            if v is not None:
                setattr(self, k, v.to(device))
        self._inv_perm = None
        self.__dict__.pop('_shard_cache', None)
        self.__dict__.pop('_hub_partials', None)
        return self

    @property
    def inv_perm(self):
        if self._inv_perm is None:
            inv = torch.empty_like(self.perm)
            inv[self.perm] = torch.arange(self.perm.numel(), device=self.perm.device)
            self._inv_perm = inv
        return self._inv_perm

    def _shard_bounds(self, n0, n1):
        key = (int(n0), int(n1))
        cache = self.__dict__.setdefault('_shard_cache', {})
        if key not in cache:
            rp = self.rowptr[:, [key[0], key[1]]].cpu().tolist()
            c0, c1 = self.chunk_range(*key)
            hub = (self._chunk_slot0[c0], self._chunk_slot0[c1]) if self.num_chunks else (0, 0)
            cache[key] = ((rp[0][0], rp[0][1]), (rp[1][0], rp[1][1]), hub)
        return cache[key]

    def chunk_range(self, n0, n1):
        if not self.num_chunks:
            return 0, 0
        return self._chunkptr[int(n0)], self._chunkptr[int(n1)]

    def balanced_bounds(self, world, node_weight=1.0, align=32):
        N, W = self.num_nodes, int(world)
        key = ('balanced', W, float(node_weight), int(align))
        cache = self.__dict__.setdefault('_shard_cache', {})
        if key not in cache:
            rp = self.rowptr.cpu().to(torch.int64)
            work = (rp[0, 1:] - rp[0, :-1]) + (rp[1, 1:] - rp[1, :-1])
            if self.num_chunks:
                ch = self.chunks.cpu().to(torch.int64)
                hub = self.hubinfo.cpu().to(torch.int64)
                first, cnt = hub[:, :, 0], hub[:, :, 1]
                has = cnt > 0
                beg = ch[first.clamp(min=0), 0]
                end = ch[(first + cnt - 1).clamp(min=0), 1]
                work = work + torch.where(has, end - beg, torch.zeros_like(beg)).sum(0)
            prefix = torch.cat([work.new_zeros(1), torch.cumsum(work.double() + node_weight, 0)])
            total = float(prefix[-1])
            bounds = [0]
            for r in range(1, W):
                cut = int(torch.searchsorted(prefix, torch.tensor(total * r / W, dtype=prefix.dtype)))
                cut = min(N, max(bounds[-1], (cut + align // 2) // align * align))
                bounds.append(cut)
            bounds.append(N)
            cache[key] = bounds
        return list(cache[key])

    def workgroup_bounds(self, n0, n1, groups, row_weight=8, min_gain=1.08):
        n0, n1, groups = int(n0), int(n1), int(groups)
        key = ('wg', n0, n1, groups, int(row_weight), float(min_gain))
        cache = self.__dict__.setdefault('_shard_cache', {})
        if key not in cache:
            n = n1 - n0
            g = max(1, min(groups, n))
            rp = self.rowptr[:, n0:n1 + 1].cpu().to(torch.int64)
            prefix = (rp[0] - rp[0, 0]) + (rp[1] - rp[1, 0]) + row_weight * torch.arange(n + 1, dtype=torch.int64)
            rpw = (-(-n // groups) + 15) // 16 * 16
            eq = torch.arange(0, n + rpw, rpw, dtype=torch.int64).clamp(max=n)
            eq_work = prefix[eq[1:]] - prefix[eq[:-1]]
            if float(eq_work.max()) <= min_gain * float(prefix[-1]) / groups:
                cache[key] = None
                return None
            idx = torch.arange(1, g, dtype=torch.int64)
            cuts = torch.searchsorted(prefix, (idx * int(prefix[-1])) // g)
            cuts = torch.minimum(torch.maximum(cuts, idx), n - (g - idx))
            cuts = torch.cummax(cuts, 0).values if g > 1 else cuts
            per = -(-n // g)
            cap = (per + 15) // 16 * 16 if per <= 80 else (per + 79) // 80 * 80
            b = [0] + cuts.tolist() + [n]
            for i in range(1, g):
                b[i] = min(max(b[i], b[i - 1] + 1), b[i - 1] + cap)
            for i in range(g - 1, 0, -1):
                b[i] = max(b[i], b[i + 1] - cap)
            bounds = torch.tensor(b, dtype=torch.int32)
            cache[key] = bounds.to(self.rowptr.device)
        return cache[key]

    def shard_slot_counts(self, n0, n1):
        (i0, i1), (o0, o1), (h0, h1) = self._shard_bounds(n0, n1)
        return i1 - i0, o1 - o0, h1 - h0

    def shard_ee_sub(self, n0, n1):
        (i0, i1), (o0, o1), (h0, h1) = self._shard_bounds(n0, n1)
        return i0, o0 - (i1 - i0), h0 - (i1 - i0) - (o1 - o0)

    def shard_backward_index(self, n0, n1):
        key = ('bwd', int(n0), int(n1))
        cache = self.__dict__.setdefault('_shard_cache', {})
        if key not in cache:
            (i0, i1), (o0, o1), (h0, h1) = self._shard_bounds(n0, n1)
            dev, i32 = self.rec.device, torch.int32
            slots = torch.cat([torch.arange(i0, i1), torch.arange(o0, o1), torch.arange(h0, h1)]).to(dev)
            e2, N = 2 * self.num_edges_half, self.num_nodes
            rec = self.rec.index_select(0, slots).to(torch.int64)
            half = (self.slot_dst.index_select(0, slots).to(torch.int64) >> 31) & 1
            typ = rec[:, 1]
            type_rows = torch.sort(typ, stable=True).indices
            counts = torch.bincount(typ, minlength=self.num_rel_rows)
            type_ptr = torch.cat([counts.new_zeros(1), counts.cumsum(0)])
            group = rec[:, 0] * 2 + half
            skey = group * e2 + self.mirror.index_select(0, slots).to(torch.int64)
            skey_sorted, src_rows = torch.sort(skey)
            counts = torch.bincount(group, minlength=2 * N)
            src_ptr = torch.cat([counts.new_zeros(1), counts.cumsum(0)])
            src_chunks = torch.zeros((max(self.num_chunks, 1), 4), dtype=torch.int64, device=dev)
            if self.num_chunks:
                ch = self.chunks[:self.num_chunks].to(torch.int64)
                sd = self.slot_dst.index_select(0, ch[:, 0]).to(torch.int64)
                base = ((sd & 0x7fffffff) * 2 + (1 - ((sd >> 31) & 1))) * e2
                src_chunks[:self.num_chunks, 0] = torch.searchsorted(skey_sorted, base + ch[:, 0])
                src_chunks[:self.num_chunks, 1] = torch.searchsorted(skey_sorted, base + ch[:, 1])
                src_chunks[:self.num_chunks, 2:] = ch[:, 2:]
            cache[key] = dict(type_ptr=type_ptr.to(i32), type_rows=type_rows.to(i32), src_ptr=src_ptr.to(i32),
                              src_rows=src_rows.to(i32), src_chunks=src_chunks.to(i32).contiguous())
        return cache[key]

    def edge_table_shard(self, table_slot_order, n0, n1):
        (i0, i1), (o0, o1), (h0, h1) = self._shard_bounds(n0, n1)
        return torch.cat([table_slot_order[i0:i1], table_slot_order[o0:o1], table_slot_order[h0:h1]], dim=0).contiguous()

    def norms(self):
        return self.rec[:, 2].contiguous().view(torch.float32)


class Graph(object):
    def __init__(self, edge_index=None, edge_attr=None, **kwargs):
        self.edge_index = edge_index
        self.edge_attr = edge_attr
        for k, v in kwargs.items():
            setattr(self, k, v)
        self._csr = {}

    def to(self, device):
        for k, v in list(self.__dict__.items()):
            if torch.is_tensor(v):
                setattr(self, k, v.to(device))
        for c in self._csr.values():
            c.to(device)
        return self

    def csr(self, num_rel_rows, with_backward=True):
        dev = self.edge_index.device
        key = (int(num_rel_rows), self.edge_index.data_ptr(), self.edge_attr.data_ptr(), str(dev))
        hit = self._csr.get(key)
        if hit is None or (with_backward and not hit.has_backward):
            self._csr.clear()
            n = self.num_nodes if getattr(self, 'num_nodes', None) is not None else int(self.edge_index.max()) + 1
            hit = GraphCSR(n, num_rel_rows, self.edge_index, self.edge_attr[0], dev, with_backward)
            self._csr[key] = hit
        return hit


_tensor_csr_cache = {}


def csr_for_tensors(num_nodes, num_rel_rows, edge_index, edge_type):
    key = (int(num_nodes), int(num_rel_rows), edge_index.data_ptr(), edge_type.data_ptr(), tuple(edge_index.shape),
           edge_index._version, edge_type._version, str(edge_index.device))
    hit = _tensor_csr_cache.get(key)
    if hit is None:
        if len(_tensor_csr_cache) > 8:
            _tensor_csr_cache.clear()
        hit = GraphCSR(num_nodes, num_rel_rows, edge_index, edge_type, edge_index.device)
        _tensor_csr_cache[key] = hit
    return hit
```

Measured before the change: 2.779 billion edges/s.

## Walk a compacted live-edge CSR view that drops zero-norm slots in fused forward

Builds a second CSR on the host that keeps only edge records with nonzero norm and stores each record's original slot id in eid. The fused forward kernels (generations 2 and 3) can walk this view and recover the original slot through a shuffle when they index per-edge embeddings, so slots that contribute nothing are never gathered. It is on by default through an environment flag. The cost is extra memory for the live view and another template variant of each kernel.

```diff
diff --git a/include/mgcn_hip.h b/include/mgcn_hip.h
--- a/include/mgcn_hip.h
+++ b/include/mgcn_hip.h
@@ -45,6 +45,10 @@
                         int32_t *chunks_host, int64_t max_chunks, int64_t *num_chunks_host,
                         int32_t *slot_dst_host, int32_t *mirror_host, int32_t *typeptr_host,
                         int32_t *typeslots_host);
+
+int mgcn_csr_live_view_host(int64_t num_nodes, const int32_t *rowptr_host, const mgcn_edge_rec *rec_host,
+                            int32_t *live_rowptr_host, mgcn_edge_rec *live_rec_host, int64_t max_live,
+                            int64_t *num_live_host, int64_t *num_dead_host);
 
 int64_t mgcn_hub_partial_floats(int64_t num_chunks, int32_t dim);
 int mgcn_aggregate_fwd(int64_t num_nodes, int64_t num_edges_half, int32_t dim, int32_t num_rel_rows,
@@ -91,6 +95,18 @@
                          const int32_t *chunks_dev, int64_t chunk_begin, int64_t chunk_end, float *partial_dev,
                          const float *rels_weight_dev, float *rel_out_dev, const int32_t *row_bounds_dev,
                          int32_t num_row_bounds, int32_t tune, uint32_t *status_dev, void *stream);
+int mgcn_layer_fwd_fused_live(int64_t num_nodes, int64_t num_edges_half, int32_t dim_in, int32_t dim_out,
+                              int32_t num_rel_rows, const int32_t *live_rowptr_dev, const mgcn_edge_rec *live_rec_dev,
+                              const mgcn_edge_rec *rec_dev, const float *x_dev, int64_t ldx, const float *rel_dev,
+                              const float *loop_rel_dev, const float *ee_dev, int32_t ee_in_slot_order,
+                              const float *loop_edge_dev, const float *wp_dev, const float *bias_dev,
+                              const float *bn_mean_dev, const float *bn_var_dev, const float *bn_gamma_dev,
+                              const float *bn_beta_dev, float bn_eps, float *out_dev, int64_t ldo, int64_t node_begin,
+                              int64_t node_end, int64_t ee_sub_in, int64_t ee_sub_out, int64_t ee_sub_hub,
+                              const int32_t *hubinfo_dev, const int32_t *chunks_dev, int64_t chunk_begin,
+                              int64_t chunk_end, float *partial_dev, const float *rels_weight_dev, float *rel_out_dev,
+                              const int32_t *row_bounds_dev, int32_t num_row_bounds, int32_t tune, uint32_t *status_dev,
+                              void *stream);
 int mgcn_pack_weights(int32_t dim_in, int32_t dim_out, const float *w_dev, float *wp_dev, size_t wp_bytes, void *stream);
 size_t mgcn_packed_weights_bytes(int32_t dim_in, int32_t dim_out);
 int mgcn_pack_weights_gen(int32_t generation, int32_t dim_in, int32_t dim_out, const float *w_dev, float *wp_dev,
diff --git a/kgc-gcn_amd/_native.py b/kgc-gcn_amd/_native.py
--- a/kgc-gcn_amd/_native.py
+++ b/kgc-gcn_amd/_native.py
@@ -35,6 +35,11 @@
                                             _ptr, _ptr, _ptr, _ptr, _ptr, _ptr, _ptr, _f32, _ptr, _i64, _i64, _i64,
                                             _i64, _i64, _i64, _ptr, _ptr, _i64, _i64, _ptr, _ptr, _ptr, _ptr, _i32, _i32, _ptr,
                                             _ptr]),
+    'mgcn_layer_fwd_fused_live': (ctypes.c_int, [_i64, _i64, _i32, _i32, _i32, _ptr, _ptr, _ptr, _ptr, _i64, _ptr, _ptr, _ptr, _i32,
+                                                 _ptr, _ptr, _ptr, _ptr, _ptr, _ptr, _ptr, _f32, _ptr, _i64, _i64, _i64,
+                                                 _i64, _i64, _i64, _ptr, _ptr, _i64, _i64, _ptr, _ptr, _ptr, _ptr, _i32, _i32, _ptr,
+                                                 _ptr]),
+    'mgcn_csr_live_view_host': (ctypes.c_int, [_i64, _ptr, _ptr, _ptr, _ptr, _i64, ctypes.POINTER(_i64), ctypes.POINTER(_i64)]),
     'mgcn_pack_weights': (ctypes.c_int, [_i32, _i32, _ptr, _ptr, ctypes.c_size_t, _ptr]),
     'mgcn_packed_weights_bytes': (ctypes.c_size_t, [_i32, _i32]),
     'mgcn_pack_weights_gen': (ctypes.c_int, [_i32, _i32, _i32, _ptr, _ptr, ctypes.c_size_t, _ptr]),
@@ -184,6 +189,30 @@
     return out
 
 
+def csr_live_view_host(rowptr, rec):
+    if rowptr.dim() != 2 or rowptr.size(0) != 2 or rowptr.size(1) < 1 or rowptr.dtype != torch.int32 or rowptr.is_cuda or \
+            not rowptr.is_contiguous() or rec.dtype != torch.int32 or rec.is_cuda or not rec.is_contiguous() or \
+            (rec.numel() and (rec.dim() != 2 or rec.size(1) != 4)):
+        raise NativeError('csr_live_view: rowptr must be a contiguous host int32 [2, N+1], rec a contiguous host int32 [2E, 4]')
+    N = rowptr.size(1) - 1
+    if int(rowptr[1, N]) > rec.size(0) or int(rowptr[0, 0]) < 0:
+        raise NativeError('csr_live_view: rowptr points past the records')
+    live, dead = ctypes.c_int64(0), ctypes.c_int64(0)
+    call = lambda lrp, lrec, cap: _check(lib().mgcn_csr_live_view_host(
+        N, rowptr.data_ptr(), rec.data_ptr(), lrp, lrec, cap, ctypes.byref(live), ctypes.byref(dead)), 'mgcn_csr_live_view_host')
+    L = int(rowptr[1, N]) - int(rowptr[0, 0])
+    out = dict(live_rowptr=torch.empty((2, N + 1), dtype=torch.int32), live_rec=torch.empty((max(L, 1), 4), dtype=torch.int32))
+    call(out['live_rowptr'].data_ptr(), out['live_rec'].data_ptr(), L)
+    if dead.value == 0:
+        return None
+    out['live_rec'] = out['live_rec'][:max(int(live.value), 1)].contiguous()
+    out['num_live'], out['num_dead'] = int(live.value), int(dead.value)
+    return out
+
+
+LIVE_SLOTS = os.environ.get('MGCN_LIVE_SLOTS', '1') != '0'
+
+
 def _hub_args(csr, d, device, n0, n1):
     c0, c1 = csr.chunk_range(n0, n1)
     if c1 == c0:
@@ -425,7 +454,7 @@
 
 def layer_fwd_fused(csr, x, rel, loop_rel, ee, ee_in_slot_order, loop_edge, w_packed, d_out, bias, bn_mean, bn_var,
                     bn_gamma, bn_beta, eps, out, node_range=None, ee_sub=(0, 0, 0), rels_weight=None, rel_out=None,
-                    tune=None, balance=True):
+                    tune=None, balance=True, live=None):
     N, E, D, O = csr.num_nodes, csr.num_edges_half, x.size(1), int(d_out)
     n0, n1 = (0, N) if node_range is None else (int(node_range[0]), int(node_range[1]))
     if not 0 <= n0 <= n1 <= N:
@@ -464,8 +493,17 @@
         ee = x.new_zeros((1, D))
     hub_info, hub_chunks, hub_c0, hub_c1, hub_partial = _hub_args(csr, D, x.device, n0, n1)
     bounds = csr.workgroup_bounds(n0, n1, _cu_count(x.device)) if balance and n1 > n0 else None
-    rc = lib().mgcn_layer_fwd_fused(
-        N, E, D, O, csr.num_rel_rows, _dev(csr.rowptr, torch.int32, 'rowptr'), _dev(csr.rec, torch.int32, 'rec'),
+    has_view = getattr(csr, 'live_rowptr', None) is not None and tune_generation(tune) != 4
+    if live and not has_view:
+        raise NativeError('layer_fwd_fused: live=True, but this graph has no live view (no dead slot) or tune forces generation 4')
+    live = has_view and (LIVE_SLOTS if live is None else bool(live))
+    if live:
+        fn, head = lib().mgcn_layer_fwd_fused_live, (_dev(csr.live_rowptr, torch.int32, 'live_rowptr'),
+                                                     _dev(csr.live_rec, torch.int32, 'live_rec'), _dev(csr.rec, torch.int32, 'rec'))
+    else:
+        fn, head = lib().mgcn_layer_fwd_fused, (_dev(csr.rowptr, torch.int32, 'rowptr'), _dev(csr.rec, torch.int32, 'rec'))
+    rc = fn(
+        N, E, D, O, csr.num_rel_rows, *head,
         _dev(x, torch.float32, 'x'), _ld(x), _dev(rel, torch.float32, 'rel'), _dev(loop_rel, torch.float32, 'loop_rel'),
         _dev(ee, torch.float32, 'ee', True), int(bool(ee_in_slot_order)), _dev(loop_edge, torch.float32, 'loop_edge'),
         _dev(w_packed, torch.float32, 'w_packed'), _dev(bias, torch.float32, 'bias', True),
diff --git a/kgc-gcn_amd/csrc/csr_build.cpp b/kgc-gcn_amd/csrc/csr_build.cpp
--- a/kgc-gcn_amd/csrc/csr_build.cpp
+++ b/kgc-gcn_amd/csrc/csr_build.cpp
@@ -119,3 +119,40 @@
   }
   return MGCN_OK;
 }
+
+extern "C" int mgcn_csr_live_view_host(int64_t num_nodes, const int32_t *rowptr_host, const mgcn_edge_rec *rec_host,
+                                       int32_t *live_rowptr_host, mgcn_edge_rec *live_rec_host, int64_t max_live,
+                                       int64_t *num_live_host, int64_t *num_dead_host) {
+  const int64_t N = num_nodes;
+  MGCN_REQUIRE(N >= 0 && rowptr_host && num_live_host && num_dead_host, "csr_live_view: bad arguments");
+  int64_t live = 0, dead = 0;
+  for (int64_t i = 0; i < 2 * N + 1; ++i)
+    MGCN_REQUIRE(rowptr_host[i] >= 0 && rowptr_host[i] <= rowptr_host[i + 1], "csr_live_view: rowptr decreases at entry %lld",
+                 (long long)i);
+  for (int h = 0; h < 2; ++h) {
+    const int32_t *rowptr = rowptr_host + h * (N + 1);
+    MGCN_REQUIRE(rowptr[N] == rowptr[0] || rec_host, "csr_live_view: null records");
+    for (int64_t s = rowptr[0]; s < rowptr[N]; ++s) (rec_host[s].norm != 0.0f ? live : dead)++;
+  }
+  *num_live_host = live;
+  *num_dead_host = dead;
+  if (dead == 0) return MGCN_OK;
+  MGCN_REQUIRE(live_rowptr_host && (live == 0 || live_rec_host) && max_live >= live,
+               "csr_live_view: outputs missing or too small for %lld live slots", (long long)live);
+  int64_t pos = 0;
+  for (int h = 0; h < 2; ++h) {
+    const int32_t *rowptr = rowptr_host + h * (N + 1);
+    int32_t *lrp = live_rowptr_host + h * (N + 1);
+    for (int64_t n = 0; n < N; ++n) {
+      lrp[n] = int32_t(pos);
+      for (int64_t s = rowptr[n]; s < rowptr[n + 1]; ++s) {
+        if (rec_host[s].norm == 0.0f) continue;
+        mgcn_edge_rec r = rec_host[s];
+        r.eid = int32_t(s);
+        live_rec_host[pos++] = r;
+      }
+    }
+    lrp[N] = int32_t(pos);
+  }
+  return MGCN_OK;
+}
diff --git a/kgc-gcn_amd/csrc/layer_fused.hip b/kgc-gcn_amd/csrc/layer_fused.hip
--- a/kgc-gcn_amd/csrc/layer_fused.hip
+++ b/kgc-gcn_amd/csrc/layer_fused.hip
@@ -50,18 +50,17 @@
   return (with_row_bounds && few_tiles && dim_out > 128) ? 3 : 2;
 }
 
-extern "C" int mgcn_layer_fwd_fused(int64_t num_nodes, int64_t num_edges_half, int32_t dim_in, int32_t dim_out,
-                                    int32_t num_rel_rows, const int32_t *rowptr_dev, const mgcn_edge_rec *rec_dev,
-                                    const float *x_dev, int64_t ldx, const float *rel_dev, const float *loop_rel_dev,
-                                    const float *ee_dev, int32_t ee_in_slot_order, const float *loop_edge_dev,
-                                    const float *wp_dev, const float *bias_dev, const float *bn_mean_dev,
-                                    const float *bn_var_dev, const float *bn_gamma_dev, const float *bn_beta_dev,
-                                    float bn_eps, float *out_dev, int64_t ldo, int64_t node_begin, int64_t node_end,
-                                    int64_t ee_sub_in, int64_t ee_sub_out, int64_t ee_sub_hub,
-                                    const int32_t *hubinfo_dev, const int32_t *chunks_dev, int64_t chunk_begin,
-                                    int64_t chunk_end, float *partial_dev, const float *rels_weight_dev,
-                                    float *rel_out_dev, const int32_t *row_bounds_dev, int32_t num_row_bounds,
-                                    int32_t tune, uint32_t *status_dev, void *stream) {
+namespace {
+int layer_fwd_fused(int64_t num_nodes, int64_t num_edges_half, int32_t dim_in, int32_t dim_out, int32_t num_rel_rows,
+                    const int32_t *rowptr_dev, const mgcn_edge_rec *rec_dev, const int32_t *live_rowptr_dev,
+                    const mgcn_edge_rec *live_rec_dev, const float *x_dev, int64_t ldx, const float *rel_dev,
+                    const float *loop_rel_dev, const float *ee_dev, int32_t ee_in_slot_order, const float *loop_edge_dev,
+                    const float *wp_dev, const float *bias_dev, const float *bn_mean_dev, const float *bn_var_dev,
+                    const float *bn_gamma_dev, const float *bn_beta_dev, float bn_eps, float *out_dev, int64_t ldo,
+                    int64_t node_begin, int64_t node_end, int64_t ee_sub_in, int64_t ee_sub_out, int64_t ee_sub_hub,
+                    const int32_t *hubinfo_dev, const int32_t *chunks_dev, int64_t chunk_begin, int64_t chunk_end,
+                    float *partial_dev, const float *rels_weight_dev, float *rel_out_dev, const int32_t *row_bounds_dev,
+                    int32_t num_row_bounds, int32_t tune, uint32_t *status_dev, void *stream) {
   MGCN_REQUIRE(num_nodes >= 0 && num_edges_half >= 0 && dim_in > 0 && dim_out > 0 && num_rel_rows > 0,
                "layer_fwd_fused: bad sizes");
   MGCN_REQUIRE(node_begin >= 0 && node_begin <= node_end && node_end <= num_nodes, "layer_fwd_fused: bad node range");
@@ -98,12 +97,55 @@
                dim_in, dim_out);
   MGCN_REQUIRE(num_row_bounds >= 0 && num_row_bounds <= 4096 && (num_row_bounds == 0 || row_bounds_dev),
                "layer_fwd_fused: bad row bounds");
-  const mgcn::FusedLaunch a = {num_nodes, dim_in, dim_out, num_rel_rows, rowptr_dev, rec_dev, x_dev, ldx, rel_dev, loop_rel_dev, ee_dev,
+  const bool live = live_rowptr_dev != nullptr;
+  MGCN_REQUIRE(!live || gen != 4, "layer_fwd_fused: tune %d: generation 4 does not walk a live view", tune);
+  const mgcn::FusedLaunch a = {num_nodes, dim_in, dim_out, num_rel_rows, live ? live_rowptr_dev : rowptr_dev,
+                               live ? live_rec_dev : rec_dev, x_dev, ldx, rel_dev, loop_rel_dev, ee_dev,
                                loop_edge_dev, wp_dev, bias_dev, bn_mean_dev, bn_var_dev, bn_gamma_dev, bn_beta_dev, bn_eps, out_dev, ldo,
                                node_begin, node_end, ee_sub_in, ee_sub_out, num_chunks > 0 ? hubinfo_dev : nullptr, chunk_begin,
                                partial_dev, want_rel ? rels_weight_dev : nullptr, want_rel ? rel_out_dev : nullptr, row_bounds_dev,
-                               num_row_bounds, tune, status_dev, stream};
+                               num_row_bounds, tune, status_dev, stream, live};
   if (gen == 4) return mgcn::fused4_launch(a);
   if (gen == 2) return mgcn::fused2_launch(a);
   return mgcn::fused3_launch(a);
 }
+}
+
+extern "C" int mgcn_layer_fwd_fused(int64_t num_nodes, int64_t num_edges_half, int32_t dim_in, int32_t dim_out,
+                                    int32_t num_rel_rows, const int32_t *rowptr_dev, const mgcn_edge_rec *rec_dev,
+                                    const float *x_dev, int64_t ldx, const float *rel_dev, const float *loop_rel_dev,
+                                    const float *ee_dev, int32_t ee_in_slot_order, const float *loop_edge_dev,
+                                    const float *wp_dev, const float *bias_dev, const float *bn_mean_dev,
+                                    const float *bn_var_dev, const float *bn_gamma_dev, const float *bn_beta_dev,
+                                    float bn_eps, float *out_dev, int64_t ldo, int64_t node_begin, int64_t node_end,
+                                    int64_t ee_sub_in, int64_t ee_sub_out, int64_t ee_sub_hub,
+                                    const int32_t *hubinfo_dev, const int32_t *chunks_dev, int64_t chunk_begin,
+                                    int64_t chunk_end, float *partial_dev, const float *rels_weight_dev,
+                                    float *rel_out_dev, const int32_t *row_bounds_dev, int32_t num_row_bounds,
+                                    int32_t tune, uint32_t *status_dev, void *stream) {
+  return layer_fwd_fused(num_nodes, num_edges_half, dim_in, dim_out, num_rel_rows, rowptr_dev, rec_dev, nullptr, nullptr, x_dev, ldx,
+                         rel_dev, loop_rel_dev, ee_dev, ee_in_slot_order, loop_edge_dev, wp_dev, bias_dev, bn_mean_dev, bn_var_dev,
+                         bn_gamma_dev, bn_beta_dev, bn_eps, out_dev, ldo, node_begin, node_end, ee_sub_in, ee_sub_out, ee_sub_hub,
+                         hubinfo_dev, chunks_dev, chunk_begin, chunk_end, partial_dev, rels_weight_dev, rel_out_dev, row_bounds_dev,
+                         num_row_bounds, tune, status_dev, stream);
+}
+
+extern "C" int mgcn_layer_fwd_fused_live(int64_t num_nodes, int64_t num_edges_half, int32_t dim_in, int32_t dim_out,
+                                         int32_t num_rel_rows, const int32_t *live_rowptr_dev,
+                                         const mgcn_edge_rec *live_rec_dev, const mgcn_edge_rec *rec_dev, const float *x_dev,
+                                         int64_t ldx, const float *rel_dev, const float *loop_rel_dev, const float *ee_dev,
+                                         int32_t ee_in_slot_order, const float *loop_edge_dev, const float *wp_dev,
+                                         const float *bias_dev, const float *bn_mean_dev, const float *bn_var_dev,
+                                         const float *bn_gamma_dev, const float *bn_beta_dev, float bn_eps, float *out_dev,
+                                         int64_t ldo, int64_t node_begin, int64_t node_end, int64_t ee_sub_in,
+                                         int64_t ee_sub_out, int64_t ee_sub_hub, const int32_t *hubinfo_dev,
+                                         const int32_t *chunks_dev, int64_t chunk_begin, int64_t chunk_end, float *partial_dev,
+                                         const float *rels_weight_dev, float *rel_out_dev, const int32_t *row_bounds_dev,
+                                         int32_t num_row_bounds, int32_t tune, uint32_t *status_dev, void *stream) {
+  MGCN_REQUIRE(live_rowptr_dev && live_rec_dev, "layer_fwd_fused_live: null live view");
+  return layer_fwd_fused(num_nodes, num_edges_half, dim_in, dim_out, num_rel_rows, live_rowptr_dev, rec_dev, live_rowptr_dev,
+                         live_rec_dev, x_dev, ldx, rel_dev, loop_rel_dev, ee_dev, ee_in_slot_order, loop_edge_dev, wp_dev, bias_dev,
+                         bn_mean_dev, bn_var_dev, bn_gamma_dev, bn_beta_dev, bn_eps, out_dev, ldo, node_begin, node_end, ee_sub_in,
+                         ee_sub_out, ee_sub_hub, hubinfo_dev, chunks_dev, chunk_begin, chunk_end, partial_dev, rels_weight_dev,
+                         rel_out_dev, row_bounds_dev, num_row_bounds, tune, status_dev, stream);
+}
diff --git a/kgc-gcn_amd/csrc/layer_fused2.hip b/kgc-gcn_amd/csrc/layer_fused2.hip
--- a/kgc-gcn_amd/csrc/layer_fused2.hip
+++ b/kgc-gcn_amd/csrc/layer_fused2.hip
@@ -31,7 +31,7 @@
 constexpr int EPI_FLOATS = 2 * 208;
 constexpr int REL_LDS_MAX_BYTES = 32 * 1024;
 
-template <int NT, int NRT, bool RELLDS, bool HUBS>
+template <int NT, int NRT, bool RELLDS, bool HUBS, bool LIVE>
 __global__ __launch_bounds__(T2, 4) void layer_fused2_kernel(Args2 p) {
   constexpr int BM = NRT * 16;
   constexpr int PIECE = 16 * BM * 16;
@@ -192,7 +192,8 @@
                 if (MGCN_ABLATE(16)) rsrc[u] = 0;
                 xv[u] = *reinterpret_cast<const float4 *>(xb + uint64_t(uint32_t(rsrc[u])) * ldx32);
                 if (!RELLDS) rv[u] = *reinterpret_cast<const float4 *>(relb + uint64_t(uint32_t(rtyp[u])) * d32);
-                const uint32_t erow = MGCN_ABLATE(16) ? 0u : uint32_t(((s + u < end) ? s + u : end - 1) - ee_sub_mode);
+                const int pos = (s + u < end) ? s + u : end - 1;
+                const uint32_t erow = MGCN_ABLATE(16) ? 0u : uint32_t((LIVE ? __shfl(myrec.w, glane0 + (pos - cbase)) : pos) - ee_sub_mode);
                 ev[u] = *reinterpret_cast<const float4 *>(eeb + uint64_t(erow) * d32);
               }
 #ifdef MGCN_DIAG
@@ -450,18 +451,34 @@
   }
 }
 
-template <int NT, int NRT, bool RELLDS, bool HUBS>
+template <int NT, int NRT, bool RELLDS, bool HUBS, bool LIVE>
 int launch2(const Args2 &p, int grid, hipStream_t st) {
   constexpr size_t lds_bytes = size_t(2) * 3 * 16 * (NRT * 16) * 16 + EPI_FLOATS * 4 + (RELLDS ? REL_LDS_MAX_BYTES : 0);
-  if (hipFuncSetAttribute(reinterpret_cast<const void *>(&layer_fused2_kernel<NT, NRT, RELLDS, HUBS>),
+  if (hipFuncSetAttribute(reinterpret_cast<const void *>(&layer_fused2_kernel<NT, NRT, RELLDS, HUBS, LIVE>),
                           hipFuncAttributeMaxDynamicSharedMemorySize, int(lds_bytes)) != hipSuccess)
     return mgcn::fail(MGCN_ELAUNCH, "layer_fused2: cannot reserve %zu bytes of LDS", lds_bytes);
-  hipLaunchKernelGGL((layer_fused2_kernel<NT, NRT, RELLDS, HUBS>), dim3(unsigned(grid)), dim3(T2), lds_bytes, st, p);
+  hipLaunchKernelGGL((layer_fused2_kernel<NT, NRT, RELLDS, HUBS, LIVE>), dim3(unsigned(grid)), dim3(T2), lds_bytes, st, p);
   MGCN_CHECK_LAUNCH("layer_fused2_kernel");
   return MGCN_OK;
 }
 
 int pick_nt2(int o) { return o <= 32 ? 2 : o <= 64 ? 4 : o <= 128 ? 8 : 13; }
+
+template <bool LIVE>
+int pick2(const Args2 &p, int dim_out, int nrt, int grid, int grid5, bool rel_lds, bool hubs, hipStream_t st) {
+  switch (pick_nt2(dim_out)) {
+    case 2: return launch2<2, 5, false, true, LIVE>(p, grid5, st);
+    case 4: return launch2<4, 5, false, true, LIVE>(p, grid5, st);
+    case 8: return launch2<8, 5, false, true, LIVE>(p, grid5, st);
+    default:
+      if (nrt == 4) {
+        if (rel_lds) return hubs ? launch2<13, 4, true, true, LIVE>(p, grid, st) : launch2<13, 4, true, false, LIVE>(p, grid, st);
+        return hubs ? launch2<13, 4, false, true, LIVE>(p, grid, st) : launch2<13, 4, false, false, LIVE>(p, grid, st);
+      }
+      if (rel_lds) return hubs ? launch2<13, 5, true, true, LIVE>(p, grid, st) : launch2<13, 5, true, false, LIVE>(p, grid, st);
+      return hubs ? launch2<13, 5, false, true, LIVE>(p, grid, st) : launch2<13, 5, false, false, LIVE>(p, grid, st);
+  }
+}
 
 struct Shape2 {
   int nch, nkb_last, kbm, G;
@@ -533,18 +550,8 @@
   hipStream_t st = static_cast<hipStream_t>(a.stream);
   const bool rel_lds = a.rel && size_t(a.num_rel_rows - 1) * dim_in * 4 <= size_t(REL_LDS_MAX_BYTES);
   const bool hubs = a.hubinfo != nullptr;
-  switch (pick_nt2(dim_out)) {
-    case 2: return launch2<2, 5, false, true>(p, grid_for(5), st);
-    case 4: return launch2<4, 5, false, true>(p, grid_for(5), st);
-    case 8: return launch2<8, 5, false, true>(p, grid_for(5), st);
-    default:
-      if (nrt == 4) {
-        if (rel_lds) return hubs ? launch2<13, 4, true, true>(p, grid, st) : launch2<13, 4, true, false>(p, grid, st);
-        return hubs ? launch2<13, 4, false, true>(p, grid, st) : launch2<13, 4, false, false>(p, grid, st);
-      }
-      if (rel_lds) return hubs ? launch2<13, 5, true, true>(p, grid, st) : launch2<13, 5, true, false>(p, grid, st);
-      return hubs ? launch2<13, 5, false, true>(p, grid, st) : launch2<13, 5, false, false>(p, grid, st);
-  }
-}
-
-}
+  return a.live ? pick2<true>(p, dim_out, nrt, grid, grid_for(5), rel_lds, hubs, st)
+                : pick2<false>(p, dim_out, nrt, grid, grid_for(5), rel_lds, hubs, st);
+}
+
+}
diff --git a/kgc-gcn_amd/csrc/layer_fused3.hip b/kgc-gcn_amd/csrc/layer_fused3.hip
--- a/kgc-gcn_amd/csrc/layer_fused3.hip
+++ b/kgc-gcn_amd/csrc/layer_fused3.hip
@@ -45,7 +45,7 @@
   asm volatile("" ::: "memory");
 }
 
-template <int NT, int NRT, int NCH, bool RELLDS>
+template <int NT, int NRT, int NCH, bool RELLDS, bool LIVE>
 __global__ __launch_bounds__(T3, 4) void layer_fused3_kernel(Args3 p) {
   constexpr int BM = NRT * 16;
   constexpr int UB = 4 / NCH;
@@ -261,7 +261,8 @@
               float4 xv[UB][NCH], rv[UB][NCH], ev[UB][NCH];
 #pragma unroll
               for (int u = 0; u < UB; ++u) {
-                const uint32_t erow = uint32_t(((s + u < end) ? s + u : end - 1) - ee_sub_mode);
+                const int pos = (s + u < end) ? s + u : end - 1;
+                const uint32_t erow = uint32_t((LIVE ? __shfl(myrec.w, glane0 + (pos - cbase)) : pos) - ee_sub_mode);
 #pragma unroll
                 for (int j = 0; j < NCH; ++j) {
                   xv[u][j] = *reinterpret_cast<const float4 *>(p.x + coff[j] + uint64_t(uint32_t(rsrc[u])) * ldx32);
@@ -595,27 +596,31 @@
   return size_t(3) * s.ncc * (nrt * 16) * 16 + size_t(nimg) * (nrt * 16) * s.ncc * 32 + 64 + size_t(2) * nt * 16 * 4 + rel_bytes;
 }
 
-template <int NT, int NRT, int NCH, bool RELLDS>
+template <int NT, int NRT, int NCH, bool RELLDS, bool LIVE>
 int launch3(const Args3 &p, int grid, size_t lds, hipStream_t st) {
-  if (hipFuncSetAttribute(reinterpret_cast<const void *>(&layer_fused3_kernel<NT, NRT, NCH, RELLDS>),
+  if (hipFuncSetAttribute(reinterpret_cast<const void *>(&layer_fused3_kernel<NT, NRT, NCH, RELLDS, LIVE>),
                           hipFuncAttributeMaxDynamicSharedMemorySize, int(LDS_MAX)) != hipSuccess)
     return mgcn::fail(MGCN_ELAUNCH, "layer_fused3: cannot reserve %zu bytes of LDS", LDS_MAX);
-  hipLaunchKernelGGL((layer_fused3_kernel<NT, NRT, NCH, RELLDS>), dim3(unsigned(grid)), dim3(T3), lds, st, p);
+  hipLaunchKernelGGL((layer_fused3_kernel<NT, NRT, NCH, RELLDS, LIVE>), dim3(unsigned(grid)), dim3(T3), lds, st, p);
   MGCN_CHECK_LAUNCH("layer_fused3_kernel");
   return MGCN_OK;
 }
 
 template <int NT, int NRT, int NCH>
-int launch3_rel(const Args3 &p, int grid, size_t lds, bool rel_lds, hipStream_t st) {
-  if (rel_lds) return launch3<NT, NRT, NCH, true>(p, grid, lds, st);
-  return launch3<NT, NRT, NCH, false>(p, grid, lds, st);
+int launch3_rel(const Args3 &p, int grid, size_t lds, bool rel_lds, bool live, hipStream_t st) {
+  if (live) {
+    if (rel_lds) return launch3<NT, NRT, NCH, true, true>(p, grid, lds, st);
+    return launch3<NT, NRT, NCH, false, true>(p, grid, lds, st);
+  }
+  if (rel_lds) return launch3<NT, NRT, NCH, true, false>(p, grid, lds, st);
+  return launch3<NT, NRT, NCH, false, false>(p, grid, lds, st);
 }
 
 template <int NT, int NCH>
-int launch3_nrt(const Args3 &p, int nrt, int grid, size_t lds, bool rel_lds, hipStream_t st) {
-  if (nrt == 3) return launch3_rel<NT, 3, NCH>(p, grid, lds, rel_lds, st);
-  if (nrt == 4) return launch3_rel<NT, 4, NCH>(p, grid, lds, rel_lds, st);
-  return launch3_rel<NT, 5, NCH>(p, grid, lds, rel_lds, st);
+int launch3_nrt(const Args3 &p, int nrt, int grid, size_t lds, bool rel_lds, bool live, hipStream_t st) {
+  if (nrt == 3) return launch3_rel<NT, 3, NCH>(p, grid, lds, rel_lds, live, st);
+  if (nrt == 4) return launch3_rel<NT, 4, NCH>(p, grid, lds, rel_lds, live, st);
+  return launch3_rel<NT, 5, NCH>(p, grid, lds, rel_lds, live, st);
 }
 
 }
@@ -695,11 +700,11 @@
   const size_t lds = lds_bytes3(s, nrt, nimg, nt, rel_lds ? rel_bytes : 0);
   hipStream_t st = static_cast<hipStream_t>(a.stream);
   if (nt == 32) {
-    if (s.nch == 1) return launch3_rel<32, 3, 1>(p, grid, lds, rel_lds, st);
-    return launch3_rel<32, 3, 2>(p, grid, lds, rel_lds, st);
+    if (s.nch == 1) return launch3_rel<32, 3, 1>(p, grid, lds, rel_lds, a.live, st);
+    return launch3_rel<32, 3, 2>(p, grid, lds, rel_lds, a.live, st);
   }
-  if (s.nch == 1) return launch3_nrt<13, 1>(p, nrt, grid, lds, rel_lds, st);
-  return launch3_nrt<13, 2>(p, nrt, grid, lds, rel_lds, st);
-}
-
-}
+  if (s.nch == 1) return launch3_nrt<13, 1>(p, nrt, grid, lds, rel_lds, a.live, st);
+  return launch3_nrt<13, 2>(p, nrt, grid, lds, rel_lds, a.live, st);
+}
+
+}
diff --git a/kgc-gcn_amd/csrc/mgcn_common.h b/kgc-gcn_amd/csrc/mgcn_common.h
--- a/kgc-gcn_amd/csrc/mgcn_common.h
+++ b/kgc-gcn_amd/csrc/mgcn_common.h
@@ -56,6 +56,7 @@
   int32_t tune;
   uint32_t *status;
   void *stream;
+  bool live;
 };
 
 bool fused2_takes(int32_t dim_in, int32_t dim_out);
diff --git a/kgc-gcn_amd/graph.py b/kgc-gcn_amd/graph.py
--- a/kgc-gcn_amd/graph.py
+++ b/kgc-gcn_amd/graph.py
@@ -5,12 +5,16 @@
 
 class GraphCSR(object):
 
-    _FIELDS = ('rowptr', 'rec', 'perm', 'hubinfo', 'chunks', 'slot_dst', 'mirror', 'typeptr', 'typeslots')
+    _FIELDS = ('rowptr', 'rec', 'perm', 'hubinfo', 'chunks', 'slot_dst', 'mirror', 'typeptr', 'typeslots', 'live_rowptr', 'live_rec')
 
     def __init__(self, num_nodes, num_rel_rows, edge_index, edge_type, device, with_backward=True, hub_threshold=None,
                  hub_chunk=None):
         host = _native.csr_build_host(num_nodes, num_rel_rows, edge_index, edge_type, with_backward, hub_threshold,
                                       hub_chunk)
+        live = _native.csr_live_view_host(host['rowptr'], host['rec'])
+        if live is not None:
+            host.update(live_rowptr=live['live_rowptr'], live_rec=live['live_rec'])
+        self.num_dead_slots = live['num_dead'] if live is not None else 0
         self.num_chunks = host['num_chunks']
         self.num_nodes = int(num_nodes)
         self.num_edges_half = int(edge_index.size(1)) // 2
```

New measurement: 2.901 billion edges/s, median of 6. +4.4%, better.
